# google/dynibar

Measured on AMD Instinct MI355X. Metric: rays/sec (64 samples x 8 src views), higher is better.
Workload: dtype f32 in / f32 accumulate; products from two half-float parts per operand (22-bit operands, 3 of the 4 partial products on the f16 matrix pipe, ~2^-20 relative per product); the exact 6-term bf16 build is tested beside it

## Files before the change

### dynibar_amd/csrc/dyn_mlp.h

```cpp
#pragma once
#include <utility>

#include "dyn_device.h"

#ifndef DYN_EXCLUSIVE_CU
#define DYN_EXCLUSIVE_CU 1
#endif
#if DYN_EXCLUSIVE_CU && defined(__AMDGCN__)
#define DYN_CLAIM_REGISTER_FILE() asm volatile("; the whole register file" ::: "v255", "a255")
#else
#define DYN_CLAIM_REGISTER_FILE()
#endif
#define DYN_NET_THREADS 256
#define DYN_VIEW_THREADS 512

__host__ __device__ constexpr int dyn_fi(int r, int h) { return (r & 3) + 8 * (r >> 2) + 4 * h; }

__device__ __forceinline__ f32x16 mfma32(float a, float b, f32x16 c) { return __builtin_amdgcn_mfma_f32_32x32x2f32(a, b, c, 0, 0, 0); }

template <int NT>
__device__ __forceinline__ void acc_zero(f32x16 (&acc)[NT]) {
#pragma unroll
  for (int t = 0; t < NT; ++t)
#pragma unroll
// ... 201 lines not shown
  int fill, issued;
  int nbuf;
#ifdef DYN_PHASE_TIMING
  int kid;
#endif
};


#ifndef B6_DMA_POLICY
#define B6_DMA_POLICY ""
#endif
#ifndef B6_DMA_WINDOW_NUM
#define B6_DMA_WINDOW_NUM 2
#define B6_DMA_WINDOW_DEN 3
#endif
template <int OFF>
__device__ __forceinline__ void b6_dma_piece(const float* g_uniform, unsigned lane_off, unsigned l, float* l_emu) {
#if defined(__AMDGCN__)
#pragma clang diagnostic push
#pragma clang diagnostic ignored "-Winline-asm"
  asm volatile("s_mov_b32 m0, %2\n\ts_nop 0\n\tglobal_load_lds_dwordx4 %0, %1 offset:%3" B6_DMA_POLICY ::"v"(lane_off), "s"(g_uniform), "s"(l), "n"(OFF) : "m0", "memory");
#pragma clang diagnostic pop
#else
  __builtin_amdgcn_global_load_lds((const __attribute__((address_space(1))) void*)((const char*)g_uniform + lane_off),
                                   (__attribute__((address_space(3))) void*)l_emu, 16, OFF, 0);
#endif
}
__device__ __forceinline__ int ring6_pieces(const WeightRing6& R) { return B6_CHUNK / R.round; }
__device__ __forceinline__ void ring6_piece(const WeightRing6& R, int k) {
  const int waves = R.round / 256, per_wave = B6_CHUNK / waves;
  const int grp = k / 6, i = k % 6;
  const int chunk = R.fill;
  const float* gu = R.gbase + (long)(chunk + (chunk >= R.skip_at ? R.skip_n : 0)) * B6_CHUNK + grp * 1536;
  const int slot = R.nbuf == 2 ? (chunk & 1) : 0;
  const unsigned l = R.lds_wave + (unsigned)((slot * B6_CHUNK + grp * 1536) * sizeof(float));
  float* le = R.buf + slot * B6_CHUNK + (threadIdx.x >> 6) * per_wave + 512 + grp * 1536;
  if (i == 0) b6_dma_piece<-2048>(gu, R.lane_off, l, le);
  if (i == 1) b6_dma_piece<-1024>(gu, R.lane_off, l, le);
  if (i == 2) b6_dma_piece<0>(gu, R.lane_off, l, le);
  if (i == 3) b6_dma_piece<1024>(gu, R.lane_off, l, le);
  if (i == 4) b6_dma_piece<2048>(gu, R.lane_off, l, le);
  if (i == 5) b6_dma_piece<3072>(gu, R.lane_off, l, le);
}
__device__ __forceinline__ void ring6_feed(WeightRing6& R, int pr, int npc) {
  if (R.fill < 0) return;
  const int n = ring6_pieces(R);
  const int den = (B6_DMA_WINDOW_NUM * npc + B6_DMA_WINDOW_DEN - 1) / B6_DMA_WINDOW_DEN > 0 ? (B6_DMA_WINDOW_NUM * npc + B6_DMA_WINDOW_DEN - 1) / B6_DMA_WINDOW_DEN : 1;
  int want = (n * (pr + 1) + den - 1) / den;
  if (want > n) want = n;
  for (; R.issued < want; ++R.issued) ring6_piece(R, R.issued);
}

__device__ __forceinline__ void ring6_issue(const WeightRing6& R, int chunk) {
  const int waves = R.round / 256, wave = threadIdx.x >> 6, lane = threadIdx.x & 63;
  const int per_wave = B6_CHUNK / waves;
  const float* g = R.gbase + (long)(chunk + (chunk >= R.skip_at ? R.skip_n : 0)) * B6_CHUNK + wave * per_wave + 512 + lane * 4;
  float* l = R.buf + (R.nbuf == 2 ? (chunk & 1) : 0) * B6_CHUNK + wave * per_wave + 512;
#pragma unroll
  for (int grp = 0; grp < 2; ++grp)
    if (grp * 1536 < per_wave) {
      const auto* gg = (const __attribute__((address_space(1))) void*)(g + grp * 1536);
      auto* ll = (__attribute__((address_space(3))) void*)(l + grp * 1536);
      __builtin_amdgcn_global_load_lds(gg, ll, 16, -2048, 0);
      __builtin_amdgcn_global_load_lds(gg, ll, 16, -1024, 0);
      __builtin_amdgcn_global_load_lds(gg, ll, 16, 0, 0);
      __builtin_amdgcn_global_load_lds(gg, ll, 16, 1024, 0);
      __builtin_amdgcn_global_load_lds(gg, ll, 16, 2048, 0);
      __builtin_amdgcn_global_load_lds(gg, ll, 16, 3072, 0);
    }
}
__device__ __forceinline__ void ring6_init(WeightRing6& R, const float* stream, int total, float* lds, int skip_at = 1 << 30, int skip_n = 0,
                                           int threads = 0, int nbuf = 2) {
  R.gbase = stream;
  R.buf = lds;
  R.next = 0;
  R.total = total - skip_n;
  R.skip_at = skip_at;
  R.skip_n = skip_n;
  R.round = (threads > 0 ? threads : (int)blockDim.x) * 4;
  R.nbuf = nbuf;
#if defined(__AMDGCN__)
  R.half = __builtin_amdgcn_readfirstlane((int)threadIdx.x >> 8);
#else
  R.half = (int)threadIdx.x >> 8;
#endif
  {
    const int waves = R.round / 256, per_wave = B6_CHUNK / waves;
#if defined(__AMDGCN__)
    const int wave = __builtin_amdgcn_readfirstlane((int)threadIdx.x >> 6);
    R.lds_wave = (unsigned)(size_t)(__attribute__((address_space(3))) void*)(lds + wave * per_wave + 512);
#else
    const int wave = (int)threadIdx.x >> 6;
    R.lds_wave = 0;
#endif
    R.lane_off = (unsigned)((wave * per_wave + 512 + (threadIdx.x & 63) * 4) * sizeof(float));
  }
  R.fill = -1;
  R.issued = 0;
  DYN_PHASE_RING_KID(R, 0);
  ring6_issue(R, 0);
}
__device__ __forceinline__ const float* ring6_acquire(WeightRing6& R) {
  DYN_PHASE_T0
  if (R.nbuf == 1) {
    const int c = R.next++;
    if (c > 0) {
      __syncthreads();
      ring6_issue(R, c);
    }
    __builtin_amdgcn_s_waitcnt(0x0F70);
    __syncthreads();
    DYN_PHASE_WAIT(R, c);
    return R.buf;
  }
  if (R.fill >= 0) {
    const int n = ring6_pieces(R);
    for (; R.issued < n; ++R.issued) ring6_piece(R, R.issued);
    R.fill = -1;
  }
  __builtin_amdgcn_s_waitcnt(0x0F70);
#ifdef DYN_PHASE_SKEW
  const unsigned long long skew_t1 = __builtin_readcyclecounter();
#endif
  __syncthreads();
  const int c = R.next++;
#ifdef DYN_PHASE_SKEW
  if ((threadIdx.x & 63) == 0 && blockIdx.x == gridDim.x / 2 && R.kid == 0) {
    g_skew[threadIdx.x >> 6][0] += skew_t1 - phase_t0;
    g_skew[threadIdx.x >> 6][1] += __builtin_readcyclecounter() - skew_t1;
    g_skew[threadIdx.x >> 6][2] += 1;
  }
#endif
  DYN_PHASE_WAIT(R, c);
  R.fill = c + 1 < R.total ? c + 1 : -1;
  R.issued = 0;
  return R.buf + (c & 1) * B6_CHUNK;
}

#ifndef B6_PRIO_FLIP
#define B6_PRIO_FLIP 2
#endif
#ifndef B6_PRIO_MODE
#define B6_PRIO_MODE 5
#endif
__device__ __forceinline__ void ring6_prio_flip(const WeightRing6& R, int phase) {
#if defined(__AMDGCN__)
  if (R.round != 8 * 256) return;
#if B6_PRIO_MODE == 1
  if (phase & 1) __builtin_amdgcn_s_setprio(1);
  else __builtin_amdgcn_s_setprio(0);
#elif B6_PRIO_MODE == 5
  if ((((int)threadIdx.x >> 8) ^ phase) & 1) __builtin_amdgcn_s_setprio(1);
  else __builtin_amdgcn_s_setprio(0);
#endif
#endif
}
__device__ __forceinline__ void split3_pair(float a, float b, unsigned& hi, unsigned& mid, unsigned& lo) {
#if DYN_SPLIT_F16
  const auto h = __builtin_amdgcn_cvt_pkrtz(a, b);
  hi = __builtin_bit_cast(unsigned, h);
#if defined(__AMDGCN__)
  unsigned m;
  asm("v_fma_mixlo_f16 %0, %1, -1.0, %2 op_sel_hi:[1,0,0]" : "=v"(m) : "v"(hi), "v"(a));
  asm("v_fma_mixhi_f16 %0, %1, -1.0, %2 op_sel:[1,0,0] op_sel_hi:[1,0,0]" : "+v"(m) : "v"(hi), "v"(b));
  mid = m;
#else
  const float ra = a - (float)h[0], rb = b - (float)h[1];
  mid = __builtin_bit_cast(unsigned, __builtin_amdgcn_cvt_pkrtz(ra, rb));
#endif
  lo = 0u;
#else
  f32x2v v = {a, b};
  hi = __builtin_bit_cast(unsigned, __builtin_convertvector(v, bf16x2v));
  f32x2v hf = {__uint_as_float(hi << 16), __uint_as_float(hi & 0xffff0000u)};
  f32x2v r1 = v - hf;
  mid = __builtin_bit_cast(unsigned, __builtin_convertvector(r1, bf16x2v));
#if DYN_SPLIT_PARTS == 3
  f32x2v mf = {__uint_as_float(mid << 16), __uint_as_float(mid & 0xffff0000u)};
  f32x2v r2 = r1 - mf;
  lo = __builtin_bit_cast(unsigned, __builtin_convertvector(r2, bf16x2v));
#else
  lo = 0u;
#endif
#endif
}

__device__ __forceinline__ f32x16 mfma_bf16(u32x4v a, u32x4v b, f32x16 c) {
#if DYN_SPLIT_F16
  return __builtin_amdgcn_mfma_f32_32x32x16_f16(__builtin_bit_cast(f16x8, a), __builtin_bit_cast(f16x8, b), c, 0, 0, 0);
#else
  return __builtin_amdgcn_mfma_f32_32x32x16_bf16(__builtin_bit_cast(bf16x8, a), __builtin_bit_cast(bf16x8, b), c, 0, 0, 0);
#endif
}

__host__ __device__ constexpr int b6_layer_chunks(int NT, int NSLOTS, int CP = B6_CHUNK_PAIRS) {
  return (((NSLOTS + 7) / 8) + (CP / NT) - 1) / (CP / NT);
}

struct B6A {
  u32x4v hi, mid, lo;
};
__device__ __forceinline__ B6A b6_load_a(const float* pair, int lane) {
  const u32x4v* w = reinterpret_cast<const u32x4v*>(pair) + lane;
  B6A a;
  a.hi = w[0]; a.mid = w[64];
#if DYN_SPLIT_PARTS == 3
  a.lo = w[128];
#endif
  return a;
}

template <int NSLOTS, int P0, int P1, class Feed>
__device__ __forceinline__ void b6_split_pairs(Feed& feed, int g, u32x4v& bh, u32x4v& bm, u32x4v& bl) {
#pragma unroll
  for (int p2 = P0; p2 < P1; ++p2) {
    const float v0 = (g * 8 + 2 * p2 < NSLOTS) ? feed(g * 8 + 2 * p2) : 0.f;
    const float v1 = (g * 8 + 2 * p2 + 1 < NSLOTS) ? feed(g * 8 + 2 * p2 + 1) : 0.f;
    unsigned h_, m_, l_;
    split3_pair(v0, v1, h_, m_, l_);
    bh[p2] = h_; bm[p2] = m_; bl[p2] = l_;
  }
}

#ifndef B6_AHEAD
#define B6_AHEAD 1
#endif
template <int NT, int NSLOTS, int AHEAD = B6_AHEAD, class Feed>
__device__ __forceinline__ void mlp_layer_b6(WeightRing6& R, f32x16 (&acc)[NT], Feed&& feed) {
  constexpr int NG = (NSLOTS + 7) / 8;
  constexpr int GPC = B6_CHUNK_PAIRS / NT;
  constexpr int NCH = (NG + GPC - 1) / GPC;
  static_assert(B6_CHUNK_PAIRS % NT == 0, "tiles per layer must divide the pairs of a chunk");
  static_assert(NT == 1 || NT == 2 || NT == 4 || NT == 8, "output tiles per layer");
  const int lane = threadIdx.x & 63;
  u32x4v bh, bm, bl, nh, nm, nl;
  b6_split_pairs<NSLOTS, 0, 4>(feed, 0, bh, bm, bl);
  nh = bh; nm = bm; nl = bl;
  __builtin_amdgcn_sched_barrier(0);
#pragma unroll
  for (int c = 0; c < NCH; ++c) {
    const float* buf = ring6_acquire(R);
    constexpr int NPC_MAX = B6_CHUNK_PAIRS;
    const int npc = (NG - c * GPC < GPC ? NG - c * GPC : GPC) * NT;
    B6A q[AHEAD + 1];
#pragma unroll
    for (int i = 0; i < AHEAD; ++i)
      if (i < npc) q[i] = b6_load_a(buf + i * B6_PAIR_FLOATS, lane);
    __builtin_amdgcn_sched_barrier(0);
#pragma unroll
    for (int pr = 0; pr < NPC_MAX; ++pr) {
      if (pr < npc) {
        const int gi = pr / NT, t = pr % NT;
        const int g = c * GPC + gi;
        ring6_feed(R, pr, npc);
#if B6_PRIO_FLIP && (B6_PRIO_MODE == 1 || B6_PRIO_MODE == 5)
        if (pr % B6_PRIO_FLIP == 0) ring6_prio_flip(R, (pr / B6_PRIO_FLIP) & 1);
#endif
        if (pr + AHEAD < npc) q[(pr + AHEAD) % (AHEAD + 1)] = b6_load_a(buf + (pr + AHEAD) * B6_PAIR_FLOATS, lane);
        if (g + 1 < NG) {
          if (NT == 1) b6_split_pairs<NSLOTS, 0, 4>(feed, g + 1, nh, nm, nl);
          if (NT == 2 && t == 0) b6_split_pairs<NSLOTS, 0, 2>(feed, g + 1, nh, nm, nl);
          if (NT == 2 && t == 1) b6_split_pairs<NSLOTS, 2, 4>(feed, g + 1, nh, nm, nl);
          if (NT == 4 && t == 0) b6_split_pairs<NSLOTS, 0, 1>(feed, g + 1, nh, nm, nl);
          if (NT == 4 && t == 1) b6_split_pairs<NSLOTS, 1, 2>(feed, g + 1, nh, nm, nl);
          if (NT == 4 && t == 2) b6_split_pairs<NSLOTS, 2, 3>(feed, g + 1, nh, nm, nl);
          if (NT == 4 && t == 3) b6_split_pairs<NSLOTS, 3, 4>(feed, g + 1, nh, nm, nl);
          if (NT == 8 && t == 0) b6_split_pairs<NSLOTS, 0, 1>(feed, g + 1, nh, nm, nl);
          if (NT == 8 && t == 2) b6_split_pairs<NSLOTS, 1, 2>(feed, g + 1, nh, nm, nl);
          if (NT == 8 && t == 4) b6_split_pairs<NSLOTS, 2, 3>(feed, g + 1, nh, nm, nl);
          if (NT == 8 && t == 6) b6_split_pairs<NSLOTS, 3, 4>(feed, g + 1, nh, nm, nl);
        }
        const B6A& cur = q[pr % (AHEAD + 1)];
#if DYN_SPLIT_TERMS == 6
        acc[t] = mfma_bf16(cur.lo, bh, acc[t]);
        acc[t] = mfma_bf16(cur.hi, bl, acc[t]);
        acc[t] = mfma_bf16(cur.mid, bm, acc[t]);
#endif
        acc[t] = mfma_bf16(cur.mid, bh, acc[t]);
        acc[t] = mfma_bf16(cur.hi, bm, acc[t]);
        acc[t] = mfma_bf16(cur.hi, bh, acc[t]);
        if (t == NT - 1) { bh = nh; bm = nm; bl = nl; }
        __builtin_amdgcn_sched_barrier(0);
      }
    }
  }
}

#ifndef B6D_AHEAD
#define B6D_AHEAD 4
#endif
#define B6D_SLOTS 3
struct WeightRing3 {
  const float* gbase;
  const float* glane;
  float* buf;
  unsigned lds_wave;
  unsigned lane_off;
  int next, total;
  int waves;
  int cf;
  int fill, issued;
  float* slot[B6D_SLOTS];
  unsigned lds_slot[B6D_SLOTS];
  int wrap;
  bool more;
#ifdef DYN_PHASE_TIMING
  int kid;
#endif
};
template <int OFF>
__device__ __forceinline__ void ring3_dma(const float* g, float* l_emu, unsigned l, const float* g_uniform, unsigned lane_off) {
#if defined(__AMDGCN__)
#pragma clang diagnostic push
#pragma clang diagnostic ignored "-Winline-asm"
  asm volatile("s_mov_b32 m0, %2\n\ts_nop 0\n\tglobal_load_lds_dwordx4 %0, %1 offset:%3" ::"v"(lane_off), "s"(g_uniform), "s"(l), "n"(OFF) : "m0", "memory");
#pragma clang diagnostic pop
#else
  __builtin_amdgcn_global_load_lds((const __attribute__((address_space(1))) void*)g, (__attribute__((address_space(3))) void*)l_emu, 16, OFF, 0);
#endif
}
__device__ __forceinline__ int ring3_pieces(const WeightRing3& R) { return R.cf / (R.waves * 256); }
__device__ __forceinline__ void ring3_piece(const WeightRing3& R, int chunk, int k) {
  const int per_wave = R.cf / R.waves;
  const int grp = k / 6, i = k % 6;
  const int sc = chunk >= R.total ? chunk - R.total : chunk;
  const float* g = R.glane + (long)sc * R.cf + grp * 1536;
  const float* gu = R.gbase + (long)sc * R.cf + grp * 1536;
  const unsigned l = R.lds_slot[chunk % B6D_SLOTS] + (unsigned)(grp * 1536 * sizeof(float));
  float* le = R.slot[chunk % B6D_SLOTS] + (threadIdx.x >> 6) * per_wave + 512 + grp * 1536;
  if (i == 0) ring3_dma<-2048>(g, le, l, gu, R.lane_off);
  if (i == 1) ring3_dma<-1024>(g, le, l, gu, R.lane_off);
  if (i == 2) ring3_dma<0>(g, le, l, gu, R.lane_off);
  if (i == 3) ring3_dma<1024>(g, le, l, gu, R.lane_off);
  if (i == 4) ring3_dma<2048>(g, le, l, gu, R.lane_off);
  if (i == 5) ring3_dma<3072>(g, le, l, gu, R.lane_off);
}
template <int ALLOW = 0>
__device__ __forceinline__ void ring3_barrier() {
#if defined(__AMDGCN__)
  static_assert(ALLOW >= 0 && ALLOW < 16, "vmcnt immediate");
  __builtin_amdgcn_s_waitcnt(0x0F70 | ALLOW);
  __builtin_amdgcn_s_barrier();
#else
  __syncthreads();
#endif
}
__device__ __forceinline__ void ring3_init(WeightRing3& R, const float* stream, int total, float* lds, int threads, int chunk_pairs = B6_CHUNK_PAIRS) {
  R.gbase = stream;
  R.buf = lds;
  R.next = 0;
  R.total = total;
  R.waves = threads / 64;
  R.cf = chunk_pairs * B6_PAIR_FLOATS;
  {
    const int per_wave = R.cf / R.waves;
#if defined(__AMDGCN__)
    const int wave = __builtin_amdgcn_readfirstlane((int)threadIdx.x >> 6);
    R.lds_wave = (unsigned)(size_t)(__attribute__((address_space(3))) void*)(lds + wave * per_wave + 512);
#else
    const int wave = threadIdx.x >> 6;
    R.lds_wave = 0;
#endif
    R.glane = stream + wave * per_wave + 512 + (threadIdx.x & 63) * 4;
    R.lane_off = (unsigned)((wave * per_wave + 512 + (threadIdx.x & 63) * 4) * sizeof(float));
  }
  R.fill = -1;
  R.issued = 0;
  R.wrap = 0;
  R.more = false;
  for (int j = 0; j < B6D_SLOTS; ++j) {
    R.slot[j] = lds + j * R.cf;
    R.lds_slot[j] = R.lds_wave + (unsigned)(j * R.cf * sizeof(float));
  }
  DYN_PHASE_RING_KID(R, 0);
  for (int c = 0; c < 2 && c < total; ++c)
    for (int k = 0; k < ring3_pieces(R); ++k) ring3_piece(R, c, k);
}
__device__ __forceinline__ void ring3_enter(WeightRing3& R) {
  if (R.next != 0) return;
  const int n = R.total > 1 ? ring3_pieces(R) : 0;
  if (n == 12) ring3_barrier<12>();
  else if (n == 8) ring3_barrier<8>();
  else if (n == 6) ring3_barrier<6>();
  else if (n == 4) ring3_barrier<4>();
  else ring3_barrier<0>();
}
__device__ __forceinline__ const float* ring3_slot(const WeightRing3& R, int chunk) { return R.slot[chunk % B6D_SLOTS]; }
#ifndef B6D_DMA_MARGIN
#define B6D_DMA_MARGIN 4
#endif
__device__ __forceinline__ void ring3_feed(WeightRing3& R, int half, int num, int den) {
  if (R.fill < 0) return;
  if (R.fill >= R.total && !R.more) return;
  const int n = ring3_pieces(R), h0 = n / 2;
  int want = half == 0 ? (h0 * num + den - 1) / den : h0 + ((n - h0) * num + den - 1) / den;
  if (want > n) want = n;
  for (; R.issued < want; ++R.issued) ring3_piece(R, R.fill, R.issued);
}
__device__ __forceinline__ void ring3_mid(WeightRing3& R) {
  DYN_PHASE_T0
  ring3_feed(R, 1, 1, 1);
  if (R.next + 1 < R.total || R.wrap) ring3_barrier();
  DYN_PHASE_WAIT(R, R.next);
  R.fill = (R.next + 2 < R.total || R.wrap) ? R.next + 2 : -1;
  R.issued = 0;
}
__device__ __forceinline__ void ring3_leave(WeightRing3& R) {
  if (R.wrap && R.next == R.total - 1) ring3_feed(R, 1, 1, 1);
  ++R.next;
}
__device__ __forceinline__ void ring3_next_pass(WeightRing3& R) {
  float* s0[B6D_SLOTS];
  unsigned l0[B6D_SLOTS];
  for (int j = 0; j < B6D_SLOTS; ++j) { s0[j] = R.slot[j]; l0[j] = R.lds_slot[j]; }
  for (int j = 0; j < B6D_SLOTS; ++j) { R.slot[j] = s0[(R.total + j) % B6D_SLOTS]; R.lds_slot[j] = l0[(R.total + j) % B6D_SLOTS]; }
  R.next = 0;
  R.fill = -1;
  R.issued = 0;
}

__device__ __forceinline__ float relu1(float v) {
#if defined(__AMDGCN__)
  float r;
  asm("v_max_f32_e32 %0, 0, %1" : "=v"(r) : "v"(v));
  return r;
#else
  return v > 0.f ? v : 0.f;
#endif
}

template <class F, int... Is>
__device__ __forceinline__ void dyn_static_for_impl(F&& f, std::integer_sequence<int, Is...>) {
  (f(std::integral_constant<int, Is>{}), ...);
}
template <int N, class F>
__device__ __forceinline__ void dyn_static_for(F&& f) {
  dyn_static_for_impl(static_cast<F&&>(f), std::make_integer_sequence<int, N>{});
}
#define DYN_INLINE_LAMBDA __attribute__((always_inline))

__device__ __forceinline__ f32x16 mfma_pinned(const u32x4v& a, u32x4v& b, f32x16 c) {
#if defined(__AMDGCN__)
  asm volatile("" : "+v"(b));
  f32x16 d = mfma_bf16(a, b, c);
  asm volatile("" : "+a"(d));
  return d;
#else
  return mfma_bf16(a, b, c);
#endif
}

template <int NT, int NSLOTS, int CP = B6_CHUNK_PAIRS, int AHEAD = B6D_AHEAD, class Feed>
__device__ __forceinline__ void mlp_layer_b6_duo(WeightRing3& R, f32x16 (&acc)[NT], Feed&& feed) {
  constexpr int NG = (NSLOTS + 7) / 8;
  constexpr int NP = NG * NT;
  constexpr int U = NT >= 2 ? 2 : 1;
  constexpr int QN = AHEAD + U;
  constexpr int NM = 3 * 4 * U / NT;
  static_assert(CP % NT == 0 && (NT == 1 || NT == 2 || NT == 4 || NT == 8), "output tiles per layer; pairs per chunk (CP) a multiple of them");
  static_assert(AHEAD % 2 == 0 && AHEAD >= 2 && AHEAD <= CP / 2, "the look-ahead must stay inside the published half chunk");
  const int lane = threadIdx.x & 63;
  const int c0 = R.next;
  u32x4v bh, bm, bl, nh, nm, nl;
  b6_split_pairs<NSLOTS, 0, 4>(feed, 0, bh, bm, bl);
  nh = bh; nm = bm; nl = bl;
  float v0 = 0.f, v1 = 0.f;
  B6A q[QN];
  auto load = [&](int P) DYN_INLINE_LAMBDA {
    return b6_load_a(ring3_slot(R, c0 + P / CP) + (P % CP) * B6_PAIR_FLOATS, lane);
  };
  ring3_enter(R);
#if !defined(__AMDGCN__)
  for (int i = 0; i < AHEAD && i < NP; ++i) q[i % QN] = load(i);
  for (int P = 0; P < NP; P += U) {
    const int pr = P % CP, npc = NP - (P - pr) < CP ? NP - (P - pr) : CP, mid = (npc / 2) / U * U;
    const int g = P / NT, t0 = P % NT, t1 = t0 + U - 1, um = (P % NT) / U;
    if (pr == mid) ring3_mid(R);
    auto gap = [&](int K) {
      for (int m = 0; m < NM; ++m) {
        const int at = NT == 1 ? 0 : (NM <= 4 ? 2 + m : m * 6 / NM);
        if (at != K || g + 1 >= NG) continue;
        const int step = um * NM + m, p2 = step / 3, st = step % 3, s0 = (g + 1) * 8 + 2 * p2;
        if (st == 0) v0 = s0 < NSLOTS ? feed(s0) : 0.f;
        if (st == 1) v1 = s0 + 1 < NSLOTS ? feed(s0 + 1) : 0.f;
        if (st == 2) {
          unsigned h_, m_, l_;
          split3_pair(v0, v1, h_, m_, l_);
          nh[p2] = h_; nm[p2] = m_; nl[p2] = l_;
        }
      }
    };
    auto dma = [&](int done) {
      const int wend = mid - B6D_DMA_MARGIN;
      if (pr >= mid) ring3_feed(R, 0, pr + done - mid, npc - mid);
      else if (wend <= 0) ring3_feed(R, 1, 1, 1);
      else ring3_feed(R, 1, pr + done < wend ? pr + done : wend, wend);
    };
    if (P + AHEAD < NP) q[(P + AHEAD) % QN] = load(P + AHEAD);
    gap(0);
    const B6A a0 = q[P % QN], a1 = q[(P + U - 1) % QN];
#if DYN_SPLIT_TERMS == 6
    acc[t0] = mfma_bf16(a0.lo, bh, acc[t0]);
    if (U == 2) acc[t1] = mfma_bf16(a1.lo, bh, acc[t1]);
    acc[t0] = mfma_bf16(a0.hi, bl, acc[t0]);
    if (U == 2) acc[t1] = mfma_bf16(a1.hi, bl, acc[t1]);
    acc[t0] = mfma_bf16(a0.mid, bm, acc[t0]);
    if (U == 2) acc[t1] = mfma_bf16(a1.mid, bm, acc[t1]);
#endif
    acc[t0] = mfma_bf16(a0.mid, bh, acc[t0]);
    if (U == 2) {
      if (P + AHEAD + 1 < NP) q[(P + AHEAD + 1) % QN] = load(P + AHEAD + 1);
      gap(1);
      acc[t1] = mfma_bf16(a1.mid, bh, acc[t1]);
      gap(2);
    }
    acc[t0] = mfma_bf16(a0.hi, bm, acc[t0]);
    if (U == 2) {
      gap(3);
      dma(1);
      acc[t1] = mfma_bf16(a1.hi, bm, acc[t1]);
      gap(4);
    }
    acc[t0] = mfma_bf16(a0.hi, bh, acc[t0]);
    if (U == 2) {
      gap(5);
      dma(U);
      acc[t1] = mfma_bf16(a1.hi, bh, acc[t1]);
    } else {
      dma(U);
    }
    if (t1 == NT - 1) { bh = nh; bm = nm; bl = nl; }
    if (pr + U == npc) ring3_leave(R);
  }
  return;
#endif
  dyn_static_for<(AHEAD < NP ? AHEAD : NP)>([&](auto I) DYN_INLINE_LAMBDA { q[decltype(I)::value % QN] = load(decltype(I)::value); });
  __builtin_amdgcn_sched_barrier(0);
  dyn_static_for<NP / U>([&](auto I) DYN_INLINE_LAMBDA {
    constexpr int P = decltype(I)::value * U;
    constexpr int pr = P % CP;
    constexpr int npc = NP - (P - pr) < CP ? NP - (P - pr) : CP;
    constexpr int mid = (npc / 2) / U * U;
    constexpr int g = P / NT, t0 = P % NT, t1 = t0 + U - 1;
    constexpr int um = (P % NT) / U;
    if constexpr (pr == mid) ring3_mid(R);
    auto gap = [&](auto K) DYN_INLINE_LAMBDA {
      dyn_static_for<NM>([&](auto M) DYN_INLINE_LAMBDA {
        constexpr int m = decltype(M)::value;
        constexpr int at = NT == 1 ? 0 : (NM <= 4 ? 2 + m : m * 6 / NM);
        if constexpr (at == decltype(K)::value && g + 1 < NG) {
          constexpr int step = um * NM + m, p2 = step / 3, st = step % 3, s0 = (g + 1) * 8 + 2 * p2;
          if constexpr (st == 0) v0 = s0 < NSLOTS ? feed(s0) : 0.f;
          if constexpr (st == 1) v1 = s0 + 1 < NSLOTS ? feed(s0 + 1) : 0.f;
          if constexpr (st == 2) {
            unsigned h_, m_, l_;
            split3_pair(v0, v1, h_, m_, l_);
            nh[p2] = h_; nm[p2] = m_; nl[p2] = l_;
          }
        }
      });
    };
    auto dma = [&](auto D) DYN_INLINE_LAMBDA {
      constexpr int done = decltype(D)::value;
      constexpr int wend = mid - B6D_DMA_MARGIN;
      if constexpr (pr >= mid) ring3_feed(R, 0, pr + done - mid, npc - mid);
      else if constexpr (wend <= 0) ring3_feed(R, 1, 1, 1);
      else ring3_feed(R, 1, pr + done < wend ? pr + done : wend, wend);
    };
    if constexpr (P + AHEAD < NP) q[(P + AHEAD) % QN] = load(P + AHEAD);
    gap(std::integral_constant<int, 0>{});
    const B6A& a0 = q[P % QN];
    const B6A& a1 = q[(P + U - 1) % QN];
#if DYN_SPLIT_TERMS == 6
    acc[t0] = mfma_pinned(a0.lo, bh, acc[t0]);
    if constexpr (U == 2) acc[t1] = mfma_pinned(a1.lo, bh, acc[t1]);
    acc[t0] = mfma_pinned(a0.hi, bl, acc[t0]);
    if constexpr (U == 2) acc[t1] = mfma_pinned(a1.hi, bl, acc[t1]);
    acc[t0] = mfma_pinned(a0.mid, bm, acc[t0]);
    if constexpr (U == 2) acc[t1] = mfma_pinned(a1.mid, bm, acc[t1]);
#endif
    acc[t0] = mfma_pinned(a0.mid, bh, acc[t0]);
    __builtin_amdgcn_sched_barrier(0);
    if constexpr (U == 2) {
      if constexpr (P + AHEAD + 1 < NP) q[(P + AHEAD + 1) % QN] = load(P + AHEAD + 1);
      gap(std::integral_constant<int, 1>{});
      acc[t1] = mfma_pinned(a1.mid, bh, acc[t1]);
      __builtin_amdgcn_sched_barrier(0);
      gap(std::integral_constant<int, 2>{});
    }
    acc[t0] = mfma_pinned(a0.hi, bm, acc[t0]);
    if constexpr (U == 2) {
      __builtin_amdgcn_sched_barrier(0);
      gap(std::integral_constant<int, 3>{});
      dma(std::integral_constant<int, 1>{});
      acc[t1] = mfma_pinned(a1.hi, bm, acc[t1]);
      __builtin_amdgcn_sched_barrier(0);
      gap(std::integral_constant<int, 4>{});
    }
    acc[t0] = mfma_pinned(a0.hi, bh, acc[t0]);
    if constexpr (U == 2) {
      __builtin_amdgcn_sched_barrier(0);
      gap(std::integral_constant<int, 5>{});
      dma(std::integral_constant<int, U>{});
      acc[t1] = mfma_pinned(a1.hi, bh, acc[t1]);
    } else {
      dma(std::integral_constant<int, U>{});
    }
    if constexpr (t1 == NT - 1) { bh = nh; bm = nm; bl = nl; }
    if constexpr (pr + U == npc) ring3_leave(R);
    __builtin_amdgcn_sched_barrier(0);
  });
}

template <int NT, int NSLOTS, int AHEAD = B6_AHEAD, class Feed>
__device__ __forceinline__ void mlp_layer_b6_lds(const float* w, f32x16 (&acc)[NT], Feed&& feed) {
  constexpr int NG = (NSLOTS + 7) / 8, NPR = NG * NT;
  static_assert(NT == 1 || NT == 2 || NT == 4 || NT == 8, "output tiles per layer");
  const int lane = threadIdx.x & 63;
  u32x4v bh, bm, bl, nh, nm, nl;
  b6_split_pairs<NSLOTS, 0, 4>(feed, 0, bh, bm, bl);
  nh = bh; nm = bm; nl = bl;
  B6A q[AHEAD + 1];
#pragma unroll
  for (int i = 0; i < AHEAD; ++i)
    if (i < NPR) q[i] = b6_load_a(w + i * B6_PAIR_FLOATS, lane);
  __builtin_amdgcn_sched_barrier(0);
#pragma unroll
  for (int pr = 0; pr < NPR; ++pr) {
    const int g = pr / NT, t = pr % NT;
    if (pr + AHEAD < NPR) q[(pr + AHEAD) % (AHEAD + 1)] = b6_load_a(w + (pr + AHEAD) * B6_PAIR_FLOATS, lane);
    if (g + 1 < NG) {
      if (NT == 1) b6_split_pairs<NSLOTS, 0, 4>(feed, g + 1, nh, nm, nl);
      if (NT == 2 && t == 0) b6_split_pairs<NSLOTS, 0, 2>(feed, g + 1, nh, nm, nl);
      if (NT == 2 && t == 1) b6_split_pairs<NSLOTS, 2, 4>(feed, g + 1, nh, nm, nl);
      if (NT == 4 && t == 0) b6_split_pairs<NSLOTS, 0, 1>(feed, g + 1, nh, nm, nl);
      if (NT == 4 && t == 1) b6_split_pairs<NSLOTS, 1, 2>(feed, g + 1, nh, nm, nl);
      if (NT == 4 && t == 2) b6_split_pairs<NSLOTS, 2, 3>(feed, g + 1, nh, nm, nl);
      if (NT == 4 && t == 3) b6_split_pairs<NSLOTS, 3, 4>(feed, g + 1, nh, nm, nl);
      if (NT == 8 && t == 0) b6_split_pairs<NSLOTS, 0, 1>(feed, g + 1, nh, nm, nl);
      if (NT == 8 && t == 2) b6_split_pairs<NSLOTS, 1, 2>(feed, g + 1, nh, nm, nl);
      if (NT == 8 && t == 4) b6_split_pairs<NSLOTS, 2, 3>(feed, g + 1, nh, nm, nl);
      if (NT == 8 && t == 6) b6_split_pairs<NSLOTS, 3, 4>(feed, g + 1, nh, nm, nl);
    }
    const B6A& cur = q[pr % (AHEAD + 1)];
#if DYN_SPLIT_TERMS == 6
    acc[t] = mfma_bf16(cur.lo, bh, acc[t]);
    acc[t] = mfma_bf16(cur.hi, bl, acc[t]);
    acc[t] = mfma_bf16(cur.mid, bm, acc[t]);
#endif
    acc[t] = mfma_bf16(cur.mid, bh, acc[t]);
    acc[t] = mfma_bf16(cur.hi, bm, acc[t]);
    acc[t] = mfma_bf16(cur.hi, bh, acc[t]);
    if (t == NT - 1) { bh = nh; bm = nm; bl = nl; }
    __builtin_amdgcn_sched_barrier(0);
  }
}

template <int NSLOTS>
struct B6TileW {
  B6A a[(NSLOTS + 7) / 8];
};
template <int NT, int NSLOTS>
__device__ __forceinline__ void b6_tile_prefetch(const float* layer_chunks, int my_tile, B6TileW<NSLOTS>& w) {
  constexpr int NG = (NSLOTS + 7) / 8;
  constexpr int GPC = B6_CHUNK_PAIRS / NT;
  const int lane = threadIdx.x & 63;
#pragma unroll
  for (int g = 0; g < NG; ++g) w.a[g] = b6_load_a(layer_chunks + (g / GPC) * B6_CHUNK + ((g % GPC) * NT + my_tile) * B6_PAIR_FLOATS, lane);
}
template <int NSLOTS, class Feed>
__device__ __forceinline__ void b6_tile_apply(const B6TileW<NSLOTS>& w, f32x16& acc, Feed&& feed) {
  constexpr int NG = (NSLOTS + 7) / 8;
#pragma unroll
  for (int g = 0; g < NG; ++g) {
    u32x4v bh, bm, bl;
    b6_split_pairs<NSLOTS, 0, 4>(feed, g, bh, bm, bl);
#if DYN_SPLIT_TERMS == 6
    acc = mfma_bf16(w.a[g].lo, bh, acc);
    acc = mfma_bf16(w.a[g].hi, bl, acc);
    acc = mfma_bf16(w.a[g].mid, bm, acc);
#endif
    acc = mfma_bf16(w.a[g].mid, bh, acc);
    acc = mfma_bf16(w.a[g].hi, bm, acc);
    acc = mfma_bf16(w.a[g].hi, bh, acc);
  }
}

typedef WeightRing6 NetRing;
#define NET_CHUNK B6_CHUNK
#define net_ring_init ring6_init
#define net_ring_init_t(R, stream, total, lds, threads) ring6_init(R, stream, total, lds, 1 << 30, 0, threads)
#define net_ring_init_1(R, stream, total, lds, threads) ring6_init(R, stream, total, lds, 1 << 30, 0, threads, 1)
#define net_layer mlp_layer_b6
__host__ __device__ constexpr int net_layer_chunks(int NT, int NSLOTS) { return b6_layer_chunks(NT, NSLOTS); }
```

### dynibar_amd/csrc/dyn_nets.hip

```cpp
#include <math.h>
#include <stdlib.h>
#include <string.h>

#include <functional>
#include <vector>

#include "dyn_host.h"
#include "dyn_mlp.h"
#include "dyn_pack.h"

namespace {

using SlotFn = std::function<float(int t, int i, int s, int h)>;

thread_local int g_pack_chunk_pairs = B6_CHUNK_PAIRS;
void pack_layer_b6(std::vector<float>& out, int NT, int NSLOTS, const SlotFn& fn) {
  const int CPAIRS = g_pack_chunk_pairs, CFLOATS = CPAIRS * B6_PAIR_FLOATS;
  const int NG = (NSLOTS + 7) / 8, GPC = CPAIRS / NT, NCH = (NG + GPC - 1) / GPC;
  const size_t base = out.size();
  out.resize(base + (size_t)NCH * CFLOATS, 0.f);
  unsigned short* img = reinterpret_cast<unsigned short*>(out.data() + base);
  for (int c = 0; c < NCH; ++c)
    for (int gi = 0; gi < GPC; ++gi) {
      const int g = c * GPC + gi;
      if (g >= NG) continue;
      for (int t = 0; t < NT; ++t)
        for (int lane = 0; lane < 64; ++lane)
          for (int e = 0; e < 8; ++e) {
            const int s = g * 8 + e;
            if (s >= NSLOTS) continue;
            const float w = fn(t, lane & 31, s, lane >> 5);
            unsigned short hi, mid, lo;
            split_weight(w, hi, mid, lo);
            const size_t pair = (size_t)c * CFLOATS * 2 + (size_t)(gi * NT + t) * B6_PAIR_FLOATS * 2;
            img[pair + 0 * 512 + lane * 8 + e] = hi;
            img[pair + 1 * 512 + lane * 8 + e] = mid;
            if (DYN_SPLIT_PARTS == 3) img[pair + 2 * 512 + lane * 8 + e] = lo;
          }
    }
}

void pack_net_layer(std::vector<float>& out, int NT, int NSLOTS, const SlotFn& fn) {
  pack_layer_b6(out, NT, NSLOTS, fn);
}

inline int chain_feature(int s, int h) { return 32 * (s / 16) + dyn_fi(s % 16, h); }

SlotFn chained(const float* W, const float* b, int nout, int nin, int ld, int col0 = 0) {
  return [=](int t, int i, int s, int h) -> float {
    const int n = 32 * t + i;
    if (n >= nout) return 0.f;
    const int nsteps_in = nin / 2;
    if (s < nsteps_in) return W[(size_t)n * ld + col0 + chain_feature(s, h)];
    if (s == nsteps_in && h == 0 && b != nullptr) return b[n];
    return 0.f;
  };
}

void pack_rowtab(std::vector<float>& out, const float* w, int n, double scale = 1.0) {
  for (int h = 0; h < 2; ++h)
    for (int k = 0; k < n / 2; ++k) out.push_back((float)((double)w[chain_feature(k, h)] * scale));
}

SlotFn scaled_wb(SlotFn fn, int nsteps_w, double kw, double kb) {
  return [=](int t, int i, int s, int h) -> float { return (float)((double)fn(t, i, s, h) * (s < nsteps_w ? kw : kb)); };
}

SlotFn scaled(SlotFn fn, double scale) {
  if (scale == 1.0) return fn;
  return [=](int t, int i, int s, int h) -> float { return (float)((double)fn(t, i, s, h) * scale); };
}

}

enum {
  ST_RAYDIR0_W, ST_RAYDIR0_B, ST_RAYDIR2_W, ST_RAYDIR2_B, ST_REFFEAT_W, ST_REFFEAT_B, ST_BASE0_W, ST_BASE0_B, ST_BASE2_W, ST_BASE2_B,
  ST_VIS0_W, ST_VIS0_B, ST_VIS2_W, ST_VIS2_B, ST_VISB0_W, ST_VISB0_B, ST_VISB2_W, ST_VISB2_B, ST_GEO0_W, ST_GEO0_B, ST_GEO2_W,
  ST_GEO2_B, ST_WQ, ST_WK, ST_WV, ST_FC, ST_LN_G, ST_LN_B, ST_OG0_W, ST_OG0_B, ST_OG2_W, ST_OG2_B, ST_RGB0_W, ST_RGB0_B,
  ST_RGB2_W, ST_RGB2_B, ST_RGB4_W, ST_RGB4_B, ST_S, ST_NUM_TENSORS
};

#define SA_L1P_STEPS 17
#define SA_L1V_STEPS 36
#define SA_L2_STEPS 128
#define SA_NX 37
#define SA_L3_STEPS (3 * SA_NX + 1)
#define SA_L3P_STEPS (2 * SA_NX)
#define SA_L3V_STEPS (SA_NX + 1)
#define SA_L4_STEPS 128
#define SA_L5_STEPS 64
constexpr int SA_CHUNKS = net_layer_chunks(8, SA_L1P_STEPS) + net_layer_chunks(8, SA_L1V_STEPS) + net_layer_chunks(2, SA_L2_STEPS) + net_layer_chunks(8, SA_L3P_STEPS) + net_layer_chunks(8, SA_L3V_STEPS) +
                          net_layer_chunks(4, SA_L4_STEPS) + 3 * net_layer_chunks(4, SA_L5_STEPS);
#ifndef DYN_POINTS_DUO
#define DYN_POINTS_DUO (DYN_SPLIT_TERMS == 3 ? 1 : 0)
#endif
#ifndef DYN_POINTS_PERSIST
#define DYN_POINTS_PERSIST 0
#endif
#if DYN_POINTS_DUO
#define PTS_CP 16
#define PTS_CHUNK (PTS_CP * B6_PAIR_FLOATS)
#define PTS_RING_SLOTS B6D_SLOTS
__host__ __device__ constexpr int pts_layer_chunks(int NT, int NSLOTS) { return b6_layer_chunks(NT, NSLOTS, PTS_CP); }
typedef WeightRing3 PtsRing;
#define pts_ring_init(R, stream, total, lds) ring3_init(R, stream, total, lds, DYN_NET_THREADS, PTS_CP)
#define PTS_LAYER(NT, NSLOTS) mlp_layer_b6_duo<NT, NSLOTS, PTS_CP>
#else
#define PTS_CHUNK NET_CHUNK
#define PTS_RING_SLOTS 2
__host__ __device__ constexpr int pts_layer_chunks(int NT, int NSLOTS) { return net_layer_chunks(NT, NSLOTS); }
typedef NetRing PtsRing;
#define pts_ring_init(R, stream, total, lds) net_ring_init_t(R, stream, total, lds, DYN_NET_THREADS)
#define PTS_LAYER(NT, NSLOTS) net_layer<NT, NSLOTS>
#endif
constexpr int SB_CHUNKS = pts_layer_chunks(8, 129) + pts_layer_chunks(4, 129) + 4 * pts_layer_chunks(4, 64) + 2 * pts_layer_chunks(4, 65);
#define SC_L11_STEPS 67
constexpr int SC_CHUNKS = net_layer_chunks(4, SC_L11_STEPS) + net_layer_chunks(2, 64);
#define SA_CT 848
#define SB_CT 400
#define SC_CT 144
constexpr size_t ST_OFF_A = 0;
constexpr size_t ST_OFF_B = ST_OFF_A + (size_t)SA_CHUNKS * NET_CHUNK;
constexpr size_t ST_OFF_C = ST_OFF_B + (size_t)SB_CHUNKS * PTS_CHUNK;
constexpr size_t ST_OFF_CTA = ST_OFF_C + (size_t)SC_CHUNKS * NET_CHUNK;
constexpr size_t ST_OFF_CTB = ST_OFF_CTA + SA_CT;
constexpr size_t ST_OFF_CTC = ST_OFF_CTB + SB_CT;
constexpr size_t ST_OFF_REF = ST_OFF_CTC + SC_CT;
constexpr size_t ST_BLOB_FLOATS = ST_OFF_REF + 35 * 66 + 36;

enum {
  DT_RAYDIR0_W, DT_RAYDIR0_B, DT_RAYDIR2_W, DT_RAYDIR2_B, DT_BASE0_W, DT_BASE0_B, DT_BASE2_W, DT_BASE2_B, DT_VIS0_W, DT_VIS0_B, DT_VIS2_W,
  DT_VIS2_B, DT_VISB0_W, DT_VISB0_B, DT_VISB2_W, DT_VISB2_B, DT_GEO0_W, DT_GEO0_B, DT_GEO2_W, DT_GEO2_B, DT_WQ, DT_WK, DT_WV, DT_FC, DT_LN_G,
  DT_LN_B, DT_REFPTS0_W, DT_REFPTS0_B, DT_REFPTS2_W, DT_REFPTS2_B, DT_OG0_W, DT_OG0_B, DT_OG2_W, DT_OG2_B, DT_RGB0_W, DT_RGB0_B, DT_RGB2_W,
  DT_RGB2_B, DT_RGB4_W, DT_RGB4_B, DT_NUM_TENSORS
};
#define DA_NX 18
#define DA_L3_STEPS (3 * DA_NX + 1)
#define DA_L3P_STEPS (2 * DA_NX)
#define DA_L3V_STEPS (DA_NX + 1)
constexpr int DA_CHUNKS = net_layer_chunks(8, DA_L3P_STEPS) + net_layer_chunks(8, DA_L3V_STEPS) + net_layer_chunks(4, SA_L4_STEPS) + 3 * net_layer_chunks(4, SA_L5_STEPS);
constexpr int DB_CHUNKS = pts_layer_chunks(8, 129) + pts_layer_chunks(4, 129) + 4 * pts_layer_chunks(4, 64) + pts_layer_chunks(8, 81) +
                          pts_layer_chunks(4, 129) + pts_layer_chunks(4, 65) + pts_layer_chunks(4, 78) + pts_layer_chunks(2, 65);
#define DB_CT 592
constexpr size_t DY_OFF_A = 0;
constexpr size_t DY_OFF_B = DY_OFF_A + (size_t)DA_CHUNKS * NET_CHUNK;
constexpr size_t DY_OFF_CTA = DY_OFF_B + (size_t)DB_CHUNKS * PTS_CHUNK;
constexpr size_t DY_OFF_CTB = DY_OFF_CTA + SA_CT;
constexpr size_t DY_OFF_POSENC = DY_OFF_CTB + DB_CT;
constexpr size_t DY_OFF_TIME = DY_OFF_POSENC + 256 * 128;
constexpr size_t DY_BLOB_FLOATS = DY_OFF_TIME + 256 * 21 + 256 + 35 * 256 + 36;
__host__ __device__ constexpr int da_c35(int q, int h) { return h == 0 ? q : (q < 17 ? 18 + q : -1); }

__host__ __device__ constexpr int sa_c70(int q, int h) {
  if (q < 18) return h == 0 ? q : (q < 17 ? 18 + q : -1);
  if (q < 34) return 35 + dyn_fi(q - 18, h);
  return h == 0 ? 35 + 32 + (q - 34) : -1;
}

static int sa_l1p_col(int s, int h) {
  if (s < 15) {
    const int c = s / 5, fi = s % 5;
    return 3 + (h * 5 + fi) * 3 + c;
  }
  const int k = (s - 15) * 2 + h;
  return k < 3 ? k : -1;
}
static int sa_l1v_col(int s, int h) {
  if (s < 30) {
    const int c = s / 5, fi = s % 5;
    return 33 + 6 + (h * 5 + fi) * 6 + c;
  }
  const int k = (s - 30) * 2 + h;
  if (k < 6) return 33 + k;
  if (k < 10) return 99 + (k - 6);
  return k == 10 ? -2 : -1;
}

extern "C" size_t dyn_static_net_blob_floats(void) { return ST_BLOB_FLOATS; }

extern "C" int dyn_static_net_pack(const float* const* T, int F, float* blob, size_t blob_floats) {
  DYN_REQUIRE(T && blob, "dyn_static_net_pack: null pointer");
  DYN_REQUIRE(F == 32, "dyn_static_net_pack: the kernels are specialised for 32 feature channels (coarse_feat_dim = fine_feat_dim = 32)");
  DYN_REQUIRE(blob_floats >= ST_BLOB_FLOATS, "dyn_static_net_pack: blob too small");
  for (int i = 0; i < ST_NUM_TENSORS; ++i) DYN_REQUIRE(T[i] != nullptr, "dyn_static_net_pack: tensor %d is NULL", i);
  std::vector<float> o;
  g_pack_range_error = false;
  o.reserve(ST_BLOB_FLOATS);
  {
    const float *W = T[ST_RAYDIR0_W], *b = T[ST_RAYDIR0_B];
    pack_net_layer(o, 8, SA_L1P_STEPS, scaled([=](int t, int i, int s, int h) -> float {
      const int n = 32 * t + i, c = sa_l1p_col(s, h);
      return c >= 0 ? W[n * 103 + c] : 0.f;
    }, DYN_ELU_PRE));
    pack_net_layer(o, 8, SA_L1V_STEPS, scaled([=](int t, int i, int s, int h) -> float {
      const int n = 32 * t + i, c = sa_l1v_col(s, h);
      return c >= 0 ? W[n * 103 + c] : (c == -2 ? b[n] : 0.f);
    }, DYN_ELU_PRE));
  }
  pack_net_layer(o, 2, SA_L2_STEPS, scaled(chained(T[ST_RAYDIR2_W], nullptr, 35, 256, 256), DYN_ELU_POST));
  {
    const float *W = T[ST_BASE0_W], *b = T[ST_BASE0_B];
    pack_net_layer(o, 8, SA_L3P_STEPS, scaled([=](int t, int i, int s, int h) -> float {
      const int c = sa_c70(s % SA_NX, h);
      return c < 0 ? 0.f : W[(32 * t + i) * 210 + (s / SA_NX) * 70 + c];
    }, DYN_ELU_PRE));
    pack_net_layer(o, 8, SA_L3V_STEPS, scaled([=](int t, int i, int s, int h) -> float {
      const int n = 32 * t + i;
      if (s == SA_NX) return h == 0 ? b[n] : 0.f;
      const int c = sa_c70(s, h);
      return c < 0 ? 0.f : W[n * 210 + 140 + c];
    }, DYN_ELU_PRE));
  }
  pack_net_layer(o, 4, SA_L4_STEPS, scaled(chained(T[ST_BASE2_W], nullptr, 128, 256, 256), DYN_ELU_POST));
  pack_net_layer(o, 4, SA_L5_STEPS, scaled(chained(T[ST_VIS0_W], nullptr, 128, 128, 128), DYN_ELU_PRE));
  pack_net_layer(o, 4, SA_L5_STEPS, scaled(chained(T[ST_VIS2_W], nullptr, 128, 128, 128), DYN_ELU_POST));
  pack_net_layer(o, 4, SA_L5_STEPS, scaled(chained(T[ST_VISB0_W], nullptr, 128, 128, 128), DYN_ELU_PRE));
  DYN_REQUIRE(o.size() == ST_OFF_B, "static pack: A stream size mismatch");
#if DYN_POINTS_DUO
  g_pack_chunk_pairs = PTS_CP;
#endif
  {
    const float *W = T[ST_GEO0_W], *b = T[ST_GEO0_B];
    pack_net_layer(o, 8, 129, scaled([=](int t, int i, int s, int h) -> float {
      const int n = 32 * t + i;
      if (s < 128) return W[n * 257 + (s < 64 ? 0 : 128) + chain_feature(s % 64, h)];
      return h == 0 ? W[n * 257 + 256] : b[n];
    }, DYN_ELU_PRE));
  }
  pack_net_layer(o, 4, 129, scaled_wb(chained(T[ST_GEO2_W], T[ST_GEO2_B], 128, 256, 256), 128, DYN_ELU_POST, 1.0));
  pack_net_layer(o, 4, 64, chained(T[ST_WQ], nullptr, 128, 128, 128));
  pack_net_layer(o, 4, 64, chained(T[ST_WK], nullptr, 128, 128, 128));
  pack_net_layer(o, 4, 64, chained(T[ST_WV], nullptr, 128, 128, 128));
  pack_net_layer(o, 4, 64, chained(T[ST_FC], nullptr, 128, 128, 128));
  pack_net_layer(o, 4, 65, scaled(chained(T[ST_OG0_W], T[ST_OG0_B], 128, 128, 128), DYN_ELU_PRE));
  pack_net_layer(o, 4, 65, scaled(chained(T[ST_RGB0_W], T[ST_RGB0_B], 128, 128, 261), DYN_ELU_PRE));
  g_pack_chunk_pairs = B6_CHUNK_PAIRS;
  DYN_REQUIRE(o.size() == ST_OFF_C, "static pack: B stream size mismatch");
  {
    const float* W = T[ST_RGB0_W];
    pack_net_layer(o, 4, SC_L11_STEPS, scaled([=](int t, int i, int s, int h) -> float {
      const int n = 32 * t + i;
      if (s < 64) return W[n * 261 + 128 + chain_feature(s, h)];
      const int k = (s - 64) * 2 + h;
      return k < 5 ? W[n * 261 + 256 + k] : 0.f;
    }, DYN_ELU_PRE));
  }
  pack_net_layer(o, 2, 64, scaled(chained(T[ST_RGB2_W], nullptr, 64, 128, 128), DYN_ELU_POST * DYN_ELU_PRE));
  DYN_REQUIRE(o.size() == ST_OFF_CTA, "static pack: C stream size mismatch");
  pack_rowtab(o, T[ST_VIS2_W] + 128 * 128, 128, DYN_ELU_POST);
  pack_rowtab(o, T[ST_VISB2_W], 128, DYN_ELU_POST);
  o.push_back(T[ST_VIS2_B][128]);
  o.push_back(T[ST_VISB2_B][0]);
  o.push_back(fabsf(T[ST_S][0]));
  o.resize(ST_OFF_CTA + 272, 0.f);
  pack_rowtab(o, T[ST_BASE2_B], 128);
  pack_rowtab(o, T[ST_VIS0_B], 128, DYN_ELU_PRE);
  pack_rowtab(o, T[ST_VIS2_B], 128);
  pack_rowtab(o, T[ST_VISB0_B], 128, DYN_ELU_PRE);
  {
    float b64[64] = {0.f};
    for (int i = 0; i < 35; ++i) b64[i] = T[ST_RAYDIR2_B][i];
    pack_rowtab(o, b64, 64);
  }
  o.resize(ST_OFF_CTB, 0.f);
  pack_rowtab(o, T[ST_LN_G], 128);
  pack_rowtab(o, T[ST_LN_B], 128);
  pack_rowtab(o, T[ST_OG2_W], 128, DYN_ELU_POST);
  o.push_back(T[ST_OG2_B][0]);
  o.resize(ST_OFF_CTC, 0.f);
  pack_rowtab(o, T[ST_RGB4_W], 64, DYN_ELU_POST);
  o.push_back(T[ST_RGB4_B][0]);
  o.resize(ST_OFF_CTC + 80, 0.f);
  pack_rowtab(o, T[ST_RGB2_B], 64, DYN_ELU_PRE);
  o.resize(ST_OFF_REF, 0.f);
  for (int i = 0; i < 35 * 66; ++i) o.push_back(T[ST_REFFEAT_W][i]);
  for (int i = 0; i < 35; ++i) o.push_back(T[ST_REFFEAT_B][i]);
  o.resize(ST_BLOB_FLOATS, 0.f);
  DYN_REQUIRE(!g_pack_range_error, "dyn_static_net_pack: a weight is outside the half-float range of the split engine (|w| >= 65504 or not finite)");
  for (size_t i = 0; i < ST_BLOB_FLOATS; ++i) blob[i] = o[i];
  return 0;
}

static bool dense_views(int V) {
  static const int mode = getenv("DYN_DENSE_VIEWS") ? atoi(getenv("DYN_DENSE_VIEWS")) : -1;
  if (mode == 0) return false;
  if (mode == 1) return V >= 9;
  return (V >= 9 && V <= 12) || (V >= 17 && V <= 26);
}
struct StaticWs {
  bool dense, ragged;
  long n_pts, n_tiles_a, n_tiles_b;
  int PT, TPR;
  size_t off_x, off_vis, off_gin, off_nvalid, off_hg, off_ref, total;
  size_t off_qkvg;
  long n_seg, n_wg_max;
  size_t off_bits, off_emin, off_segcnt, off_segstart, off_wgstart;
  size_t off_rowtab, off_ptab;
};
#define RAG_SEG 1024
#define RAG_SEG_WGS 160
#define RAG_MAX_PTS 32
#define RAG_PTAB 36

#define DYN_MAX_SAMPLES 256
#define SB_GIN_RECS 33
#define SB_HG_RECS 16

#ifndef DYN_BLEND_WS
#define DYN_BLEND_WS (DYN_SPLIT_TERMS == 3 ? 1 : 0)
#endif
static bool ragged_rows_enabled() {
  static const int off = getenv("DYN_RAGGED") ? (atoi(getenv("DYN_RAGGED")) == 0) : 0;
  static const int blend_stream = getenv("DYN_BLEND_STREAM") != nullptr;
  return DYN_BLEND_WS && !off && !blend_stream;
}
static StaticWs static_ws(int R, int S, int V, bool dynamic = false) {
  StaticWs w;
  w.n_pts = (long)R * S;
  w.dense = dense_views(V);
  w.ragged = w.dense && ragged_rows_enabled();
  w.PT = w.dense ? 256 / V : 32 / (V <= 4 ? 4 : (V <= 8 ? 8 : (V <= 16 ? 16 : 32)));
  w.n_tiles_a = w.dense ? ((w.n_pts + w.PT - 1) / w.PT) * 8 : (w.n_pts + w.PT - 1) / w.PT;
  w.n_seg = (w.n_pts + RAG_SEG - 1) / RAG_SEG;
  w.n_wg_max = w.ragged ? (w.n_pts + w.PT - 1) / w.PT + w.n_seg : 0;
  if (w.ragged) w.n_tiles_a = w.n_wg_max * 8;
  int tpr = (S + 31) / 32;
  w.TPR = tpr <= 1 ? 1 : (tpr <= 2 ? 2 : ((tpr + 3) / 4) * 4);
  w.n_tiles_b = (long)R * w.TPR;
  size_t o = 0;
  w.off_x = o; o += dynamic ? 0 : (size_t)w.n_tiles_a * 64 * 64;
  w.off_vis = o; o += dynamic ? 0 : (size_t)w.n_tiles_a * 128;
  w.off_gin = o; o += (size_t)w.n_tiles_b * SB_GIN_RECS * 256;
  w.off_nvalid = o; o += (size_t)((w.n_pts + 3) & ~3L);
  w.off_hg = o; o += dynamic ? 0 : (size_t)w.n_tiles_b * SB_HG_RECS * 256;
  w.off_ref = o; o += dynamic ? 64 : (size_t)R * 36;
  o = (o + 3) & ~(size_t)3;
  w.off_qkvg = o; o += w.TPR > 4 ? (size_t)w.n_tiles_b * 4 * 4096 : 0;
  w.off_bits = o; o += w.ragged ? (size_t)((w.n_pts + 3) & ~3L) : 0;
  w.off_emin = o; o += w.ragged ? (size_t)((w.n_pts + 3) & ~3L) : 0;
  w.off_segcnt = o; o += w.ragged ? (size_t)((w.n_seg + 3) & ~3L) : 0;
  w.off_segstart = o; o += w.ragged ? (size_t)w.n_seg * RAG_SEG_WGS : 0;
  w.off_wgstart = o; o += w.ragged ? (size_t)((w.n_wg_max + 2 + 3) & ~3L) : 0;
  w.off_rowtab = o; o += w.ragged ? (size_t)w.n_wg_max * 128 : 0;
  w.off_ptab = o; o += w.ragged ? (size_t)w.n_wg_max * RAG_PTAB : 0;
  w.total = o;
  return w;
}

extern "C" size_t dyn_static_net_workspace_bytes(int R, int S, int V) {
  if (R <= 0 || S <= 0 || V <= 0 || V > 32) return 0;
  return static_ws(R, S, V).total * sizeof(float);
}

__device__ __forceinline__ void unit3(float x, float y, float z, float& ox, float& oy, float& oz) {
  const float d = fmaxf(sqrtf(x * x + y * y + z * z), 1e-12f);
  ox = x / d; oy = y / d; oz = z / d;
}

__device__ __forceinline__ void sincos_small(float x, float& s, float& c) {
  const float y = rintf(x * 0.63661977236758134f);
  const int q = (int)y;
  float r = fmaf(y, -1.57079637050628662109375f, x);
  r = fmaf(y, 4.37113900018624283e-8f, r);
  const float z = r * r;
  const float ps = fmaf(fmaf(fmaf(-1.9515295891e-4f, z, 8.3321608736e-3f), z, -1.6666654611e-1f) * z, r, r);
  const float pc = fmaf(fmaf(fmaf(2.443315711809948e-5f, z, -1.388731625493765e-3f), z, 4.166664568298827e-2f), z * z, fmaf(z, -0.5f, 1.0f));
  const bool swap = q & 1;
  const float sv = swap ? pc : ps, cv = swap ? ps : pc;
  s = __uint_as_float(__float_as_uint(sv) ^ ((unsigned)(q & 2) << 30));
  c = __uint_as_float(__float_as_uint(cv) ^ ((unsigned)((q + 1) & 2) << 30));
}

template <int NF>
__device__ __forceinline__ void octave_embed(float x, int h, float* out) {
  float sn, cs;
  sincos_small(x, sn, cs);
#pragma unroll
  for (int f = 0; f < NF; ++f) {
    out[f] = h == 0 ? cs : sn;
    const float s2 = 2.0f * sn * cs;
    cs = cs * cs - sn * sn;
    sn = s2;
  }
}

#define REF_RAYS 8
__global__ void __launch_bounds__(256, 1) k_static_ref_feat(const float* __restrict__ ray_o, const float* __restrict__ ray_d, const float* __restrict__ Wref, int R,
                                  float* __restrict__ ref_feat) {
  DYN_CLAIM_REGISTER_FILE();
  float* pe = reinterpret_cast<float*>(dyn_smem);
  const int r0 = blockIdx.x * REF_RAYS;
  for (int t = threadIdx.x; t < REF_RAYS * 66; t += 256) {
    const int rl = t / 66, jj = t - rl * 66;
    const int r = r0 + rl < R ? r0 + rl : R - 1;
    float d[3], c[6];
    unit3(ray_d[r * 3], ray_d[r * 3 + 1], ray_d[r * 3 + 2], d[0], d[1], d[2]);
    const float ox = ray_o[r * 3], oy = ray_o[r * 3 + 1], oz = ray_o[r * 3 + 2];
    c[0] = d[0]; c[1] = d[1]; c[2] = d[2];
    c[3] = oy * d[2] - oz * d[1];
    c[4] = oz * d[0] - ox * d[2];
    c[5] = ox * d[1] - oy * d[0];
    if (dyn_ref_cross_axis(R) != DYN_CROSS_XYZ) {
      float m[3];
      dyn_ref_moment_over_rays(ray_o, ray_d, r, m);
      c[3] = m[0]; c[4] = m[1]; c[5] = m[2];
    }
    const int e = jj < 6 ? jj : (jj - 6) % 6;
    float ck = c[0];
    ck = e == 1 ? c[1] : ck; ck = e == 2 ? c[2] : ck; ck = e == 3 ? c[3] : ck; ck = e == 4 ? c[4] : ck; ck = e == 5 ? c[5] : ck;
    float v = ck;
    if (jj >= 6) {
      const int f = ((jj - 6) / 6) % 5, fn = (jj - 6) / 30;
      const float a = (float)(1 << f) * ck;
      v = fn == 0 ? cosf(a) : sinf(a);
    }
    pe[t] = v;
  }
  __syncthreads();
  for (int t = threadIdx.x; t < REF_RAYS * 36; t += 256) {
    const int rl = t / 36, ch = t - rl * 36;
    if (r0 + rl >= R) continue;
    float acc = 0.f;
    if (ch < 35) {
      const float* w = Wref + ch * 66;
      const float* x = pe + rl * 66;
      acc = Wref[35 * 66 + ch];
      for (int j = 0; j < 66; ++j) acc = fmaf(w[j], x[j], acc);
    }
    ref_feat[(long)(r0 + rl) * 36 + ch] = acc;
  }
}

struct StaticArgs {
  int R, S, V, PT, TPR;
  int anti_alias, mask_rgb;
  long n_pts, n_tiles_a, n_tiles_b;
  float shift;
  const float* blob;
  const float* ray_d;
  const float* pts;
  const float* rgb_feat;
  const float* ray_diff;
  const float* mask;
  const float* centers;
  float* raw;
  float* ws;
  StaticWs o;
  const unsigned* rg_bits;
  const float* rg_emin;
  const int* rg_wg;
  const unsigned short* rg_rowtab;
  const int* rg_ptab;
};
__device__ __forceinline__ long point_rec(const StaticArgs& p, long point, int h, int n_rec) {
  const long ray = point / p.S;
  const int smp = (int)(point - ray * p.S);
  return ((ray * p.TPR + (smp >> 5)) * n_rec) * 64 + (smp & 31) + 32 * h;
}

#define POOL_FLOATS(NX) (2 * (NX) * 2 * 32)
#define RES_STRIDE 260
#define RES_FLOATS (RES_STRIDE * 32)
__device__ __forceinline__ void res_put(float* res, int wave, int j, int h, const f32x16& acc) {
  float4* d = reinterpret_cast<float4*>(res + j * RES_STRIDE + wave * 32 + 4 * h);
#pragma unroll
  for (int q = 0; q < 4; ++q) d[2 * q] = make_float4(acc[4 * q], acc[4 * q + 1], acc[4 * q + 2], acc[4 * q + 3]);
}
__device__ __forceinline__ void res_get(const float* res, int col, int h, f32x16 (&a1)[8]) {
  const float4* s4 = reinterpret_cast<const float4*>(res + col * RES_STRIDE + 4 * h);
#pragma unroll
  for (int t = 0; t < 8; ++t)
#pragma unroll
    for (int q = 0; q < 4; ++q) {
      const float4 v = s4[t * 8 + 2 * q];
      a1[t][4 * q] = v.x; a1[t][4 * q + 1] = v.y; a1[t][4 * q + 2] = v.z; a1[t][4 * q + 3] = v.w;
    }
}

#define DENSE_STRIDE 258
#define DENSE_SCALARS 512
#define DENSE_EXTRA 2304
struct DenseRows {
  int V, PTW, rw, p_local, view, base;
  int cnt;
  float* scal;
  const int* pbase;
  long point0;
  int n_rows;
};
__device__ __forceinline__ DenseRows dense_rows(int V, int PTW, float* scal, long wgi = -1) {
  DenseRows d;
  d.V = V; d.PTW = PTW; d.scal = scal;
  d.rw = (threadIdx.x >> 6) * 32 + (threadIdx.x & 31);
  d.p_local = d.rw / V;
  d.view = d.rw - d.p_local * V;
  d.base = (d.p_local < PTW ? d.p_local : PTW - 1) * V;
  d.cnt = V;
  d.pbase = nullptr;
  d.point0 = (wgi >= 0 ? wgi : (long)blockIdx.x) * PTW;
  d.n_rows = PTW * V;
  return d;
}
__device__ __forceinline__ int dense_pt_base(const DenseRows& d, int pnt) { return d.pbase != nullptr ? d.pbase[pnt] : pnt * d.V; }
__device__ __forceinline__ int dense_pt_cnt(const DenseRows& d, int pnt) { return d.pbase != nullptr ? d.pbase[pnt + 1] - d.pbase[pnt] : d.V; }

struct RaggedHead {
  unsigned short ri;
  int n_rows, point0, np;
};
__device__ __forceinline__ RaggedHead ragged_head(const unsigned short* rowtab, const int* ptab, long wgi, int rw) {
  RaggedHead h;
  h.ri = rowtab[wgi * 256 + rw];
  h.n_rows = ptab[wgi * RAG_PTAB + 32];
  h.point0 = ptab[wgi * RAG_PTAB + 33];
  h.np = ptab[wgi * RAG_PTAB + 34];
  return h;
}
__device__ __forceinline__ DenseRows ragged_rows(int V, const unsigned short* rowtab, const int* ptab, long wgi, float* scal, int* pbase,
                                                 const RaggedHead* pre = nullptr) {
  const int tid = threadIdx.x;
  const int* pt = ptab + wgi * RAG_PTAB;
  DenseRows d;
  d.rw = (tid >> 6) * 32 + (tid & 31);
  const RaggedHead hd = pre != nullptr ? *pre : ragged_head(rowtab, ptab, wgi, d.rw);
  const unsigned short ri = hd.ri;
  if (pbase != nullptr && tid < RAG_PTAB) pbase[tid] = pt[tid];
  d.V = V; d.scal = scal; d.pbase = pbase != nullptr ? pbase : pt;
  d.n_rows = hd.n_rows;
  d.point0 = hd.point0;
  d.PTW = hd.np;
  const bool live = d.rw < d.n_rows;
  d.p_local = live ? (ri & 0xff) : RAG_MAX_PTS + 1;
  d.view = live ? (ri >> 8) : 0;
  const int pc = live ? d.p_local : d.PTW - 1;
  d.base = pt[pc];
  d.cnt = pt[pc + 1] - d.base;
  return d;
}

__device__ __forceinline__ float aa_exp(float s_abs, float dot) { return expm1f(s_abs * (dot - 1.0f)); }

__global__ void __launch_bounds__(256) k_ragged_points(long n_pts, int V, const float* __restrict__ mask, const float4* __restrict__ ray_diff, const float* __restrict__ s_abs,
                                                       unsigned* __restrict__ bits, float* __restrict__ emin) {
  float* dw = reinterpret_cast<float*>(dyn_smem);
  unsigned char* mk = reinterpret_cast<unsigned char*>(dw + 256 * V);
  const long p0 = (long)blockIdx.x * 256;
  const int np = (int)(n_pts - p0 < 256 ? n_pts - p0 : 256), n = np * V;
  const bool aa = s_abs != nullptr;
  for (int i = threadIdx.x; i < n; i += 256) {
    mk[i] = mask[p0 * V + i] != 0.f ? 1 : 0;
    if (aa) dw[i] = ray_diff[p0 * V + i].w;
  }
  __syncthreads();
  const int t = threadIdx.x;
  if (t >= np) return;
  unsigned b = 0u;
  float m = 3.0e38f;
  const float sa = aa ? s_abs[0] : 0.f;
  for (int v = 0; v < V; ++v) {
    if (mk[t * V + v]) b |= 1u << v;
    if (aa) m = fminf(m, aa_exp(sa, dw[t * V + v]));
  }
  bits[p0 + t] = b;
  if (aa) emin[p0 + t] = m;
}

__global__ void __launch_bounds__(256) k_ragged_segments(long n_pts, long n_seg, const unsigned* __restrict__ bits, int* __restrict__ seg_cnt, int* __restrict__ seg_start) {
  int* pre = reinterpret_cast<int*>(dyn_smem);
  int* part = pre + RAG_SEG + 4;
  unsigned short* nxt = reinterpret_cast<unsigned short*>(part + 256);
  const int tid = threadIdx.x;
  const long seg = blockIdx.x;
  const long p0 = seg * RAG_SEG;
  const int n = (int)((p0 + RAG_SEG < n_pts ? p0 + RAG_SEG : n_pts) - p0);
  int r4[4], sum = 0;
#pragma unroll
  for (int j = 0; j < 4; ++j) {
    const int i = 4 * tid + j;
    const unsigned b = i < n ? bits[p0 + i] : 0u;
    r4[j] = i < n ? (b != 0u ? __popc(b) : 1) : 0;
// ... 336 lines not shown
      for (int r = 0; r < 16; ++r) x[t][r] += elu1(a6[t][r]);
  }
  float vis2;
  {
    f32x16 a7[4];
    acc_init_bias<4>(a7, ctab + 656);
    DYN_PHASE(15);
    net_layer<4, SA_L5_STEPS>(ring, a7, [&](int s) { return x[s / 16][s % 16] * vis; });
    DYN_PHASE(16);
    acc_elu_s(a7);
    vis2 = sigmoid1(row_dot<4>(a7, ctab + 128) + ctab[257]) * msk;
  }
  DYN_PHASE(17);
  const bool tile_ok = tile < p.n_tiles_a;
  if (STORE_X && tile_ok) {
    float4* xw = reinterpret_cast<float4*>(p.ws + p.o.off_x) + tile * 16 * 64 + lane;
#pragma unroll
    for (int t = 0; t < 4; ++t)
#pragma unroll
      for (int q = 0; q < 4; ++q) nt_store4<4>(xw + (t * 4 + q) * 64, make_float4(x[t][q * 4], x[t][q * 4 + 1], x[t][q * 4 + 2], x[t][q * 4 + 3]));
    if (h == 0) nt_store1<4>(p.ws + p.o.off_vis + (tile * 32 + (lane & 31)) * 4, vis2);
  }
  DYN_PHASE(18);
  if constexpr (VSEG == 0) {
    const DenseRows& d = *dr;
    const int tid = threadIdx.x;
    float vsum, nvalid;
    dense_all2(d, vis2, msk, vsum, nvalid);
    const float w2 = vis2 / (vsum + 1e-8f);
    const float wmean = (vsum / (vsum + 1e-8f)) / (float)V;
    constexpr int XS = 132;
    float* tab = lds_base;
    float* wrow = lds_base + 256 * XS;
    const long point0 = d.point0;
    {
      float4* mine = reinterpret_cast<float4*>(tab + d.rw * XS) + h;
#pragma unroll
      for (int t = 0; t < 4; ++t)
#pragma unroll
        for (int q = 0; q < 4; ++q) mine[8 * t + 2 * q] = make_float4(x[t][q * 4], x[t][q * 4 + 1], x[t][q * 4 + 2], x[t][q * 4 + 3]);
      if (h == 0) wrow[d.rw] = w2;
    }
    __syncthreads();
    for (int task = tid; task < d.PTW * 32; task += DYN_VIEW_THREADS) {
      const int pnt = task >> 5, qd = task & 31;
      const int pb = dense_pt_base(d, pnt), pn = dense_pt_cnt(d, pnt);
      const float* src = tab + pb * XS + qd * 4;
      const float* w = wrow + pb;
      float4 m0 = make_float4(0.f, 0.f, 0.f, 0.f), m1 = m0;
      int k = 0;
      for (; k + 2 <= pn; k += 2) {
        const float4 x0 = dense_quad(src, k, XS, pn), x1 = dense_quad(src, k + 1, XS, pn);
        const float w0 = dense_w(w, k, pn), w1 = dense_w(w, k + 1, pn);
        m0.x = fmaf(w0, x0.x, m0.x); m0.y = fmaf(w0, x0.y, m0.y); m0.z = fmaf(w0, x0.z, m0.z); m0.w = fmaf(w0, x0.w, m0.w);
        m1.x = fmaf(w1, x1.x, m1.x); m1.y = fmaf(w1, x1.y, m1.y); m1.z = fmaf(w1, x1.z, m1.z); m1.w = fmaf(w1, x1.w, m1.w);
      }
      if (k < pn) {
        const float4 x0 = dense_quad(src, k, XS, pn);
        const float w0 = dense_w(w, k, pn);
        m0.x = fmaf(w0, x0.x, m0.x); m0.y = fmaf(w0, x0.y, m0.y); m0.z = fmaf(w0, x0.z, m0.z); m0.w = fmaf(w0, x0.w, m0.w);
      }
      const float mean[4] = {m0.x + m1.x, m0.y + m1.y, m0.z + m1.z, m0.w + m1.w};
      float v0[4] = {0.f, 0.f, 0.f, 0.f}, v1[4] = {0.f, 0.f, 0.f, 0.f};
      for (k = 0; k + 2 <= pn; k += 2) {
        const float4 x0 = dense_quad(src, k, XS, pn), x1 = dense_quad(src, k + 1, XS, pn);
        const float w0 = dense_w(w, k, pn), w1 = dense_w(w, k + 1, pn);
        const float a0[4] = {x0.x, x0.y, x0.z, x0.w}, b0[4] = {x1.x, x1.y, x1.z, x1.w};
#pragma unroll
        for (int e = 0; e < 4; ++e) {
          const float d0 = a0[e] - mean[e], d1 = b0[e] - mean[e];
          v0[e] = fmaf(w0, d0 * d0, v0[e]);
          v1[e] = fmaf(w1, d1 * d1, v1[e]);
        }
      }
      if (k < pn) {
        const float4 x0 = dense_quad(src, k, XS, pn);
        const float w0 = dense_w(w, k, pn);
        const float a0[4] = {x0.x, x0.y, x0.z, x0.w};
#pragma unroll
        for (int e = 0; e < 4; ++e) {
          const float d0 = a0[e] - mean[e];
          v0[e] = fmaf(w0, d0 * d0, v0[e]);
        }
      }
      const long pt = point0 + pnt;
      if (pt < p.n_pts) {
        const int g = 4 * (qd >> 3) + ((qd >> 1) & 3);
        float4* gin = reinterpret_cast<float4*>(p.ws + p.o.off_gin) + point_rec(p, pt, qd & 1, SB_GIN_RECS);
        nt_store4<4>(gin + g * 64, make_float4(mean[0], mean[1], mean[2], mean[3]));
        nt_store4<4>(gin + (16 + g) * 64, make_float4(v0[0] + v1[0], v0[1] + v1[1], v0[2] + v1[2], v0[3] + v1[3]));
      }
    }
    if (valid && d.rw == d.base) {
      float4* gin = reinterpret_cast<float4*>(p.ws + p.o.off_gin) + point_rec(p, point, h, SB_GIN_RECS);
      gin[32 * 64] = make_float4(h == 0 ? wmean : 1.0f, 0.f, 0.f, 0.f);
      if (h == 0) p.ws[p.o.off_nvalid + point] = nvalid;
    }
  } else {
  const float w2 = vis2 / (seg_sum<VSEG>(vis2, V, seg_base) + 1e-8f);
  const float wmean = seg_sum<VSEG>(w2, V, seg_base) / (float)V;
  const float nvalid = seg_sum<VSEG>(msk, V, seg_base);
  float4* gin = reinterpret_cast<float4*>(p.ws + p.o.off_gin) + (valid ? point_rec(p, point, h, SB_GIN_RECS) : 0);
#pragma unroll
  for (int t = 0; t < 4; ++t)
#pragma unroll
    for (int q = 0; q < 4; ++q) {
      float m[4], vv[4];
#pragma unroll
      for (int e = 0; e < 4; ++e) m[e] = x[t][q * 4 + e] * w2;
      seg_sum4<VSEG>(m[0], m[1], m[2], m[3]);
#pragma unroll
      for (int e = 0; e < 4; ++e) {
        const float d = x[t][q * 4 + e] - m[e];
        vv[e] = w2 * (d * d);
      }
      seg_sum4<VSEG>(vv[0], vv[1], vv[2], vv[3]);
      const int g = t * 4 + q;
      const int sel = g & (VSEG - 1);
      const bool mine = valid && (view == (sel < V ? sel : 0));
      if (mine) {
        nt_store4<4>(gin + g * 64, make_float4(m[0], m[1], m[2], m[3]));
        nt_store4<4>(gin + (16 + g) * 64, make_float4(vv[0], vv[1], vv[2], vv[3]));
      }
    }
  if (valid && view == 0) {
    gin[32 * 64] = make_float4(h == 0 ? wmean : 1.0f, 0.f, 0.f, 0.f);
    if (h == 0) p.ws[p.o.off_nvalid + point] = nvalid;
  }
  }
}

template <int VSEG, int VC = 0, bool RAG = false>
__global__ void __launch_bounds__(DYN_VIEW_THREADS, 2) k_static_views(StaticArgs p) {
  static_assert(VC == 0 || VSEG == 0, "a compile-time view count is a dense-rows specialisation");
  static_assert(!RAG || VSEG == 0, "ragged rows are a dense-rows flavour");
  if (RAG && (int)blockIdx.x >= p.rg_wg[0]) return;
  constexpr int PHASE_KID = 0;
  (void)PHASE_KID;
  float* lds = reinterpret_cast<float*>(dyn_smem);
  float* ctab = lds + 2 * NET_CHUNK;
  const int tid = threadIdx.x, lane = tid & 63, j = lane & 31, h = lane >> 5, wave = tid >> 6;
  for (int i = tid; i < SA_CT; i += DYN_VIEW_THREADS) ctab[i] = p.blob[ST_OFF_CTA + i];
  NetRing ring;
  DYN_PHASE(0);
  constexpr bool POOLED = VSEG >= 8 || VSEG == 0;
  constexpr int SA_L1P_CHUNKS = net_layer_chunks(8, SA_L1P_STEPS);
  constexpr int SA_POOLED_AT = SA_L1P_CHUNKS + net_layer_chunks(8, SA_L1V_STEPS) + net_layer_chunks(2, SA_L2_STEPS);
  constexpr int LDS_FLOATS = 2 * NET_CHUNK + SA_CT + POOL_FLOATS(SA_NX) + RES_FLOATS + (VSEG == 0 ? DENSE_EXTRA : 0);

  const int V = VC > 0 ? VC : p.V;
  const long tile = (long)blockIdx.x * (DYN_VIEW_THREADS / 64) + wave;
  const DenseRows dr = RAG ? ragged_rows(V, p.rg_rowtab, p.rg_ptab, blockIdx.x, lds + LDS_FLOATS - DENSE_SCALARS, reinterpret_cast<int*>(lds + LDS_FLOATS))
                           : dense_rows(V, VC > 0 ? 256 / VC : p.PT, lds + LDS_FLOATS - DENSE_SCALARS);
  const int PT = RAG ? dr.PTW : (VC > 0 ? 256 / VC : p.PT);
  const int p_local = VSEG == 0 ? dr.p_local : j / (VSEG == 0 ? 1 : VSEG);
  const int view = VSEG == 0 ? dr.view : (j & (VSEG - 1));
  const long point = VSEG == 0 ? dr.point0 + p_local : tile * PT + p_local;
  const bool valid = (VSEG == 0 ? p_local < PT : view < V) && (point < p.n_pts);
  const int seg_base = 0;
  const long pv = valid ? point * V + view : 0;
  net_ring_init(ring, p.blob + ST_OFF_A + (POOLED ? (size_t)SA_L1P_CHUNKS * NET_CHUNK : 0), SA_CHUNKS - (POOLED ? SA_L1P_CHUNKS : 0), lds,
                SA_POOLED_AT - (POOLED ? SA_L1P_CHUNKS : 0), POOLED ? net_layer_chunks(8, SA_L3P_STEPS) : 0, DYN_VIEW_THREADS);

  float msk = valid ? p.mask[pv] : 0.f;
  float4 rd = valid ? reinterpret_cast<const float4*>(p.ray_diff)[pv] : make_float4(0.f, 0.f, 0.f, 0.f);
  float px = 0.f, py = 0.f, pz = 0.f, cx = 0.f, cy = 0.f, cz = 0.f;
  if (valid) {
    px = p.pts[point * 3]; py = p.pts[point * 3 + 1]; pz = p.pts[point * 3 + 2];
    cx = p.centers[view * 16 + 12]; cy = p.centers[view * 16 + 13]; cz = p.centers[view * 16 + 14];
  }
  const int cross_axis = dyn_src_cross_axis(V, p.R, p.S);
  float mq[3] = {0.f, 0.f, 0.f};
  if (cross_axis != DYN_CROSS_XYZ && valid) {
    const int ray = (int)(point / p.S), smp = (int)(point - (long)ray * p.S);
    dyn_src_moment_over_axis(cross_axis, view, ray, smp,
        [&](int, int rr, int ss, float (&q)[3]) { const float* s3 = p.pts + ((long)rr * p.S + ss) * 3; q[0] = s3[0]; q[1] = s3[1]; q[2] = s3[2]; },
        [&](int vv, float (&c3)[3]) { c3[0] = p.centers[vv * 16 + 12]; c3[1] = p.centers[vv * 16 + 13]; c3[2] = p.centers[vv * 16 + 14]; }, mq);
  }
  float xin[SA_NX];
  f32x16 a1[8];
  const bool h0 = h == 0;
  if constexpr (POOLED) {
    B6TileW<SA_L1P_STEPS> pw1;
    b6_tile_prefetch<8, SA_L1P_STEPS>(p.blob + ST_OFF_A, wave, pw1);
    const int npw = VSEG == 0 ? PT : (DYN_VIEW_THREADS / 64) * PT;
    const long qp = VSEG == 0 ? dr.point0 + j : (long)blockIdx.x * npw + j;
    const bool qok = j < npw && qp < p.n_pts;
    const float qx = qok ? p.pts[qp * 3] : 0.f, qy = qok ? p.pts[qp * 3 + 1] : 0.f, qz = qok ? p.pts[qp * 3 + 2] : 0.f;
    float in1p[SA_L1P_STEPS];
    octave_embed<5>(qx, h, in1p);
    octave_embed<5>(qy, h, in1p + 5);
    octave_embed<5>(qz, h, in1p + 10);
    in1p[15] = h0 ? qx : qy;
    in1p[16] = h0 ? qz : 0.f;
    f32x16 accp[1];
    acc_zero(accp);
    b6_tile_apply<SA_L1P_STEPS>(pw1, accp[0], [&](int s) { return in1p[s]; });
    float* res = ctab + SA_CT + POOL_FLOATS(SA_NX);
    res_put(res, wave, j, h, accp[0]);
    __syncthreads();
    res_get(res, VSEG == 0 ? (dr.p_local < dr.PTW ? dr.p_local : dr.PTW - 1) : wave * PT + p_local, h, a1);
  } else {
    float in1p[SA_L1P_STEPS];
    octave_embed<5>(px, h, in1p);
    octave_embed<5>(py, h, in1p + 5);
    octave_embed<5>(pz, h, in1p + 10);
    in1p[15] = h0 ? px : py;
    in1p[16] = h0 ? pz : 0.f;
    acc_zero(a1);
    net_layer<8, SA_L1P_STEPS>(ring, a1, [&](int s) { return in1p[s]; });
  }
  {
    float c6[6];
    unit3(px - cx, py - cy, pz - cz, c6[0], c6[1], c6[2]);
    c6[3] = cy * c6[2] - cz * c6[1];
    c6[4] = cz * c6[0] - cx * c6[2];
    c6[5] = cx * c6[1] - cy * c6[0];
    if (cross_axis != DYN_CROSS_XYZ) { c6[3] = mq[0]; c6[4] = mq[1]; c6[5] = mq[2]; }
    float in1[SA_L1V_STEPS];
#pragma unroll
    for (int c = 0; c < 6; ++c) octave_embed<5>(c6[c], h, in1 + c * 5);
    in1[30] = h0 ? c6[0] : c6[1];
    in1[31] = h0 ? c6[2] : c6[3];
    in1[32] = h0 ? c6[4] : c6[5];
    in1[33] = h0 ? rd.x : rd.y;
    in1[34] = h0 ? rd.z : rd.w;
    in1[35] = h0 ? 1.0f : 0.0f;
    DYN_PHASE(1);
    net_layer<8, SA_L1V_STEPS>(ring, a1, [&](int s) { return in1[s]; });
    DYN_PHASE(2);
  }
  {
    f32x16 a2[2];
    acc_init_bias<2>(a2, ctab + 784);
    net_layer<2, SA_L2_STEPS>(ring, a2, [&](int s) {
      if (s == 64) {
#pragma unroll
        for (int q = 0; q < 18; ++q) {
          const int ch = h == 0 ? q : 18 + q;
          xin[q] = (valid && ch < 35) ? nt_load1<2>(p.rgb_feat + pv * 35 + ch) : 0.f;
        }
      }
      return elu_s(a1[s / 16][s % 16]);
    });
    const float* rf = p.ws + p.o.off_ref + (valid ? (point / p.S) * 36 : 0);
#pragma unroll
    for (int r = 0; r < 16; ++r) xin[18 + r] = a2[0][r] * rf[dyn_fi(r, h)];
#pragma unroll
    for (int r = 0; r < 3; ++r) xin[34 + r] = h == 0 ? a2[1][r] * rf[32 + r] : 0.f;
    if (h == 0 && tile < p.n_tiles_a) {
      float* rec = p.ws + p.o.off_vis + (tile * 32 + j) * 4;
      nt_store1<4>(rec + 1, xin[0]); nt_store1<4>(rec + 2, xin[1]); nt_store1<4>(rec + 3, xin[2]);
    }
  }
  DYN_PHASE(4);
  if (p.mask_rgb) {
    const float s3 = (xin[0] + xin[1]) + xin[2];
    msk *= (__shfl(s3, j) > 1e-3f) ? 1.0f : 0.0f;
  }
  float wgt;
  if (p.anti_alias) {
    const float e = ((VSEG == 0 ? p_local < PT : view < V)) ? aa_exp(ctab[258], rd.w) : 3.0e38f;
    const float emin = RAG ? (valid ? p.rg_emin[point] : e) : views_min<VSEG>(dr, e);
    wgt = (e - emin) * msk;
  } else {
    wgt = msk;
  }
  const float wraw = views_sum<VSEG>(dr, wgt);
  wgt = wgt / (wraw + 1e-8f);

  DYN_PHASE(5);
  base_fc0<VSEG, SA_NX>(ring, p.blob + ST_OFF_A + (size_t)SA_POOLED_AT * NET_CHUNK, xin, wgt, V, view, p_local, ctab + SA_CT, a1, &dr, wraw / (wraw + 1e-8f));
  DYN_PHASE(10);
  views_tail<VSEG, true>(ring, a1, p, ctab, wgt, msk, tile, point, valid, view, seg_base, &dr, lds, VC);
  DYN_PHASE(20);
}

#define SB_KL_FLOATS 4096
#define SB_VL_LD 132
#define SB_VL_FLOATS (32 * SB_VL_LD)

__device__ __forceinline__ void lds_barrier() {
#if defined(__AMDGCN__) && DYN_POINTS_DUO
  __builtin_amdgcn_s_waitcnt(0xC07F);
  __builtin_amdgcn_s_barrier();
#else
  __syncthreads();
#endif
}

constexpr int SB_CHUNKS_QKV = pts_layer_chunks(8, 129) + pts_layer_chunks(4, 129) + 3 * pts_layer_chunks(4, 64);
static int dyn_cu_count() {
  static int n_cu[DYN_MAX_DEVICES] = {0};
  int dev = 0;
  (void)hipGetDevice(&dev);
  const int slot = (dev >= 0 && dev < DYN_MAX_DEVICES) ? dev : 0;
  if (n_cu[slot] == 0) {
    hipDeviceProp_t prop;
    n_cu[slot] = (hipGetDeviceProperties(&prop, dev) == hipSuccess && prop.multiProcessorCount > 0) ? prop.multiProcessorCount : 256;
  }
  return n_cu[slot];
}

static dim3 points_grid(dim3 full) {
#if DYN_POINTS_DUO && DYN_POINTS_PERSIST
  static int n_cu[DYN_MAX_DEVICES] = {0};
  int dev = 0;
  (void)hipGetDevice(&dev);
  const int slot = (dev >= 0 && dev < DYN_MAX_DEVICES) ? dev : 0;
  if (n_cu[slot] == 0) {
    hipDeviceProp_t prop;
    n_cu[slot] = (hipGetDeviceProperties(&prop, dev) == hipSuccess && prop.multiProcessorCount > 0) ? prop.multiProcessorCount : 256;
  }
  static const int no_persist = getenv("DYN_POINTS_NO_PERSIST") != nullptr;
  return (no_persist || full.x <= (unsigned)n_cu[slot]) ? full : dim3((unsigned)n_cu[slot]);
#else
  return full;
#endif
}

template <bool DYN, int PHASE>
__global__ void __launch_bounds__(DYN_NET_THREADS, 1) k_net_points(StaticArgs p) {
  constexpr int PHASE_KID = 1;
  (void)PHASE_KID;
  DYN_PHASE(0);
  DYN_CLAIM_REGISTER_FILE();
  float* lds = reinterpret_cast<float*>(dyn_smem);
  float* ctab = lds + PTS_RING_SLOTS * PTS_CHUNK;
  float* Kl = ctab + (DYN ? DB_CT : SB_CT);
  float* Vl = Kl + SB_KL_FLOATS;
  const int tid = threadIdx.x, lane = tid & 63, j = lane & 31, h = lane >> 5, wave = tid >> 6;
  constexpr int CT = DYN ? DB_CT : SB_CT;
  for (int i = tid; i < CT; i += DYN_NET_THREADS) ctab[i] = p.blob[(DYN ? DY_OFF_CTB : ST_OFF_CTB) + i];
  PtsRing ring;
  if (PHASE == 2)
    pts_ring_init(ring, p.blob + (DYN ? DY_OFF_B : ST_OFF_B) + (size_t)SB_CHUNKS_QKV * PTS_CHUNK, (DYN ? DB_CHUNKS : SB_CHUNKS) - SB_CHUNKS_QKV, lds);
  else
    pts_ring_init(ring, p.blob + (DYN ? DY_OFF_B : ST_OFF_B), PHASE == 1 ? SB_CHUNKS_QKV : (DYN ? DB_CHUNKS : SB_CHUNKS), lds);
  DYN_PHASE_RING_KID(ring, 1);
  lds_barrier();

  const int TPR = p.TPR;
  const float one_h0 = h == 0 ? 1.0f : 0.0f;
  constexpr bool PERSIST = DYN_POINTS_PERSIST && DYN_POINTS_DUO && PHASE == 0;
  const long n_wg = (p.n_tiles_b + 3) / 4;
  auto gin_src = [&](long wgi, bool& valid_) DYN_INLINE_LAMBDA {
    const long tile_ = wgi * 4 + wave;
    const long ray_ = tile_ / TPR;
    valid_ = (ray_ < p.R) && ((int)(tile_ - ray_ * TPR) * 32 + j < p.S);
    return reinterpret_cast<const float4*>(p.ws + p.o.off_gin) + (tile_ < p.n_tiles_b ? tile_ : 0) * SB_GIN_RECS * 64 + lane;
  };
#if DYN_POINTS_DUO
  ring.wrap = PERSIST ? 1 : 0;
#endif
  long wgi = blockIdx.x;
  do {
  const bool more = PERSIST && wgi + gridDim.x < n_wg;
#if DYN_POINTS_DUO
  ring.more = more;
#endif
  const long tile = wgi * 4 + wave;
  const long ray = tile / TPR;
  const int kt_self = (int)(tile - ray * TPR);
  const int smp = kt_self * 32 + j;
  const bool valid = (ray < p.R) && (smp < p.S);
  const long point = valid ? ray * p.S + smp : 0;
  const float nvalid = valid ? p.ws[p.o.off_nvalid + point] : 0.f;

  float4* hand = reinterpret_cast<float4*>(p.ws + p.o.off_qkvg) + (PHASE == 0 ? 0 : tile * 4096) + lane;
  f32x16 g[4];
  if (PHASE == 2) {
    if (ray < p.R) {
#pragma unroll
      for (int t = 0; t < 4; ++t)
#pragma unroll
        for (int q = 0; q < 4; ++q) {
          const float4 v = hand[(t * 4 + q) * 64];
          g[t][q * 4] = v.x; g[t][q * 4 + 1] = v.y; g[t][q * 4 + 2] = v.z; g[t][q * 4 + 3] = v.w;
        }
    } else {
      acc_zero(g);
    }
  } else {
    f32x16 a9[8];
    {
      float gin[129];
      bool gv;
      const float4* src = gin_src(wgi, gv);
#pragma unroll
      for (int i = 0; i < 32; ++i) {
        const float4 v = gv ? nt_load4<4>(src + i * 64) : make_float4(0.f, 0.f, 0.f, 0.f);
        gin[i * 4] = v.x; gin[i * 4 + 1] = v.y; gin[i * 4 + 2] = v.z; gin[i * 4 + 3] = v.w;
      }
      gin[128] = gv ? src[32 * 64].x : (h == 1 ? 1.0f : 0.f);
      acc_zero(a9);
      PTS_LAYER(8, 129)(ring, a9, [&](int s) { return gin[s]; });
    }
    acc_zero(g);
    PTS_LAYER(4, 129)(ring, g, [&](int s) { return s < 128 ? elu_s(a9[s / 16][s % 16]) : one_h0; });
    acc_elu(g);
  }
  if (DYN && PHASE != 2) {
    const float4* pe = reinterpret_cast<const float4*>(p.blob + DY_OFF_POSENC + ((valid ? smp : 0) * 2 + h) * 64);
#pragma unroll
    for (int t = 0; t < 4; ++t)
#pragma unroll
      for (int q = 0; q < 4; ++q) {
        const float4 v = pe[t * 4 + q];
        g[t][q * 4] += v.x; g[t][q * 4 + 1] += v.y; g[t][q * 4 + 2] += v.z; g[t][q * 4 + 3] += v.w;
      }
  }
  DYN_PHASE(1);
  f32x16 att[4];
  const float inv_temp = 1.0f / 5.656854249492381f;
  const bool q_ok = nvalid > 1.0f;
  if (PHASE == 2) {
    f32x16 qh[4];
#pragma unroll
    for (int t = 0; t < 4; ++t)
#pragma unroll
      for (int q = 0; q < 4; ++q) {
        const float4 v = hand[(16 + t * 4 + q) * 64];
        qh[t][q * 4] = v.x * inv_temp; qh[t][q * 4 + 1] = v.y * inv_temp; qh[t][q * 4 + 2] = v.z * inv_temp; qh[t][q * 4 + 3] = v.w * inv_temp;
      }
    const float4* ray_hand = reinterpret_cast<const float4*>(p.ws + p.o.off_qkvg) + ray * TPR * 4096;
    const int n_blocks = TPR / 4;
#pragma unroll
    for (int hd = 0; hd < 4; ++hd) {
      float run_max = -3.0e38f, run_sum = 0.f;
      f32x16 oh;
#pragma unroll
      for (int r = 0; r < 16; ++r) oh[r] = 0.f;
      for (int kb = 0; kb < n_blocks; ++kb) {
        __syncthreads();
        {
          const float4* kv = ray_hand + (long)(kb * 4 + wave) * 4096 + lane;
#pragma unroll
          for (int q = 0; q < 4; ++q) {
            reinterpret_cast<float4*>(Kl)[(wave * 4 + q) * 64 + lane] = kv[(32 + hd * 4 + q) * 64];
            const float4 v = kv[(48 + hd * 4 + q) * 64];
            Vl[dyn_fi(q * 4 + 0, h) * SB_VL_LD + wave * 32 + j] = v.x;
            Vl[dyn_fi(q * 4 + 1, h) * SB_VL_LD + wave * 32 + j] = v.y;
            Vl[dyn_fi(q * 4 + 2, h) * SB_VL_LD + wave * 32 + j] = v.z;
            Vl[dyn_fi(q * 4 + 3, h) * SB_VL_LD + wave * 32 + j] = v.w;
          }
        }
        __syncthreads();
        f32x16 sc[4];
        acc_zero(sc);
#pragma unroll
        for (int kt = 0; kt < 4; ++kt)
#pragma unroll
          for (int q = 0; q < 4; ++q) {
            const float4 a = reinterpret_cast<const float4*>(Kl)[(kt * 4 + q) * 64 + lane];
            sc[kt] = mfma32(a.x, qh[hd][q * 4 + 0], sc[kt]);
            sc[kt] = mfma32(a.y, qh[hd][q * 4 + 1], sc[kt]);
            sc[kt] = mfma32(a.z, qh[hd][q * 4 + 2], sc[kt]);
            sc[kt] = mfma32(a.w, qh[hd][q * 4 + 3], sc[kt]);
          }
        float mx = run_max;
#pragma unroll
        for (int kt = 0; kt < 4; ++kt)
#pragma unroll
          for (int r = 0; r < 16; ++r) {
            const bool key_ok = (kb * 4 + kt) * 32 + dyn_fi(r, h) < p.S;
            float v = q_ok ? sc[kt][r] : -1e9f;
            v = key_ok ? v : -3.0e38f;
            sc[kt][r] = v;
            mx = fmaxf(mx, v);
          }
        mx = fmaxf(mx, __shfl_xor(mx, 32));
        const float rescale = __expf(run_max - mx);
        float sum = 0.f;
#pragma unroll
        for (int kt = 0; kt < 4; ++kt)
#pragma unroll
          for (int r = 0; r < 16; ++r) {
            const float e = sc[kt][r] > -1.0e38f ? __expf(sc[kt][r] - mx) : 0.f;
            sc[kt][r] = e;
            sum += e;
          }
        sum += __shfl_xor(sum, 32);
        run_sum = run_sum * rescale + sum;
        run_max = mx;
#pragma unroll
        for (int r = 0; r < 16; ++r) oh[r] *= rescale;
#pragma unroll
        for (int kt = 0; kt < 4; ++kt)
#pragma unroll
          for (int q = 0; q < 4; ++q) {
            const float4 a = *reinterpret_cast<const float4*>(Vl + j * SB_VL_LD + kt * 32 + 8 * q + 4 * h);
            oh = mfma32(a.x, sc[kt][q * 4 + 0], oh);
            oh = mfma32(a.y, sc[kt][q * 4 + 1], oh);
            oh = mfma32(a.z, sc[kt][q * 4 + 2], oh);
            oh = mfma32(a.w, sc[kt][q * 4 + 3], oh);
          }
      }
      const float inv = 1.0f / run_sum;
#pragma unroll
      for (int r = 0; r < 16; ++r) att[hd][r] = oh[r] * inv;
    }
  } else {
    f32x16 qh[4], kh[4], vh[4];
    acc_zero(qh); acc_zero(kh); acc_zero(vh);
    PTS_LAYER(4, 64)(ring, qh, [&](int s) { return g[s / 16][s % 16]; });
    PTS_LAYER(4, 64)(ring, kh, [&](int s) { return g[s / 16][s % 16]; });
    PTS_LAYER(4, 64)(ring, vh, [&](int s) { return g[s / 16][s % 16]; });
    if (PHASE == 1) {
#pragma unroll
      for (int t = 0; t < 4; ++t)
#pragma unroll
        for (int q = 0; q < 4; ++q) {
          hand[(t * 4 + q) * 64] = make_float4(g[t][q * 4], g[t][q * 4 + 1], g[t][q * 4 + 2], g[t][q * 4 + 3]);
          hand[(16 + t * 4 + q) * 64] = make_float4(qh[t][q * 4], qh[t][q * 4 + 1], qh[t][q * 4 + 2], qh[t][q * 4 + 3]);
          hand[(32 + t * 4 + q) * 64] = make_float4(kh[t][q * 4], kh[t][q * 4 + 1], kh[t][q * 4 + 2], kh[t][q * 4 + 3]);
          hand[(48 + t * 4 + q) * 64] = make_float4(vh[t][q * 4], vh[t][q * 4 + 1], vh[t][q * 4 + 2], vh[t][q * 4 + 3]);
        }
      return;
    }
    const int wave0 = wave - kt_self;
    DYN_PHASE(2);
    auto split8 = [&](const float (&v)[8], u32x4v& hi, u32x4v& mid) {
#pragma unroll
      for (int p2 = 0; p2 < 4; ++p2) {
        unsigned h_, m_, l_;
        split3_pair(v[2 * p2], v[2 * p2 + 1], h_, m_, l_);
        hi[p2] = h_; mid[p2] = m_;
      }
    };
    u32x4v* Kimg = reinterpret_cast<u32x4v*>(Kl);
#pragma unroll
    for (int hd = 0; hd < 4; ++hd) {
      lds_barrier();
#pragma unroll
      for (int m = 0; m < 2; ++m) {
        float kv[8];
#pragma unroll
        for (int e = 0; e < 8; ++e) kv[e] = kh[hd][8 * m + e];
        u32x4v khi, kmid;
        split8(kv, khi, kmid);
        Kimg[((wave * 2 + m) * 2 + 0) * 64 + lane] = khi;
        Kimg[((wave * 2 + m) * 2 + 1) * 64 + lane] = kmid;
      }
#pragma unroll
      for (int r = 0; r < 16; ++r) Vl[dyn_fi(r, h) * SB_VL_LD + wave * 32 + j] = vh[hd][r];
      u32x4v qhi[2], qmid[2];
#pragma unroll
      for (int m = 0; m < 2; ++m) {
        float qv[8];
#pragma unroll
        for (int e = 0; e < 8; ++e) qv[e] = qh[hd][8 * m + e] * inv_temp;
        split8(qv, qhi[m], qmid[m]);
      }
      lds_barrier();
      f32x16 sc[4];
      acc_zero(sc);
#pragma unroll
      for (int kt = 0; kt < 4; ++kt)
        if (kt < TPR) {
#pragma unroll
          for (int m = 0; m < 2; ++m) {
            const u32x4v ahi = Kimg[(((wave0 + kt) * 2 + m) * 2 + 0) * 64 + lane], amid = Kimg[(((wave0 + kt) * 2 + m) * 2 + 1) * 64 + lane];
            sc[kt] = mfma_bf16(amid, qhi[m], sc[kt]);
            sc[kt] = mfma_bf16(ahi, qmid[m], sc[kt]);
            sc[kt] = mfma_bf16(ahi, qhi[m], sc[kt]);
          }
        }
      float mx = -3.0e38f;
#pragma unroll
      for (int kt = 0; kt < 4; ++kt)
        if (kt < TPR) {
#pragma unroll
          for (int r = 0; r < 16; ++r) {
            const bool key_ok = kt * 32 + dyn_fi(r, h) < p.S;
            float v = q_ok ? sc[kt][r] : -1e9f;
            v = key_ok ? v : -3.0e38f;
            sc[kt][r] = v;
            mx = fmaxf(mx, v);
          }
        }
      mx = fmaxf(mx, __shfl_xor(mx, 32));
      float sum = 0.f;
#pragma unroll
      for (int kt = 0; kt < 4; ++kt)
        if (kt < TPR) {
#pragma unroll
          for (int r = 0; r < 16; ++r) {
            const float e = sc[kt][r] > -1.0e38f ? __expf(sc[kt][r] - mx) : 0.f;
            sc[kt][r] = e;
            sum += e;
          }
        }
      sum += __shfl_xor(sum, 32);
      const float inv = 1.0f / sum;
      f32x16 oh;
#pragma unroll
      for (int r = 0; r < 16; ++r) oh[r] = 0.f;
#pragma unroll
      for (int kt = 0; kt < 4; ++kt)
        if (kt < TPR) {
#pragma unroll
          for (int m = 0; m < 2; ++m) {
            const float* vrow = Vl + j * SB_VL_LD + (wave0 + kt) * 32 + 16 * m + 4 * h;
            const float4 v0 = *reinterpret_cast<const float4*>(vrow), v1 = *reinterpret_cast<const float4*>(vrow + 8);
            const float vv[8] = {v0.x, v0.y, v0.z, v0.w, v1.x, v1.y, v1.z, v1.w};
            float pv[8];
#pragma unroll
            for (int e = 0; e < 8; ++e) pv[e] = sc[kt][8 * m + e] * inv;
            u32x4v ahi, amid, phi, pmid;
            split8(vv, ahi, amid);
            split8(pv, phi, pmid);
            oh = mfma_bf16(amid, phi, oh);
            oh = mfma_bf16(ahi, pmid, oh);
            oh = mfma_bf16(ahi, phi, oh);
          }
        }
      att[hd] = oh;
    }
  }
  {
    f32x16 o[4];
    acc_zero(o);
    DYN_PHASE(3);
    PTS_LAYER(4, 64)(ring, o, [&](int s) { return att[s / 16][s % 16]; });
    float s1 = 0.f;
#pragma unroll
    for (int t = 0; t < 4; ++t)
#pragma unroll
      for (int r = 0; r < 16; ++r) {
        o[t][r] += g[t][r];
        s1 += o[t][r];
      }
    s1 += __shfl_xor(s1, 32);
    const float mu = s1 * (1.0f / 128.0f);
    float s2 = 0.f;
#pragma unroll
    for (int t = 0; t < 4; ++t)
#pragma unroll
      for (int r = 0; r < 16; ++r) {
        const float d = o[t][r] - mu;
        s2 += d * d;
      }
    s2 += __shfl_xor(s2, 32);
    const float rstd = 1.0f / sqrtf(s2 * (1.0f / 128.0f) + 1e-6f);
    const float* gam = ctab + h * 64;
    const float* bet = ctab + 128 + h * 64;
#pragma unroll
    for (int t = 0; t < 4; ++t)
#pragma unroll
      for (int r = 0; r < 16; ++r) g[t][r] = (o[t][r] - mu) * rstd * gam[t * 16 + r] + bet[t * 16 + r];
  }
  DYN_PHASE(4);
  float pf[SB_GIN_RECS];
  if (PERSIST) {
    bool gv;
    const float* nsrc = reinterpret_cast<const float*>(gin_src(more ? wgi + gridDim.x : wgi, gv));
#pragma unroll
    for (int i = 0; i < SB_GIN_RECS; ++i) pf[i] = (more && gv) ? nsrc[i * 256] : 0.f;
  }
  if (!DYN) {
    f32x16 a[4];
    acc_zero(a);
    PTS_LAYER(4, 65)(ring, a, [&](int s) { return s < 64 ? g[s / 16][s % 16] : one_h0; });
    acc_elu_s(a);
    float sigma = row_dot<4>(a, ctab + 256) + ctab[384];
    if (nvalid < 1.0f) sigma = -1e9f;
    if (valid && h == 0) p.raw[point * 4 + 3] = sigma;
    acc_zero(a);
    PTS_LAYER(4, 65)(ring, a, [&](int s) { return s < 64 ? g[s / 16][s % 16] : one_h0; });
    if (valid) {
      float4* dst = reinterpret_cast<float4*>(p.ws + p.o.off_hg) + tile * SB_HG_RECS * 64 + lane;
#pragma unroll
      for (int t = 0; t < 4; ++t)
#pragma unroll
        for (int q = 0; q < 4; ++q) dst[(t * 4 + q) * 64] = make_float4(a[t][q * 4], a[t][q * 4 + 1], a[t][q * 4 + 2], a[t][q * 4 + 3]);
    }
  } else {
    f32x16 g2[4];
    {
      float pe[17];
      float c3[3] = {0.f, 0.f, 0.f};
      if (valid) { c3[0] = p.pts[point * 3]; c3[1] = p.pts[point * 3 + 1]; c3[2] = p.pts[point * 3 + 2]; }
#pragma unroll
      for (int c = 0; c < 3; ++c) octave_embed<5>(c3[c], h, pe + c * 5);
      pe[15] = h == 0 ? c3[0] : c3[1];
      pe[16] = h == 0 ? c3[2] : 1.0f;
      f32x16 a8[8];
      acc_zero(a8);
      PTS_LAYER(8, 81)(ring, a8, [&](int s) { return s < 64 ? g[s / 16][s % 16] : pe[s - 64]; });
      acc_zero(g2);
      PTS_LAYER(4, 129)(ring, g2, [&](int s) { return s < 128 ? elu_s(a8[s / 16][s % 16]) : one_h0; });
    }
    f32x16 a[4];
    acc_zero(a);
    PTS_LAYER(4, 65)(ring, a, [&](int s) {
      if (s >= 64) return one_h0;
      const float r = elu1(g2[s / 16][s % 16]);
      g2[s / 16][s % 16] = r;
      return r;
    });
    acc_elu_s(a);
    float sigma = row_dot<4>(a, ctab + 256) + ctab[384] - p.shift;
    if (nvalid < 1.0f) sigma = -1e9f;
    float pd[14];
    {
      float d3[3] = {0.f, 0.f, 1.f};
      if (valid) unit3(p.ray_d[ray * 3], p.ray_d[ray * 3 + 1], p.ray_d[ray * 3 + 2], d3[0], d3[1], d3[2]);
#pragma unroll
      for (int c = 0; c < 3; ++c) octave_embed<4>(d3[c], h, pd + c * 4);
      pd[12] = h == 0 ? d3[0] : d3[1];
      pd[13] = h == 0 ? d3[2] : 1.0f;
    }
    acc_zero(a);
    PTS_LAYER(4, 78)(ring, a, [&](int s) { return s < 64 ? g2[s / 16][s % 16] : pd[s - 64]; });
    f32x16 b2[2];
    acc_zero(b2);
    PTS_LAYER(2, 65)(ring, b2, [&](int s) { return s < 64 ? elu_s(a[s / 16][s % 16]) : one_h0; });
    acc_elu_s(b2);
    float rgb[3];
#pragma unroll
    for (int c = 0; c < 3; ++c) {
      rgb[c] = sigmoid1(row_dot<2>(b2, ctab + 400 + c * 64) + ctab[385 + c]);
      if (nvalid == 0.f) rgb[c] = 0.f;
    }
    if (valid && h == 0) reinterpret_cast<float4*>(p.raw)[point] = make_float4(rgb[0], rgb[1], rgb[2], sigma);
  }
  DYN_PHASE(20);
#if DYN_POINTS_DUO
  if (PERSIST) {
    float sink = nvalid;
#if defined(__AMDGCN__)
    asm volatile("" : "+v"(sink));
#endif
#pragma unroll
    for (int i = 0; i < SB_GIN_RECS; ++i) sink += pf[i];
#if defined(__AMDGCN__)
    asm volatile("" ::"v"(sink));
#endif
    ring3_next_pass(ring);
  }
#endif
  wgi += gridDim.x;
  } while (PERSIST && wgi < n_wg);
}

#define DYN_BLEND_THREADS 256
template <int VSEG, int THREADS>
__device__ __forceinline__ void static_blend_body(StaticArgs p) {
  constexpr int PHASE_KID = 2;
  (void)PHASE_KID;
  DYN_PHASE(0);
  float* lds = reinterpret_cast<float*>(dyn_smem);
  float* ctab = lds + NET_CHUNK;
  const int tid = threadIdx.x, lane = tid & 63, j = lane & 31, h = lane >> 5, wave = tid >> 6;
  for (int i = tid; i < SC_CT; i += THREADS) ctab[i] = p.blob[ST_OFF_CTC + i];
  NetRing ring;
  net_ring_init_1(ring, p.blob + ST_OFF_C, SC_CHUNKS, lds, THREADS);
  DYN_PHASE_RING_KID(ring, 2);

  const int V = p.V;
  const long tile = (long)blockIdx.x * (THREADS / 64) + wave;
  const bool tile_ok = tile < p.n_tiles_a;
  const DenseRows dr = dense_rows(V, p.PT, ctab + SC_CT);
  const int p_local = VSEG == 0 ? dr.p_local : j / (VSEG == 0 ? 1 : VSEG);
  const int view = VSEG == 0 ? dr.view : (j & (VSEG - 1));
  const long point = VSEG == 0 ? (long)blockIdx.x * p.PT + p_local : tile * p.PT + p_local;
  const bool valid = (VSEG == 0 ? p_local < p.PT : view < V) && (point < p.n_pts);
  const long pv = valid ? point * V + view : 0;

  float msk = valid ? p.mask[pv] : 0.f;
  const float4 rd = valid ? reinterpret_cast<const float4*>(p.ray_diff)[pv] : make_float4(0.f, 0.f, 0.f, 0.f);
  const float4 vrec = tile_ok ? reinterpret_cast<const float4*>(p.ws + p.o.off_vis)[tile * 32 + j] : make_float4(0.f, 0.f, 0.f, 0.f);
  const float vis2 = vrec.x;
  const float rgb_in[3] = {valid ? vrec.y : 0.f, valid ? vrec.z : 0.f, valid ? vrec.w : 0.f};
  if (p.mask_rgb && !((rgb_in[0] + rgb_in[1]) + rgb_in[2] > 1e-3f)) msk = 0.f;
  f32x16 a[4];
  {
    f32x16 x[4];
    const float4* xw = reinterpret_cast<const float4*>(p.ws + p.o.off_x) + (tile_ok ? tile : 0) * 16 * 64 + lane;
    const float4* hg = reinterpret_cast<const float4*>(p.ws + p.o.off_hg) + (valid ? point_rec(p, point, h, SB_HG_RECS) : 0);
#pragma unroll
    for (int t = 0; t < 4; ++t)
#pragma unroll
      for (int q = 0; q < 4; ++q) {
        const float4 v = tile_ok ? nt_load4<8>(xw + (t * 4 + q) * 64) : make_float4(0.f, 0.f, 0.f, 0.f);
        x[t][q * 4] = v.x; x[t][q * 4 + 1] = v.y; x[t][q * 4 + 2] = v.z; x[t][q * 4 + 3] = v.w;
        const float4 b = valid ? hg[(t * 4 + q) * 64] : make_float4(0.f, 0.f, 0.f, 0.f);
        a[t][q * 4] = b.x; a[t][q * 4 + 1] = b.y; a[t][q * 4 + 2] = b.z; a[t][q * 4 + 3] = b.w;
      }
    const float extra[3] = {h == 0 ? vis2 : rd.x, h == 0 ? rd.y : rd.z, h == 0 ? rd.w : 0.f};
    net_layer<4, SC_L11_STEPS>(ring, a, [&](int s) { return s < 64 ? x[s / 16][s % 16] : extra[s - 64]; });
  }
  f32x16 b2[2];
  acc_init_bias<2>(b2, ctab + 80);
  net_layer<2, 64>(ring, b2, [&](int s) { return elu_s(a[s / 16][s % 16]); });
  acc_elu_s(b2);
  float logit = row_dot<2>(b2, ctab) + ctab[64];
  if (msk == 0.f) logit = -1e9f;
  if (VSEG == 0 ? p_local >= p.PT : view >= V) logit = -3.0e38f;
  const float mx = views_max<VSEG>(dr, logit);
  const float e = (VSEG == 0 && p_local >= p.PT) ? 0.f : __expf(logit - mx);
  const float bw = e / views_sum<VSEG>(dr, e);
#pragma unroll
  for (int c = 0; c < 3; ++c) {
    const float v = views_sum<VSEG>(dr, rgb_in[c] * bw);
    if (valid && (VSEG == 0 ? dr.rw == dr.base : view == 0) && h == 0) p.raw[point * 4 + c] = v;
  }
  DYN_PHASE(20);
}
#define SC_L11_PAIRS (((SC_L11_STEPS + 7) / 8) * 4)
#define SC_L12_PAIRS ((64 / 8) * 2)
#define SC_WS_FLOATS ((SC_L11_PAIRS + SC_L12_PAIRS) * B6_PAIR_FLOATS)
#ifndef DYN_BLEND_WS_THREADS
#define DYN_BLEND_WS_THREADS 512
#endif
#if DYN_BLEND_WS
__device__ __forceinline__ long n_units_of(const StaticArgs& p, bool rag, int vseg, int nw) {
  return rag ? p.rg_wg[0] : (vseg == 0 ? (p.n_tiles_a + nw - 1) / nw : p.n_tiles_a);
}
template <int VSEG, int THREADS, bool RAG = false>
__device__ __forceinline__ void static_blend_ws_body(StaticArgs p) {
  float* lds = reinterpret_cast<float*>(dyn_smem);
  float* ctab = lds + SC_WS_FLOATS;
  const int tid = threadIdx.x, lane = tid & 63, j = lane & 31, h = lane >> 5, wave = tid >> 6;
  for (int i = tid; i < SC_CT; i += THREADS) ctab[i] = p.blob[ST_OFF_CTC + i];
  {
    constexpr int CP = B6_CHUNK_PAIRS, L11_CH = net_layer_chunks(4, SC_L11_STEPS);
    const float4* src = reinterpret_cast<const float4*>(p.blob + ST_OFF_C);
    float4* dst = reinterpret_cast<float4*>(lds);
    for (int i = tid; i < SC_WS_FLOATS / 4; i += THREADS) {
      const int pair = i / (B6_PAIR_FLOATS / 4), within = i - pair * (B6_PAIR_FLOATS / 4);
      const int sp = pair < SC_L11_PAIRS ? pair : L11_CH * CP + (pair - SC_L11_PAIRS);
      dst[i] = src[(long)sp * (B6_PAIR_FLOATS / 4) + within];
    }
  }
  __syncthreads();
  const float* w11 = lds;
  const float* w12 = lds + SC_L11_PAIRS * B6_PAIR_FLOATS;
  const int V = p.V;
  constexpr int NW = THREADS / 64;
  DenseRows dr = dense_rows(V, p.PT, ctab + SC_CT, 0);
#ifndef DYN_BLEND_PREFETCH
#define DYN_BLEND_PREFETCH 1
#endif
  f32x16 x[4];
  auto tile_of = [&](long u_) { return VSEG == 0 ? u_ * NW + wave : u_; };
  auto load_x = [&](long u_, int t) DYN_INLINE_LAMBDA {
    const long tl = tile_of(u_);
    const bool ok = u_ < n_units_of(p, RAG, VSEG, NW) && tl < p.n_tiles_a;
    const float4* xw = reinterpret_cast<const float4*>(p.ws + p.o.off_x) + (ok ? tl : 0) * 16 * 64 + lane;
#pragma unroll
    for (int q = 0; q < 4; ++q) {
      const float4 v = ok ? nt_load4<8>(xw + (t * 4 + q) * 64) : make_float4(0.f, 0.f, 0.f, 0.f);
      x[t][q * 4] = v.x; x[t][q * 4 + 1] = v.y; x[t][q * 4 + 2] = v.z; x[t][q * 4 + 3] = v.w;
    }
  };
  const long n_units = n_units_of(p, RAG, VSEG, NW);
  const long first = VSEG == 0 ? blockIdx.x : (long)blockIdx.x * NW + wave, step = VSEG == 0 ? gridDim.x : (long)gridDim.x * NW;
  if (DYN_BLEND_PREFETCH) {
#pragma unroll
    for (int t = 0; t < 4; ++t) load_x(first, t);
  }
  RaggedHead head_next = {0, 0, 0, 0};
  if (RAG && first < n_units) head_next = ragged_head(p.rg_rowtab, p.rg_ptab, first, dr.rw);
  for (long u = first; u < n_units; u += step) {
    if (RAG) {
      const RaggedHead head = head_next;
      if (u + step < n_units) head_next = ragged_head(p.rg_rowtab, p.rg_ptab, u + step, dr.rw);
      dr = ragged_rows(V, p.rg_rowtab, p.rg_ptab, u, ctab + SC_CT, nullptr, &head);
    } else if (VSEG == 0) {
      dr.point0 = u * p.PT;
    }
    const int PT = RAG ? dr.PTW : p.PT;
    const int p_local = VSEG == 0 ? dr.p_local : j / (VSEG == 0 ? 1 : VSEG);
    const int view = VSEG == 0 ? dr.view : (j & (VSEG - 1));
    const long tile = VSEG == 0 ? u * NW + wave : u;
    const bool tile_ok = tile < p.n_tiles_a;
    const long point = VSEG == 0 ? dr.point0 + p_local : tile * PT + p_local;
    const bool valid = (VSEG == 0 ? p_local < PT : view < V) && (point < p.n_pts);
    const long pv = valid ? point * V + view : 0;
    float msk = valid ? p.mask[pv] : 0.f;
    const float4 rd = valid ? reinterpret_cast<const float4*>(p.ray_diff)[pv] : make_float4(0.f, 0.f, 0.f, 0.f);
    const float4 vrec = tile_ok ? reinterpret_cast<const float4*>(p.ws + p.o.off_vis)[tile * 32 + j] : make_float4(0.f, 0.f, 0.f, 0.f);
    const float vis2 = vrec.x;
    const float rgb_in[3] = {valid ? vrec.y : 0.f, valid ? vrec.z : 0.f, valid ? vrec.w : 0.f};
    if (p.mask_rgb && !((rgb_in[0] + rgb_in[1]) + rgb_in[2] > 1e-3f)) msk = 0.f;
    f32x16 a[4];
    {
      const float4* hg = reinterpret_cast<const float4*>(p.ws + p.o.off_hg) + (valid ? point_rec(p, point, h, SB_HG_RECS) : 0);
#pragma unroll
      for (int t = 0; t < 4; ++t) {
        if (!DYN_BLEND_PREFETCH) load_x(u, t);
#pragma unroll
        for (int q = 0; q < 4; ++q) {
          const float4 b = valid ? hg[(t * 4 + q) * 64] : make_float4(0.f, 0.f, 0.f, 0.f);
          a[t][q * 4] = b.x; a[t][q * 4 + 1] = b.y; a[t][q * 4 + 2] = b.z; a[t][q * 4 + 3] = b.w;
        }
      }
      const float extra[3] = {h == 0 ? vis2 : rd.x, h == 0 ? rd.y : rd.z, h == 0 ? rd.w : 0.f};
      mlp_layer_b6_lds<4, SC_L11_STEPS>(w11, a, [&](int s) { return s < 64 ? x[s / 16][s % 16] : extra[s - 64]; });
    }
    f32x16 b2[2];
    acc_init_bias<2>(b2, ctab + 80);
    mlp_layer_b6_lds<2, 64>(w12, b2, [&](int s) {
      const float r = elu_s(a[s / 16][s % 16]);
      if (DYN_BLEND_PREFETCH && (s & 15) == 15) load_x(u + step, s / 16);
      return r;
    });
    acc_elu_s(b2);
    float logit = row_dot<2>(b2, ctab) + ctab[64];
    if (msk == 0.f) logit = -1e9f;
    if (VSEG == 0 ? p_local >= PT : view >= V) logit = -3.0e38f;
    const float mx = views_max<VSEG>(dr, logit);
    const float e = (VSEG == 0 && p_local >= PT) ? 0.f : __expf(logit - mx);
    const float bw = e / views_sum<VSEG>(dr, e);
    const bool writer = valid && (VSEG == 0 ? dr.rw == dr.base : view == 0) && h == 0;
    const bool all_masked = RAG && writer && p.ws[p.o.off_nvalid + point] == 0.f;
#pragma unroll
    for (int c = 0; c < 3; ++c) {
      float v = views_sum<VSEG>(dr, rgb_in[c] * bw);
      if (all_masked) {
        const float wv = 1.0f / (float)V;
        v = 0.f;
        for (int k = 0; k < V; ++k) v += p.rgb_feat[(point * V + k) * 35 + c] * wv;
      }
      if (writer) p.raw[point * 4 + c] = v;
    }
  }
}
template <int VSEG>
__global__ void __launch_bounds__(DYN_BLEND_WS_THREADS, 1) k_static_blend_ws(StaticArgs p) { static_blend_ws_body<VSEG, DYN_BLEND_WS_THREADS>(p); }
template <bool RAG>
__global__ void __launch_bounds__(DYN_VIEW_THREADS, 1) k_static_blend_dense_ws(StaticArgs p) { static_blend_ws_body<0, DYN_VIEW_THREADS, RAG>(p); }
#endif

template <int VSEG>
__global__ void __launch_bounds__(DYN_BLEND_THREADS, 3) k_static_blend(StaticArgs p) { static_blend_body<VSEG, DYN_BLEND_THREADS>(p); }
__global__ void __launch_bounds__(DYN_VIEW_THREADS, 1) k_static_blend_dense(StaticArgs p) { static_blend_body<0, DYN_VIEW_THREADS>(p); }


static int ragged_plan(StaticArgs& a, const float* s_abs, hipStream_t stream) {
  unsigned* bits = reinterpret_cast<unsigned*>(a.ws + a.o.off_bits);
  float* emin = a.ws + a.o.off_emin;
  int* seg_cnt = reinterpret_cast<int*>(a.ws + a.o.off_segcnt);
  int* seg_start = reinterpret_cast<int*>(a.ws + a.o.off_segstart);
  int* wg = reinterpret_cast<int*>(a.ws + a.o.off_wgstart);
  unsigned short* rowtab = reinterpret_cast<unsigned short*>(a.ws + a.o.off_rowtab);
  int* ptab = reinterpret_cast<int*>(a.ws + a.o.off_ptab);
  a.rg_bits = bits; a.rg_emin = emin; a.rg_wg = wg; a.rg_rowtab = rowtab; a.rg_ptab = ptab;
  DYN_REQUIRE(a.n_pts < (1L << 31), "ragged plan: R * S must stay below 2^31 points");
  DYN_LAUNCH(DYN_K_STATIC_PLAN, "k_ragged_points", k_ragged_points, dim3(dyn_cdiv(a.n_pts, 256)), dim3(256), (size_t)256 * a.V * 5, stream, a.n_pts, a.V, a.mask,
             reinterpret_cast<const float4*>(a.ray_diff), s_abs, bits, emin);
  DYN_LAUNCH(DYN_K_STATIC_PLAN, "k_ragged_segments", k_ragged_segments, dim3((unsigned)a.o.n_seg), dim3(256), (RAG_SEG + 4 + 256) * sizeof(int) + RAG_SEG * sizeof(unsigned short), stream, a.n_pts, a.o.n_seg, bits, seg_cnt, seg_start);
  DYN_LAUNCH(DYN_K_STATIC_PLAN, "k_ragged_scatter", k_ragged_scatter, dim3(1), dim3(1024), 1028 * sizeof(int), stream, a.n_pts, a.o.n_seg, seg_cnt, seg_start, wg);
  DYN_LAUNCH(DYN_K_STATIC_PLAN, "k_ragged_tables", k_ragged_tables, dim3((unsigned)a.o.n_wg_max), dim3(64), 0, stream, bits, wg, rowtab, ptab);
  return 0;
}

extern "C" int dyn_static_net(const DynStaticNetParams* q, void* stream_) {
  DYN_REQUIRE(q, "dyn_static_net: null params");
  DYN_REQUIRE(q->R > 0 && q->S > 0 && q->V > 0, "dyn_static_net: empty problem");
  DYN_REQUIRE(q->V <= 32, "dyn_static_net: at most 32 source views");
  DYN_REQUIRE(q->S <= DYN_MAX_SAMPLES, "dyn_static_net: at most %d samples per ray", DYN_MAX_SAMPLES);
  DYN_REQUIRE(q->blob && q->ray_o && q->ray_d && q->pts && q->rgb_feat && q->ray_diff && q->mask && q->centers && q->raw && q->workspace,
              "dyn_static_net: null pointer");
  hipStream_t stream = (hipStream_t)stream_;
  StaticArgs a;
  a.R = q->R; a.S = q->S; a.V = q->V;
  a.o = static_ws(q->R, q->S, q->V);
  DYN_REQUIRE(q->workspace_bytes >= a.o.total * sizeof(float), "dyn_static_net: workspace too small (%zu < %zu bytes)", q->workspace_bytes,
              a.o.total * sizeof(float));
  a.PT = a.o.PT; a.TPR = a.o.TPR;
  a.anti_alias = q->anti_alias_pooling; a.mask_rgb = q->mask_rgb;
  a.n_pts = a.o.n_pts; a.n_tiles_a = a.o.n_tiles_a; a.n_tiles_b = a.o.n_tiles_b;
  a.blob = q->blob; a.pts = q->pts; a.rgb_feat = q->rgb_feat; a.ray_diff = q->ray_diff; a.mask = q->mask; a.centers = q->centers;
  a.raw = q->raw; a.ws = (float*)q->workspace;
  a.rg_bits = nullptr; a.rg_emin = nullptr; a.rg_wg = nullptr; a.rg_rowtab = nullptr; a.rg_ptab = nullptr;

  DYN_LAUNCH(DYN_K_STATIC_REF, "k_static_ref_feat", k_static_ref_feat, dim3(dyn_cdiv(q->R, REF_RAYS)), dim3(256), REF_RAYS * 66 * sizeof(float), stream, q->ray_o,
             q->ray_d, q->blob + ST_OFF_REF, q->R, a.ws + a.o.off_ref);
  const dim3 grid_a(dyn_cdiv(a.n_tiles_a, DYN_VIEW_THREADS / 64)), grid_b(dyn_cdiv(a.n_tiles_b, 4)), blk(DYN_NET_THREADS), blk_v(DYN_VIEW_THREADS);
  const size_t lds_a = (2 * NET_CHUNK + SA_CT + POOL_FLOATS(SA_NX) + RES_FLOATS) * sizeof(float);
  const size_t lds_b = (PTS_RING_SLOTS * PTS_CHUNK + SB_CT + SB_KL_FLOATS + SB_VL_FLOATS) * sizeof(float);
  const size_t lds_c = (NET_CHUNK + SC_CT) * sizeof(float);
  const dim3 grid_c(dyn_cdiv(a.n_tiles_a, DYN_BLEND_THREADS / 64)), blk_c(DYN_BLEND_THREADS);
  const size_t lds_rag = (DENSE_EXTRA + RAG_PTAB) * sizeof(float);
  if (a.o.ragged) {
    const int rc = ragged_plan(a, a.anti_alias ? a.blob + ST_OFF_CTA + 258 : nullptr, stream);
    if (rc != 0) return rc;
  }
  if (a.o.ragged && a.V == 11) DYN_LAUNCH(DYN_K_STATIC_VIEWS, "k_static_views", (k_static_views<0, 11, true>), grid_a, blk_v, lds_a + lds_rag, stream, a);
  else if (a.o.ragged) DYN_LAUNCH(DYN_K_STATIC_VIEWS, "k_static_views", (k_static_views<0, 0, true>), grid_a, blk_v, lds_a + lds_rag, stream, a);
  else if (a.o.dense && a.V == 11) DYN_LAUNCH(DYN_K_STATIC_VIEWS, "k_static_views", (k_static_views<0, 11>), grid_a, blk_v, lds_a + DENSE_EXTRA * sizeof(float), stream, a);
  else if (a.o.dense) DYN_LAUNCH(DYN_K_STATIC_VIEWS, "k_static_views", k_static_views<0>, grid_a, blk_v, lds_a + DENSE_EXTRA * sizeof(float), stream, a);
  else if (q->V <= 4) DYN_LAUNCH(DYN_K_STATIC_VIEWS, "k_static_views", k_static_views<4>, grid_a, blk_v, lds_a, stream, a);
  else if (q->V <= 8) DYN_LAUNCH(DYN_K_STATIC_VIEWS, "k_static_views", k_static_views<8>, grid_a, blk_v, lds_a, stream, a);
  else if (q->V <= 16) DYN_LAUNCH(DYN_K_STATIC_VIEWS, "k_static_views", k_static_views<16>, grid_a, blk_v, lds_a, stream, a);
  else DYN_LAUNCH(DYN_K_STATIC_VIEWS, "k_static_views", k_static_views<32>, grid_a, blk_v, lds_a, stream, a);
  if (a.TPR <= 4) {
    DYN_LAUNCH(DYN_K_STATIC_POINTS, "k_static_points", (k_net_points<false, 0>), points_grid(grid_b), blk, lds_b, stream, a);
  } else {
    DYN_LAUNCH(DYN_K_STATIC_POINTS_QKV, "k_static_points_qkv", (k_net_points<false, 1>), grid_b, blk, lds_b, stream, a);
    DYN_LAUNCH(DYN_K_STATIC_POINTS, "k_static_points", (k_net_points<false, 2>), grid_b, blk, lds_b, stream, a);
  }
#if DYN_BLEND_WS
  static const int blend_stream = getenv("DYN_BLEND_STREAM") != nullptr;
  if (!blend_stream) {
    const size_t lds_w = (SC_WS_FLOATS + SC_CT + DENSE_SCALARS + RAG_PTAB) * sizeof(float);
    const unsigned n_cu = (unsigned)dyn_cu_count();
    if (a.o.dense) {
      const unsigned nb = (unsigned)dyn_cdiv(a.n_tiles_a, DYN_VIEW_THREADS / 64);
      if (a.o.ragged) DYN_LAUNCH(DYN_K_STATIC_BLEND, "k_static_blend", k_static_blend_dense_ws<true>, dim3(nb < n_cu ? nb : n_cu), blk_v, lds_w, stream, a);
      else DYN_LAUNCH(DYN_K_STATIC_BLEND, "k_static_blend", k_static_blend_dense_ws<false>, dim3(nb < n_cu ? nb : n_cu), blk_v, lds_w, stream, a);
    } else {
      const unsigned nb = (unsigned)dyn_cdiv(a.n_tiles_a, DYN_BLEND_WS_THREADS / 64);
      const dim3 gw(nb < n_cu ? nb : n_cu), bw_(DYN_BLEND_WS_THREADS);
      if (q->V <= 4) DYN_LAUNCH(DYN_K_STATIC_BLEND, "k_static_blend", k_static_blend_ws<4>, gw, bw_, lds_w, stream, a);
      else if (q->V <= 8) DYN_LAUNCH(DYN_K_STATIC_BLEND, "k_static_blend", k_static_blend_ws<8>, gw, bw_, lds_w, stream, a);
      else if (q->V <= 16) DYN_LAUNCH(DYN_K_STATIC_BLEND, "k_static_blend", k_static_blend_ws<16>, gw, bw_, lds_w, stream, a);
      else DYN_LAUNCH(DYN_K_STATIC_BLEND, "k_static_blend", k_static_blend_ws<32>, gw, bw_, lds_w, stream, a);
    }
    return 0;
  }
#endif
  if (a.o.dense) DYN_LAUNCH(DYN_K_STATIC_BLEND, "k_static_blend", k_static_blend_dense, grid_a, blk_v, lds_c + DENSE_SCALARS * sizeof(float), stream, a);
  else if (q->V <= 4) DYN_LAUNCH(DYN_K_STATIC_BLEND, "k_static_blend", k_static_blend<4>, grid_c, blk_c, lds_c, stream, a);
  else if (q->V <= 8) DYN_LAUNCH(DYN_K_STATIC_BLEND, "k_static_blend", k_static_blend<8>, grid_c, blk_c, lds_c, stream, a);
  else if (q->V <= 16) DYN_LAUNCH(DYN_K_STATIC_BLEND, "k_static_blend", k_static_blend<16>, grid_c, blk_c, lds_c, stream, a);
  else DYN_LAUNCH(DYN_K_STATIC_BLEND, "k_static_blend", k_static_blend<32>, grid_c, blk_c, lds_c, stream, a);
  return 0;
}

extern "C" size_t dyn_dynamic_net_blob_floats(void) { return DY_BLOB_FLOATS; }

extern "C" int dyn_dynamic_net_pack(const float* const* T, int F, float* blob, size_t blob_floats) {
  DYN_REQUIRE(T && blob, "dyn_dynamic_net_pack: null pointer");
  DYN_REQUIRE(F == 32, "dyn_dynamic_net_pack: the kernels are specialised for 32 feature channels");
  DYN_REQUIRE(blob_floats >= DY_BLOB_FLOATS, "dyn_dynamic_net_pack: blob too small");
  for (int i = 0; i < DT_NUM_TENSORS; ++i) DYN_REQUIRE(T[i] != nullptr, "dyn_dynamic_net_pack: tensor %d is NULL", i);
  std::vector<float> o;
  g_pack_range_error = false;
  o.reserve(DY_BLOB_FLOATS);
  {
    const float *W = T[DT_BASE0_W], *b = T[DT_BASE0_B];
    pack_net_layer(o, 8, DA_L3P_STEPS, scaled([=](int t, int i, int s, int h) -> float {
      const int c = da_c35(s % DA_NX, h);
      return c < 0 ? 0.f : W[(32 * t + i) * 105 + (s / DA_NX) * 35 + c];
    }, DYN_ELU_PRE));
    pack_net_layer(o, 8, DA_L3V_STEPS, scaled([=](int t, int i, int s, int h) -> float {
      const int n = 32 * t + i;
      if (s == DA_NX) return h == 0 ? b[n] : 0.f;
      const int c = da_c35(s, h);
      return c < 0 ? 0.f : W[n * 105 + 70 + c];
    }, DYN_ELU_PRE));
  }
  pack_net_layer(o, 4, SA_L4_STEPS, scaled(chained(T[DT_BASE2_W], nullptr, 128, 256, 256), DYN_ELU_POST));
  pack_net_layer(o, 4, SA_L5_STEPS, scaled(chained(T[DT_VIS0_W], nullptr, 128, 128, 128), DYN_ELU_PRE));
  pack_net_layer(o, 4, SA_L5_STEPS, scaled(chained(T[DT_VIS2_W], nullptr, 128, 128, 128), DYN_ELU_POST));
  pack_net_layer(o, 4, SA_L5_STEPS, scaled(chained(T[DT_VISB0_W], nullptr, 128, 128, 128), DYN_ELU_PRE));
  DYN_REQUIRE(o.size() == DY_OFF_B, "dynamic pack: A stream size mismatch");
#if DYN_POINTS_DUO
  g_pack_chunk_pairs = PTS_CP;
#endif
  {
    const float *W = T[DT_GEO0_W], *b = T[DT_GEO0_B];
    pack_net_layer(o, 8, 129, scaled([=](int t, int i, int s, int h) -> float {
      const int n = 32 * t + i;
      if (s < 128) return W[n * 257 + (s < 64 ? 0 : 128) + chain_feature(s % 64, h)];
      return h == 0 ? W[n * 257 + 256] : b[n];
    }, DYN_ELU_PRE));
  }
  pack_net_layer(o, 4, 129, scaled_wb(chained(T[DT_GEO2_W], T[DT_GEO2_B], 128, 256, 256), 128, DYN_ELU_POST, 1.0));
  pack_net_layer(o, 4, 64, chained(T[DT_WQ], nullptr, 128, 128, 128));
  pack_net_layer(o, 4, 64, chained(T[DT_WK], nullptr, 128, 128, 128));
  pack_net_layer(o, 4, 64, chained(T[DT_WV], nullptr, 128, 128, 128));
  pack_net_layer(o, 4, 64, chained(T[DT_FC], nullptr, 128, 128, 128));
  {
    const float *W = T[DT_REFPTS0_W], *b = T[DT_REFPTS0_B];
    pack_net_layer(o, 8, 81, scaled([=](int t, int i, int s, int h) -> float {
      const int n = 32 * t + i;
      if (s < 64) return W[n * 161 + chain_feature(s, h)];
      if (s < 79) { const int c = (s - 64) / 5, f = (s - 64) % 5; return W[n * 161 + 128 + 3 + (h * 5 + f) * 3 + c]; }
      if (s == 79) return W[n * 161 + 128 + h];
      return h == 0 ? W[n * 161 + 128 + 2] : b[n];
    }, DYN_ELU_PRE));
  }
  pack_net_layer(o, 4, 129, scaled_wb(chained(T[DT_REFPTS2_W], T[DT_REFPTS2_B], 128, 256, 256), 128, DYN_ELU_POST, 1.0));
  pack_net_layer(o, 4, 65, scaled(chained(T[DT_OG0_W], T[DT_OG0_B], 128, 128, 128), DYN_ELU_PRE));
  {
    const float *W = T[DT_RGB0_W], *b = T[DT_RGB0_B];
    pack_net_layer(o, 4, 78, scaled([=](int t, int i, int s, int h) -> float {
      const int n = 32 * t + i;
      if (s < 64) return W[n * 155 + chain_feature(s, h)];
      if (s < 76) { const int c = (s - 64) / 4, f = (s - 64) % 4; return W[n * 155 + 128 + 3 + (h * 4 + f) * 3 + c]; }
      if (s == 76) return W[n * 155 + 128 + h];
      return h == 0 ? W[n * 155 + 128 + 2] : b[n];
    }, DYN_ELU_PRE));
  }
  pack_net_layer(o, 2, 65, scaled_wb(chained(T[DT_RGB2_W], T[DT_RGB2_B], 64, 128, 128), 64, DYN_ELU_POST * DYN_ELU_PRE, DYN_ELU_PRE));
  g_pack_chunk_pairs = B6_CHUNK_PAIRS;
  DYN_REQUIRE(o.size() == DY_OFF_CTA, "dynamic pack: B stream size mismatch");
  pack_rowtab(o, T[DT_VIS2_W] + 128 * 128, 128, DYN_ELU_POST);
  pack_rowtab(o, T[DT_VISB2_W], 128, DYN_ELU_POST);
  o.push_back(T[DT_VIS2_B][128]);
  o.push_back(T[DT_VISB2_B][0]);
  o.resize(DY_OFF_CTA + 272, 0.f);
  pack_rowtab(o, T[DT_BASE2_B], 128);
  pack_rowtab(o, T[DT_VIS0_B], 128, DYN_ELU_PRE);
  pack_rowtab(o, T[DT_VIS2_B], 128);
  pack_rowtab(o, T[DT_VISB0_B], 128, DYN_ELU_PRE);
  o.resize(DY_OFF_CTB, 0.f);
  pack_rowtab(o, T[DT_LN_G], 128);
  pack_rowtab(o, T[DT_LN_B], 128);
  pack_rowtab(o, T[DT_OG2_W], 128, DYN_ELU_POST);
  o.push_back(T[DT_OG2_B][0]);
  for (int c = 0; c < 3; ++c) o.push_back(T[DT_RGB4_B][c]);
  o.resize(DY_OFF_CTB + 400, 0.f);
  for (int c = 0; c < 3; ++c) pack_rowtab(o, T[DT_RGB4_W] + c * 64, 64, DYN_ELU_POST);
  o.resize(DY_OFF_POSENC, 0.f);
  for (int pos = 0; pos < DYN_MAX_SAMPLES; ++pos)
    for (int h = 0; h < 2; ++h)
      for (int k = 0; k < 64; ++k) {
        const int f = chain_feature(k, h);
        const double ang = (double)pos / pow(10000.0, 2.0 * (f / 2) / 128.0);
        o.push_back((float)((f % 2 == 0) ? sin(ang) : cos(ang)));
      }
  for (int i = 0; i < 256 * 21; ++i) o.push_back(T[DT_RAYDIR0_W][i]);
  for (int i = 0; i < 256; ++i) o.push_back(T[DT_RAYDIR0_B][i]);
  for (int i = 0; i < 35 * 256; ++i) o.push_back(T[DT_RAYDIR2_W][i]);
  for (int i = 0; i < 35; ++i) o.push_back(T[DT_RAYDIR2_B][i]);
  o.resize(DY_BLOB_FLOATS, 0.f);
  DYN_REQUIRE(!g_pack_range_error, "dyn_dynamic_net_pack: a weight is outside the half-float range of the split engine (|w| >= 65504 or not finite)");
  for (size_t i = 0; i < DY_BLOB_FLOATS; ++i) blob[i] = o[i];
  return 0;
}

extern "C" size_t dyn_dynamic_net_workspace_bytes(int R, int S, int V) {
  if (R <= 0 || S <= 0 || V <= 0 || V > 32) return 0;
  return static_ws(R, S, V, true).total * sizeof(float);
}

__global__ void __launch_bounds__(256) k_dynamic_time_feat(const float* __restrict__ Wt, const float* __restrict__ time, float* __restrict__ out) {
  float* hid = reinterpret_cast<float*>(dyn_smem);
  const int tid = threadIdx.x;
  const float t = time[0];
  float pe[21];
  pe[0] = t;
  for (int f = 0; f < 10; ++f) {
    const float a = (float)(1 << f) * t;
    pe[1 + f] = cosf(a);
    pe[11 + f] = sinf(a);
  }
  {
    const float* w = Wt + tid * 21;
    float acc = Wt[256 * 21 + tid];
    for (int k = 0; k < 21; ++k) acc = fmaf(w[k], pe[k], acc);
    hid[tid] = acc > 0.f ? acc : expm1f(acc);
  }
  __syncthreads();
  if (tid < 35) {
    const float* w = Wt + 256 * 21 + 256 + tid * 256;
    float acc = Wt[256 * 21 + 256 + 35 * 256 + tid];
    for (int k = 0; k < 256; ++k) acc = fmaf(w[k], hid[k], acc);
    out[tid] = acc > 0.f ? acc : expm1f(acc);
  } else if (tid < 36) {
    out[tid] = 0.f;
  }
}

template <int VSEG, bool RAG = false>
__global__ void __launch_bounds__(DYN_VIEW_THREADS, 2) k_dynamic_views(StaticArgs p) {
  static_assert(!RAG || VSEG == 0, "ragged rows are a dense-rows flavour");
  if (RAG && (int)blockIdx.x >= p.rg_wg[0]) return;
  float* lds = reinterpret_cast<float*>(dyn_smem);
  float* ctab = lds + 2 * NET_CHUNK;
  const int tid = threadIdx.x, lane = tid & 63, j = lane & 31, h = lane >> 5, wave = tid >> 6;
  for (int i = tid; i < SA_CT; i += DYN_VIEW_THREADS) ctab[i] = p.blob[DY_OFF_CTA + i];
  NetRing ring;
  constexpr int LDS_FLOATS = 2 * NET_CHUNK + SA_CT + POOL_FLOATS(SA_NX) + RES_FLOATS + (VSEG == 0 ? DENSE_EXTRA : 0);
  net_ring_init(ring, p.blob + DY_OFF_A, DA_CHUNKS, lds, 0, (VSEG >= 8 || VSEG == 0) ? net_layer_chunks(8, DA_L3P_STEPS) : 0, DYN_VIEW_THREADS);

  const int V = p.V;
  const long tile = (long)blockIdx.x * (DYN_VIEW_THREADS / 64) + wave;
  const DenseRows dr = RAG ? ragged_rows(V, p.rg_rowtab, p.rg_ptab, blockIdx.x, lds + LDS_FLOATS - DENSE_SCALARS, reinterpret_cast<int*>(lds + LDS_FLOATS))
                           : dense_rows(V, p.PT, lds + LDS_FLOATS - DENSE_SCALARS);
  const int PT = RAG ? dr.PTW : p.PT;
  const int p_local = VSEG == 0 ? dr.p_local : j / (VSEG == 0 ? 1 : VSEG);
  const int view = VSEG == 0 ? dr.view : (j & (VSEG - 1));
  const long point = VSEG == 0 ? dr.point0 + p_local : tile * PT + p_local;
  const bool valid = (VSEG == 0 ? p_local < PT : view < V) && (point < p.n_pts);
  const int seg_base = 0;
  const long pv = valid ? point * V + view : 0;
  const float msk = valid ? p.mask[pv] : 0.f;
  const float* tf = p.ws + p.o.off_ref;
  float xin[DA_NX];
#pragma unroll
  for (int q = 0; q < DA_NX; ++q) {
    const int ch = h == 0 ? q : 18 + q;
    xin[q] = (valid && ch < 35) ? nt_load1<2>(p.rgb_feat + pv * 35 + ch) + tf[ch] : 0.f;
  }
  const float wraw = views_sum<VSEG>(dr, msk);
  const float wgt = msk / (wraw + 1e-8f);
  f32x16 a1[8];
  base_fc0<VSEG, DA_NX>(ring, p.blob + DY_OFF_A, xin, wgt, V, view, p_local, ctab + SA_CT, a1, &dr, wraw / (wraw + 1e-8f));
  views_tail<VSEG, false>(ring, a1, p, ctab, wgt, msk, tile, point, valid, view, seg_base, &dr, lds);
}

extern "C" int dyn_dynamic_net(const DynDynamicNetParams* q, void* stream_) {
  DYN_REQUIRE(q, "dyn_dynamic_net: null params");
  DYN_REQUIRE(q->R > 0 && q->S > 0 && q->V > 0, "dyn_dynamic_net: empty problem");
  DYN_REQUIRE(q->V <= 32, "dyn_dynamic_net: at most 32 source views");
  DYN_REQUIRE(q->S <= DYN_MAX_SAMPLES, "dyn_dynamic_net: at most %d samples per ray", DYN_MAX_SAMPLES);
  DYN_REQUIRE(q->blob && q->ray_d && q->pts && q->rgb_feat && q->mask && q->time && q->raw && q->workspace, "dyn_dynamic_net: null pointer");
  hipStream_t stream = (hipStream_t)stream_;
  StaticArgs a;
  a.R = q->R; a.S = q->S; a.V = q->V;
  a.o = static_ws(q->R, q->S, q->V, true);
  DYN_REQUIRE(q->workspace_bytes >= a.o.total * sizeof(float), "dyn_dynamic_net: workspace too small (%zu < %zu bytes)", q->workspace_bytes,
              a.o.total * sizeof(float));
  a.PT = a.o.PT; a.TPR = a.o.TPR;
  a.anti_alias = 0; a.mask_rgb = 0;
  a.n_pts = a.o.n_pts; a.n_tiles_a = a.o.n_tiles_a; a.n_tiles_b = a.o.n_tiles_b;
  a.shift = q->shift;
  a.blob = q->blob; a.ray_d = q->ray_d; a.pts = q->pts; a.rgb_feat = q->rgb_feat; a.ray_diff = nullptr; a.mask = q->mask; a.centers = nullptr;
  a.raw = q->raw; a.ws = (float*)q->workspace;
  a.rg_bits = nullptr; a.rg_emin = nullptr; a.rg_wg = nullptr; a.rg_rowtab = nullptr; a.rg_ptab = nullptr;
  DYN_LAUNCH(DYN_K_DYNAMIC_TIME, "k_dynamic_time_feat", k_dynamic_time_feat, dim3(1), dim3(256), 256 * sizeof(float), stream,
             q->blob + DY_OFF_TIME, q->time, a.ws + a.o.off_ref);
  const dim3 grid_a(dyn_cdiv(a.n_tiles_a, DYN_VIEW_THREADS / 64)), grid_b(dyn_cdiv(a.n_tiles_b, 4)), blk(DYN_NET_THREADS), blk_v(DYN_VIEW_THREADS);
  const size_t lds_a = (2 * NET_CHUNK + SA_CT + POOL_FLOATS(SA_NX) + RES_FLOATS) * sizeof(float);
  const size_t lds_b = (PTS_RING_SLOTS * PTS_CHUNK + DB_CT + SB_KL_FLOATS + SB_VL_FLOATS) * sizeof(float);
  if (a.o.ragged) {
    const int rc = ragged_plan(a, nullptr, stream);
    if (rc != 0) return rc;
    DYN_LAUNCH(DYN_K_DYNAMIC_VIEWS, "k_dynamic_views", (k_dynamic_views<0, true>), grid_a, blk_v, lds_a + (DENSE_EXTRA + RAG_PTAB) * sizeof(float), stream, a);
  } else if (a.o.dense) DYN_LAUNCH(DYN_K_DYNAMIC_VIEWS, "k_dynamic_views", k_dynamic_views<0>, grid_a, blk_v, lds_a + DENSE_EXTRA * sizeof(float), stream, a);
  else if (q->V <= 4) DYN_LAUNCH(DYN_K_DYNAMIC_VIEWS, "k_dynamic_views", k_dynamic_views<4>, grid_a, blk_v, lds_a, stream, a);
  else if (q->V <= 8) DYN_LAUNCH(DYN_K_DYNAMIC_VIEWS, "k_dynamic_views", k_dynamic_views<8>, grid_a, blk_v, lds_a, stream, a);
  else if (q->V <= 16) DYN_LAUNCH(DYN_K_DYNAMIC_VIEWS, "k_dynamic_views", k_dynamic_views<16>, grid_a, blk_v, lds_a, stream, a);
  else DYN_LAUNCH(DYN_K_DYNAMIC_VIEWS, "k_dynamic_views", k_dynamic_views<32>, grid_a, blk_v, lds_a, stream, a);
  if (a.TPR <= 4) {
    DYN_LAUNCH(DYN_K_DYNAMIC_POINTS, "k_dynamic_points", (k_net_points<true, 0>), points_grid(grid_b), blk, lds_b, stream, a);
  } else {
    DYN_LAUNCH(DYN_K_DYNAMIC_POINTS_QKV, "k_dynamic_points_qkv", (k_net_points<true, 1>), grid_b, blk, lds_b, stream, a);
    DYN_LAUNCH(DYN_K_DYNAMIC_POINTS, "k_dynamic_points", (k_net_points<true, 2>), grid_b, blk, lds_b, stream, a);
  }
  return 0;
}

enum { MT_L0_W, MT_L0_B, MT_L1_W, MT_L1_B, MT_L2_W, MT_L2_B, MT_L3_W, MT_L3_B, MT_L4_W, MT_L4_B, MT_L5_W, MT_L5_B, MT_L6_W, MT_L6_B, MT_L7_W,
       MT_L7_B, MT_COEFF_W, MT_COEFF_B, MT_NUM_TENSORS };
#define MO_PE_STEPS 66
constexpr int MO_CHUNKS = net_layer_chunks(8, MO_PE_STEPS + 1) + 4 * net_layer_chunks(8, 129) + net_layer_chunks(8, MO_PE_STEPS + 129) +
                          2 * net_layer_chunks(8, 129) + net_layer_chunks(1, 129);
constexpr size_t MO_OFF_FREQ = (size_t)MO_CHUNKS * NET_CHUNK;
constexpr size_t MO_BLOB_FLOATS = MO_OFF_FREQ + 16;

extern "C" size_t dyn_motion_mlp_blob_floats(void) { return MO_BLOB_FLOATS; }

static int mo_pe_col(int s, int h) {
  if (s < 64) { const int c = s / 16, f = s % 16; return 4 + (h * 16 + f) * 4 + c; }
  return (s - 64) * 2 + h;
}

extern "C" int dyn_motion_mlp_pack(const float* const* T, int num_basis, float* blob, size_t blob_floats) {
  DYN_REQUIRE(T && blob, "dyn_motion_mlp_pack: null pointer");
  DYN_REQUIRE(num_basis >= 1 && 3 * num_basis <= 32, "dyn_motion_mlp_pack: 3 * num_basis must be at most 32");
  DYN_REQUIRE(blob_floats >= MO_BLOB_FLOATS, "dyn_motion_mlp_pack: blob too small");
  for (int i = 0; i < MT_NUM_TENSORS; ++i) DYN_REQUIRE(T[i] != nullptr, "dyn_motion_mlp_pack: tensor %d is NULL", i);
  std::vector<float> o;
  g_pack_range_error = false;
  o.reserve(MO_BLOB_FLOATS);
  {
    const float *W = T[MT_L0_W], *b = T[MT_L0_B];
    pack_net_layer(o, 8, MO_PE_STEPS + 1, [=](int t, int i, int s, int h) -> float {
      const int n = 32 * t + i;
      if (s < MO_PE_STEPS) return W[n * 132 + mo_pe_col(s, h)];
      return h == 0 ? b[n] : 0.f;
    });
  }
  for (int l = 1; l <= 4; ++l) pack_net_layer(o, 8, 129, chained(T[MT_L0_W + 2 * l], T[MT_L0_B + 2 * l], 256, 256, 256));
  {
    const float *W = T[MT_L5_W], *b = T[MT_L5_B];
    pack_net_layer(o, 8, MO_PE_STEPS + 129, [=](int t, int i, int s, int h) -> float {
      const int n = 32 * t + i;
      if (s < MO_PE_STEPS) return W[n * 388 + mo_pe_col(s, h)];
      const int s2 = s - MO_PE_STEPS;
      if (s2 < 128) return W[n * 388 + 132 + chain_feature(s2, h)];
      return h == 0 ? b[n] : 0.f;
    });
  }
  pack_net_layer(o, 8, 129, chained(T[MT_L6_W], T[MT_L6_B], 256, 256, 256));
  pack_net_layer(o, 8, 129, chained(T[MT_L7_W], T[MT_L7_B], 256, 256, 256));
  pack_net_layer(o, 1, 129, chained(T[MT_COEFF_W], T[MT_COEFF_B], 3 * num_basis, 256, 256));
  DYN_REQUIRE(o.size() == MO_OFF_FREQ, "motion pack: stream size mismatch");
  {
    const float step = (17.0f - 1.0f) / 15.0f;
    for (int i = 0; i < 16; ++i) o.push_back(i < 8 ? 1.0f + (float)i * step : 17.0f - (float)(15 - i) * step);
  }
  DYN_REQUIRE(!g_pack_range_error, "dyn_motion_mlp_pack: a weight is outside the half-float range of the split engine (|w| >= 65504 or not finite)");
  for (size_t i = 0; i < MO_BLOB_FLOATS; ++i) blob[i] = o[i];
  return 0;
}

__device__ __attribute__((noinline)) float sin_or_cos_huge(float x, int want_sin) { return want_sin ? sinf(x) : cosf(x); }

__device__ __forceinline__ void motion_embed(const float (&c4)[4], const float* __restrict__ freq, int h, float (&pe)[MO_PE_STEPS]) {
#pragma unroll
  for (int c = 0; c < 4; ++c)
#pragma unroll
    for (int f = 0; f < 16; ++f) {
      float sn, cs;
      const float arg = freq[f] * c4[c];
      sincos_small(arg, sn, cs);
      float v = h == 0 ? cs : sn;
      if (__builtin_expect(fabsf(arg) > 1.0e6f, 0)) v = sin_or_cos_huge(arg, h);
      pe[c * 16 + f] = v;
    }
  pe[64] = h == 0 ? c4[0] : c4[1];
  pe[65] = h == 0 ? c4[2] : c4[3];
}

#ifndef DYN_MOTION_DUO
#define DYN_MOTION_DUO 1
#endif
#if DYN_MOTION_DUO
typedef WeightRing3 MotionRing;
#define MOTION_RING_SLOTS B6D_SLOTS
#define motion_ring_init(R, stream, total, lds) ring3_init(R, stream, total, lds, DYN_NET_THREADS)
#define motion_layer mlp_layer_b6_duo
#else
typedef NetRing MotionRing;
#define MOTION_RING_SLOTS 2
#define motion_ring_init(R, stream, total, lds) net_ring_init_t(R, stream, total, lds, DYN_NET_THREADS)
#define motion_layer net_layer
#endif

__global__ void __launch_bounds__(256) k_motion_zero_tail(long R, int S, int n_zero_last, int n_out, float* __restrict__ coeff) {
  const long i = (long)blockIdx.x * blockDim.x + threadIdx.x;
  const long per_ray = (long)n_zero_last * n_out;
  if (i >= R * per_ray) return;
  const long ray = i / per_ray;
  coeff[(ray * S + (S - n_zero_last)) * n_out + (i - ray * per_ray)] = 0.f;
}

__global__ void __launch_bounds__(DYN_NET_THREADS, 1)
k_motion_mlp(const float* __restrict__ blob, const float* __restrict__ pts, const float* __restrict__ time, long n_kept, int S, int n_zero_last,
             int n_out, float inv_div, float* __restrict__ coeff) {
  DYN_CLAIM_REGISTER_FILE();
  float* lds = reinterpret_cast<float*>(dyn_smem);
  const int tid = threadIdx.x, lane = tid & 63, j = lane & 31, h = lane >> 5, wave = tid >> 6;
  MotionRing ring;
  motion_ring_init(ring, blob, MO_CHUNKS, lds);
  const long row = ((long)blockIdx.x * 4 + wave) * 32 + j;
  const bool valid = row < n_kept;
  const int Sk = S - n_zero_last;
  const long ray = (valid ? row : 0) / Sk;
  const long point = ray * S + ((valid ? row : 0) - ray * Sk);
  float c4[4] = {0.f, 0.f, 0.f, time[0]};
  if (valid) { c4[0] = pts[point * 3]; c4[1] = pts[point * 3 + 1]; c4[2] = pts[point * 3 + 2]; }
  const float* freq = blob + MO_OFF_FREQ;
  const float one_h0 = h == 0 ? 1.0f : 0.0f;
  f32x16 a[8], b[8];
  float pe[MO_PE_STEPS];
  motion_embed(c4, freq, h, pe);
  acc_zero(a);
  motion_layer<8, MO_PE_STEPS + 1>(ring, a, [&](int s) { return s < MO_PE_STEPS ? pe[s] : one_h0; });
  acc_zero(b);
  motion_layer<8, 129>(ring, b, [&](int s) { return s < 128 ? relu1(a[s / 16][s % 16]) : one_h0; });
  acc_zero(a);
  motion_layer<8, 129>(ring, a, [&](int s) { return s < 128 ? relu1(b[s / 16][s % 16]) : one_h0; });
  acc_zero(b);
  motion_layer<8, 129>(ring, b, [&](int s) { return s < 128 ? relu1(a[s / 16][s % 16]) : one_h0; });
  acc_zero(a);
  motion_layer<8, 129>(ring, a, [&](int s) { return s < 128 ? relu1(b[s / 16][s % 16]) : one_h0; });
  acc_zero(b);
  motion_layer<8, MO_PE_STEPS + 129>(ring, b, [&](int s) {
    if (s < MO_PE_STEPS) return pe[s];
    return s - MO_PE_STEPS < 128 ? relu1(a[(s - MO_PE_STEPS) / 16][(s - MO_PE_STEPS) % 16]) : one_h0;
  });
  acc_zero(a);
  motion_layer<8, 129>(ring, a, [&](int s) { return s < 128 ? relu1(b[s / 16][s % 16]) : one_h0; });
  acc_zero(b);
  motion_layer<8, 129>(ring, b, [&](int s) { return s < 128 ? relu1(a[s / 16][s % 16]) : one_h0; });
  f32x16 c1[1];
  acc_zero(c1);
  motion_layer<1, 129>(ring, c1, [&](int s) { return s < 128 ? relu1(b[s / 16][s % 16]) : one_h0; });
  if (valid) {
#pragma unroll
    for (int r = 0; r < 16; ++r) {
      const int f = dyn_fi(r, h);
      if (f < n_out) coeff[point * n_out + f] = c1[0][r] * inv_div;
    }
  }
}

extern "C" int dyn_motion_mlp(const float* blob, const float* pts, const float* time, int R, int S, int num_basis, int n_zero_last,
                              float sf_mag_div, float* coeff, void* stream) {
  DYN_REQUIRE(blob && pts && time && coeff, "dyn_motion_mlp: null pointer");
  DYN_REQUIRE(R > 0 && S > 0 && num_basis >= 1 && 3 * num_basis <= 32 && n_zero_last >= 0 && sf_mag_div != 0.f, "dyn_motion_mlp: bad argument");
  const int nz = n_zero_last < S ? n_zero_last : S;
  const long n_kept = (long)R * (S - nz);
  if (n_kept > 0)
    DYN_LAUNCH(DYN_K_MOTION_MLP, "k_motion_mlp", k_motion_mlp, dim3(dyn_cdiv(n_kept, 128)), dim3(DYN_NET_THREADS), MOTION_RING_SLOTS * NET_CHUNK * sizeof(float),
               (hipStream_t)stream, blob, pts, time, n_kept, S, nz, 3 * num_basis, 1.0f / sf_mag_div, coeff);
  if (nz > 0)
    DYN_LAUNCH(DYN_K_MOTION_TAIL, "k_motion_zero_tail", k_motion_zero_tail, dim3(dyn_cdiv((long)R * nz * 3 * num_basis, 256)), dim3(256), 0, (hipStream_t)stream, (long)R, S, nz,
               3 * num_basis, coeff);
  return 0;
}

extern "C" int dyn_mlp_split_terms(void) {
  return DYN_SPLIT_TERMS;
}
extern "C" int dyn_mlp_split_kind(void) {
#if DYN_SPLIT_F16
  return 2;
#else
  return 1;
#endif
}

__global__ void __launch_bounds__(DYN_NET_THREADS, 2) k_selftest(const float* __restrict__ stream, const float* __restrict__ x, float* __restrict__ y,
                                                                  int rows) {
  float* lds = reinterpret_cast<float*>(dyn_smem);
  const int lane = threadIdx.x & 63, j = lane & 31, h = lane >> 5, wave = threadIdx.x >> 6;
  NetRing ring;
  net_ring_init_t(ring, stream, 2 * net_layer_chunks(2, 33), lds, DYN_NET_THREADS);
  const int row = (blockIdx.x * 4 + wave) * 32 + j;
  f32x16 in[2];
#pragma unroll
  for (int s = 0; s < 32; ++s) in[s / 16][s % 16] = row < rows ? x[row * 64 + 32 * (s / 16) + dyn_fi(s % 16, h)] : 0.f;
  const float one_h0 = h == 0 ? 1.0f : 0.0f;
#pragma unroll
  for (int rep = 0; rep < 2; ++rep) {
    f32x16 acc[2];
    acc_zero(acc);
    net_layer<2, 33>(ring, acc, [&](int s) { return s < 32 ? in[s / 16][s % 16] : one_h0; });
    acc_elu(acc);
    in[0] = acc[0];
    in[1] = acc[1];
  }
  if (row < rows)
#pragma unroll
    for (int s = 0; s < 32; ++s) y[row * 64 + 32 * (s / 16) + dyn_fi(s % 16, h)] = in[s / 16][s % 16];
}

extern "C" int dyn_mlp_selftest(const float* W, const float* b, const float* x, float* y, int rows, float* stream_buf, void* stream) {
  DYN_REQUIRE(W && b && x && y && stream_buf && rows > 0, "dyn_mlp_selftest: bad argument");
  std::vector<float> o;
  pack_net_layer(o, 2, 33, chained(W, b, 64, 64, 64));
  pack_net_layer(o, 2, 33, chained(W, b, 64, 64, 64));
  if (hipMemcpy(stream_buf, o.data(), o.size() * sizeof(float), hipMemcpyHostToDevice) != hipSuccess) {
    dyn_set_error("dyn_mlp_selftest: hipMemcpy failed");
    return DYN_E_LAUNCH;
  }
  DYN_LAUNCH(DYN_K_SELFTEST, "k_selftest", k_selftest, dim3(dyn_cdiv(rows, 128)), dim3(DYN_NET_THREADS), 2 * NET_CHUNK * sizeof(float),
             (hipStream_t)stream, stream_buf, x, y, rows);
  return 0;
}
```

Measured before the change: 1.532 million.

## Add 8-wave points kernel with head-interleaved QKV weight stream

Replaces the 4-wave points kernel with a new 512-thread, 8-wave variant (two blocks per CU) when the duo split engine is active and TPR<=4. It packs a second copy of the B weight stream with Q/K/V interleaved per head so attention can run per head, splits the first layer into parts to cut register pressure, and keeps accumulators in VGPRs instead of AGPRs. The unused persistent-grid and ring-wrap machinery is removed. This is meant to share each weight chunk across more waves and raise occupancy, at the cost of a larger weight blob and more LDS per block.

Measured after the change: 1.596 million, median of 6. 1.04x the previous value.

```diff
diff --git a/dynibar_amd/csrc/dyn_mlp.h b/dynibar_amd/csrc/dyn_mlp.h
--- a/dynibar_amd/csrc/dyn_mlp.h
+++ b/dynibar_amd/csrc/dyn_mlp.h
@@ -527,8 +527,6 @@
   int fill, issued;
   float* slot[B6D_SLOTS];
   unsigned lds_slot[B6D_SLOTS];
-  int wrap;
-  bool more;
 #ifdef DYN_PHASE_TIMING
   int kid;
 #endif
@@ -548,9 +546,8 @@
 __device__ __forceinline__ void ring3_piece(const WeightRing3& R, int chunk, int k) {
   const int per_wave = R.cf / R.waves;
   const int grp = k / 6, i = k % 6;
-  const int sc = chunk >= R.total ? chunk - R.total : chunk;
-  const float* g = R.glane + (long)sc * R.cf + grp * 1536;
-  const float* gu = R.gbase + (long)sc * R.cf + grp * 1536;
+  const float* g = R.glane + (long)chunk * R.cf + grp * 1536;
+  const float* gu = R.gbase + (long)chunk * R.cf + grp * 1536;
   const unsigned l = R.lds_slot[chunk % B6D_SLOTS] + (unsigned)(grp * 1536 * sizeof(float));
   float* le = R.slot[chunk % B6D_SLOTS] + (threadIdx.x >> 6) * per_wave + 512 + grp * 1536;
   if (i == 0) ring3_dma<-2048>(g, le, l, gu, R.lane_off);
@@ -591,8 +588,6 @@
   }
   R.fill = -1;
   R.issued = 0;
-  R.wrap = 0;
-  R.more = false;
   for (int j = 0; j < B6D_SLOTS; ++j) {
     R.slot[j] = lds + j * R.cf;
     R.lds_slot[j] = R.lds_wave + (unsigned)(j * R.cf * sizeof(float));
@@ -616,7 +611,6 @@
 #endif
 __device__ __forceinline__ void ring3_feed(WeightRing3& R, int half, int num, int den) {
   if (R.fill < 0) return;
-  if (R.fill >= R.total && !R.more) return;
   const int n = ring3_pieces(R), h0 = n / 2;
   int want = half == 0 ? (h0 * num + den - 1) / den : h0 + ((n - h0) * num + den - 1) / den;
   if (want > n) want = n;
@@ -625,24 +619,12 @@
 __device__ __forceinline__ void ring3_mid(WeightRing3& R) {
   DYN_PHASE_T0
   ring3_feed(R, 1, 1, 1);
-  if (R.next + 1 < R.total || R.wrap) ring3_barrier();
+  if (R.next + 1 < R.total) ring3_barrier();
   DYN_PHASE_WAIT(R, R.next);
-  R.fill = (R.next + 2 < R.total || R.wrap) ? R.next + 2 : -1;
+  R.fill = R.next + 2 < R.total ? R.next + 2 : -1;
   R.issued = 0;
 }
-__device__ __forceinline__ void ring3_leave(WeightRing3& R) {
-  if (R.wrap && R.next == R.total - 1) ring3_feed(R, 1, 1, 1);
-  ++R.next;
-}
-__device__ __forceinline__ void ring3_next_pass(WeightRing3& R) {
-  float* s0[B6D_SLOTS];
-  unsigned l0[B6D_SLOTS];
-  for (int j = 0; j < B6D_SLOTS; ++j) { s0[j] = R.slot[j]; l0[j] = R.lds_slot[j]; }
-  for (int j = 0; j < B6D_SLOTS; ++j) { R.slot[j] = s0[(R.total + j) % B6D_SLOTS]; R.lds_slot[j] = l0[(R.total + j) % B6D_SLOTS]; }
-  R.next = 0;
-  R.fill = -1;
-  R.issued = 0;
-}
+__device__ __forceinline__ void ring3_leave(WeightRing3& R) { ++R.next; }
 
 __device__ __forceinline__ float relu1(float v) {
 #if defined(__AMDGCN__)
@@ -664,18 +646,20 @@
 }
 #define DYN_INLINE_LAMBDA __attribute__((always_inline))
 
+template <bool ACC_AGPR = true>
 __device__ __forceinline__ f32x16 mfma_pinned(const u32x4v& a, u32x4v& b, f32x16 c) {
 #if defined(__AMDGCN__)
   asm volatile("" : "+v"(b));
   f32x16 d = mfma_bf16(a, b, c);
-  asm volatile("" : "+a"(d));
+  if constexpr (ACC_AGPR) asm volatile("" : "+a"(d));
+  else asm volatile("" : "+v"(d));
   return d;
 #else
   return mfma_bf16(a, b, c);
 #endif
 }
 
-template <int NT, int NSLOTS, int CP = B6_CHUNK_PAIRS, int AHEAD = B6D_AHEAD, class Feed>
+template <int NT, int NSLOTS, int CP = B6_CHUNK_PAIRS, int AHEAD = B6D_AHEAD, bool ACC_AGPR = true, class Feed>
 __device__ __forceinline__ void mlp_layer_b6_duo(WeightRing3& R, f32x16 (&acc)[NT], Feed&& feed) {
   constexpr int NG = (NSLOTS + 7) / 8;
   constexpr int NP = NG * NT;
@@ -797,37 +781,37 @@
     const B6A& a0 = q[P % QN];
     const B6A& a1 = q[(P + U - 1) % QN];
 #if DYN_SPLIT_TERMS == 6
-    acc[t0] = mfma_pinned(a0.lo, bh, acc[t0]);
-    if constexpr (U == 2) acc[t1] = mfma_pinned(a1.lo, bh, acc[t1]);
-    acc[t0] = mfma_pinned(a0.hi, bl, acc[t0]);
-    if constexpr (U == 2) acc[t1] = mfma_pinned(a1.hi, bl, acc[t1]);
-    acc[t0] = mfma_pinned(a0.mid, bm, acc[t0]);
-    if constexpr (U == 2) acc[t1] = mfma_pinned(a1.mid, bm, acc[t1]);
-#endif
-    acc[t0] = mfma_pinned(a0.mid, bh, acc[t0]);
+    acc[t0] = mfma_pinned<ACC_AGPR>(a0.lo, bh, acc[t0]);
+    if constexpr (U == 2) acc[t1] = mfma_pinned<ACC_AGPR>(a1.lo, bh, acc[t1]);
+    acc[t0] = mfma_pinned<ACC_AGPR>(a0.hi, bl, acc[t0]);
+    if constexpr (U == 2) acc[t1] = mfma_pinned<ACC_AGPR>(a1.hi, bl, acc[t1]);
+    acc[t0] = mfma_pinned<ACC_AGPR>(a0.mid, bm, acc[t0]);
+    if constexpr (U == 2) acc[t1] = mfma_pinned<ACC_AGPR>(a1.mid, bm, acc[t1]);
+#endif
+    acc[t0] = mfma_pinned<ACC_AGPR>(a0.mid, bh, acc[t0]);
     __builtin_amdgcn_sched_barrier(0);
     if constexpr (U == 2) {
       if constexpr (P + AHEAD + 1 < NP) q[(P + AHEAD + 1) % QN] = load(P + AHEAD + 1);
       gap(std::integral_constant<int, 1>{});
-      acc[t1] = mfma_pinned(a1.mid, bh, acc[t1]);
+      acc[t1] = mfma_pinned<ACC_AGPR>(a1.mid, bh, acc[t1]);
       __builtin_amdgcn_sched_barrier(0);
       gap(std::integral_constant<int, 2>{});
     }
-    acc[t0] = mfma_pinned(a0.hi, bm, acc[t0]);
+    acc[t0] = mfma_pinned<ACC_AGPR>(a0.hi, bm, acc[t0]);
     if constexpr (U == 2) {
       __builtin_amdgcn_sched_barrier(0);
       gap(std::integral_constant<int, 3>{});
       dma(std::integral_constant<int, 1>{});
-      acc[t1] = mfma_pinned(a1.hi, bm, acc[t1]);
+      acc[t1] = mfma_pinned<ACC_AGPR>(a1.hi, bm, acc[t1]);
       __builtin_amdgcn_sched_barrier(0);
       gap(std::integral_constant<int, 4>{});
     }
-    acc[t0] = mfma_pinned(a0.hi, bh, acc[t0]);
+    acc[t0] = mfma_pinned<ACC_AGPR>(a0.hi, bh, acc[t0]);
     if constexpr (U == 2) {
       __builtin_amdgcn_sched_barrier(0);
       gap(std::integral_constant<int, 5>{});
       dma(std::integral_constant<int, U>{});
-      acc[t1] = mfma_pinned(a1.hi, bh, acc[t1]);
+      acc[t1] = mfma_pinned<ACC_AGPR>(a1.hi, bh, acc[t1]);
     } else {
       dma(std::integral_constant<int, U>{});
     }
diff --git a/dynibar_amd/csrc/dyn_nets.hip b/dynibar_amd/csrc/dyn_nets.hip
--- a/dynibar_amd/csrc/dyn_nets.hip
+++ b/dynibar_amd/csrc/dyn_nets.hip
@@ -71,6 +71,14 @@
   return [=](int t, int i, int s, int h) -> float { return (float)((double)fn(t, i, s, h) * scale); };
 }
 
+void pack_qkv_by_head(std::vector<float>& out, const float* Wq, const float* Wk, const float* Wv) {
+  for (int hd = 0; hd < 4; ++hd) {
+    pack_net_layer(out, 2, 64, [=](int t, int i, int s, int h) -> float { return (t == 0 ? Wq : Wk)[(size_t)(32 * hd + i) * 128 + chain_feature(s, h)]; });
+    if (hd % 2 == 0)
+      pack_net_layer(out, 2, 64, [=](int t, int i, int s, int h) -> float { return Wv[(size_t)(32 * (hd + t) + i) * 128 + chain_feature(s, h)]; });
+  }
+}
+
 }
 
 enum {
@@ -93,9 +101,6 @@
                           net_layer_chunks(4, SA_L4_STEPS) + 3 * net_layer_chunks(4, SA_L5_STEPS);
 #ifndef DYN_POINTS_DUO
 #define DYN_POINTS_DUO (DYN_SPLIT_TERMS == 3 ? 1 : 0)
-#endif
-#ifndef DYN_POINTS_PERSIST
-#define DYN_POINTS_PERSIST 0
 #endif
 #if DYN_POINTS_DUO
 #define PTS_CP 16
@@ -126,7 +131,8 @@
 constexpr size_t ST_OFF_CTB = ST_OFF_CTA + SA_CT;
 constexpr size_t ST_OFF_CTC = ST_OFF_CTB + SB_CT;
 constexpr size_t ST_OFF_REF = ST_OFF_CTC + SC_CT;
-constexpr size_t ST_BLOB_FLOATS = ST_OFF_REF + 35 * 66 + 36;
+constexpr size_t ST_OFF_B8 = (ST_OFF_REF + 35 * 66 + 36 + 63) / 64 * 64;
+constexpr size_t ST_BLOB_FLOATS = ST_OFF_B8 + (DYN_POINTS_DUO ? (size_t)SB_CHUNKS * PTS_CHUNK : 0);
 
 enum {
   DT_RAYDIR0_W, DT_RAYDIR0_B, DT_RAYDIR2_W, DT_RAYDIR2_B, DT_BASE0_W, DT_BASE0_B, DT_BASE2_W, DT_BASE2_B, DT_VIS0_W, DT_VIS0_B, DT_VIS2_W,
@@ -148,7 +154,8 @@
 constexpr size_t DY_OFF_CTB = DY_OFF_CTA + SA_CT;
 constexpr size_t DY_OFF_POSENC = DY_OFF_CTB + DB_CT;
 constexpr size_t DY_OFF_TIME = DY_OFF_POSENC + 256 * 128;
-constexpr size_t DY_BLOB_FLOATS = DY_OFF_TIME + 256 * 21 + 256 + 35 * 256 + 36;
+constexpr size_t DY_OFF_B8 = (DY_OFF_TIME + 256 * 21 + 256 + 35 * 256 + 36 + 63) / 64 * 64;
+constexpr size_t DY_BLOB_FLOATS = DY_OFF_B8 + (DYN_POINTS_DUO ? (size_t)DB_CHUNKS * PTS_CHUNK : 0);
 __host__ __device__ constexpr int da_c35(int q, int h) { return h == 0 ? q : (q < 17 ? 18 + q : -1); }
 
 __host__ __device__ constexpr int sa_c70(int q, int h) {
@@ -216,6 +223,7 @@
   pack_net_layer(o, 4, SA_L5_STEPS, scaled(chained(T[ST_VIS2_W], nullptr, 128, 128, 128), DYN_ELU_POST));
   pack_net_layer(o, 4, SA_L5_STEPS, scaled(chained(T[ST_VISB0_W], nullptr, 128, 128, 128), DYN_ELU_PRE));
   DYN_REQUIRE(o.size() == ST_OFF_B, "static pack: A stream size mismatch");
+  const auto pack_b = [&](bool by_head) {
 #if DYN_POINTS_DUO
   g_pack_chunk_pairs = PTS_CP;
 #endif
@@ -228,13 +236,19 @@
     }, DYN_ELU_PRE));
   }
   pack_net_layer(o, 4, 129, scaled_wb(chained(T[ST_GEO2_W], T[ST_GEO2_B], 128, 256, 256), 128, DYN_ELU_POST, 1.0));
-  pack_net_layer(o, 4, 64, chained(T[ST_WQ], nullptr, 128, 128, 128));
-  pack_net_layer(o, 4, 64, chained(T[ST_WK], nullptr, 128, 128, 128));
-  pack_net_layer(o, 4, 64, chained(T[ST_WV], nullptr, 128, 128, 128));
+  if (by_head) {
+    pack_qkv_by_head(o, T[ST_WQ], T[ST_WK], T[ST_WV]);
+  } else {
+    pack_net_layer(o, 4, 64, chained(T[ST_WQ], nullptr, 128, 128, 128));
+    pack_net_layer(o, 4, 64, chained(T[ST_WK], nullptr, 128, 128, 128));
+    pack_net_layer(o, 4, 64, chained(T[ST_WV], nullptr, 128, 128, 128));
+  }
   pack_net_layer(o, 4, 64, chained(T[ST_FC], nullptr, 128, 128, 128));
   pack_net_layer(o, 4, 65, scaled(chained(T[ST_OG0_W], T[ST_OG0_B], 128, 128, 128), DYN_ELU_PRE));
   pack_net_layer(o, 4, 65, scaled(chained(T[ST_RGB0_W], T[ST_RGB0_B], 128, 128, 261), DYN_ELU_PRE));
   g_pack_chunk_pairs = B6_CHUNK_PAIRS;
+  };
+  pack_b(false);
   DYN_REQUIRE(o.size() == ST_OFF_C, "static pack: B stream size mismatch");
   {
     const float* W = T[ST_RGB0_W];
@@ -275,7 +289,11 @@
   o.resize(ST_OFF_REF, 0.f);
   for (int i = 0; i < 35 * 66; ++i) o.push_back(T[ST_REFFEAT_W][i]);
   for (int i = 0; i < 35; ++i) o.push_back(T[ST_REFFEAT_B][i]);
-  o.resize(ST_BLOB_FLOATS, 0.f);
+  o.resize(ST_OFF_B8, 0.f);
+#if DYN_POINTS_DUO
+  pack_b(true);
+#endif
+  DYN_REQUIRE(o.size() == ST_BLOB_FLOATS, "static pack: B8 stream size mismatch");
   DYN_REQUIRE(!g_pack_range_error, "dyn_static_net_pack: a weight is outside the half-float range of the split engine (|w| >= 65504 or not finite)");
   for (size_t i = 0; i < ST_BLOB_FLOATS; ++i) blob[i] = o[i];
   return 0;
@@ -1218,23 +1236,6 @@
   return n_cu[slot];
 }
 
-static dim3 points_grid(dim3 full) {
-#if DYN_POINTS_DUO && DYN_POINTS_PERSIST
-  static int n_cu[DYN_MAX_DEVICES] = {0};
-  int dev = 0;
-  (void)hipGetDevice(&dev);
-  const int slot = (dev >= 0 && dev < DYN_MAX_DEVICES) ? dev : 0;
-  if (n_cu[slot] == 0) {
-    hipDeviceProp_t prop;
-    n_cu[slot] = (hipGetDeviceProperties(&prop, dev) == hipSuccess && prop.multiProcessorCount > 0) ? prop.multiProcessorCount : 256;
-  }
-  static const int no_persist = getenv("DYN_POINTS_NO_PERSIST") != nullptr;
-  return (no_persist || full.x <= (unsigned)n_cu[slot]) ? full : dim3((unsigned)n_cu[slot]);
-#else
-  return full;
-#endif
-}
-
 template <bool DYN, int PHASE>
 __global__ void __launch_bounds__(DYN_NET_THREADS, 1) k_net_points(StaticArgs p) {
   constexpr int PHASE_KID = 1;
@@ -1258,24 +1259,7 @@
 
   const int TPR = p.TPR;
   const float one_h0 = h == 0 ? 1.0f : 0.0f;
-  constexpr bool PERSIST = DYN_POINTS_PERSIST && DYN_POINTS_DUO && PHASE == 0;
-  const long n_wg = (p.n_tiles_b + 3) / 4;
-  auto gin_src = [&](long wgi, bool& valid_) DYN_INLINE_LAMBDA {
-    const long tile_ = wgi * 4 + wave;
-    const long ray_ = tile_ / TPR;
-    valid_ = (ray_ < p.R) && ((int)(tile_ - ray_ * TPR) * 32 + j < p.S);
-    return reinterpret_cast<const float4*>(p.ws + p.o.off_gin) + (tile_ < p.n_tiles_b ? tile_ : 0) * SB_GIN_RECS * 64 + lane;
-  };
-#if DYN_POINTS_DUO
-  ring.wrap = PERSIST ? 1 : 0;
-#endif
-  long wgi = blockIdx.x;
-  do {
-  const bool more = PERSIST && wgi + gridDim.x < n_wg;
-#if DYN_POINTS_DUO
-  ring.more = more;
-#endif
-  const long tile = wgi * 4 + wave;
+  const long tile = (long)blockIdx.x * 4 + wave;
   const long ray = tile / TPR;
   const int kt_self = (int)(tile - ray * TPR);
   const int smp = kt_self * 32 + j;
@@ -1301,8 +1285,8 @@
     f32x16 a9[8];
     {
       float gin[129];
-      bool gv;
-      const float4* src = gin_src(wgi, gv);
+      const bool gv = valid;
+      const float4* src = reinterpret_cast<const float4*>(p.ws + p.o.off_gin) + (tile < p.n_tiles_b ? tile : 0) * SB_GIN_RECS * 64 + lane;
 #pragma unroll
       for (int i = 0; i < 32; ++i) {
         const float4 v = gv ? nt_load4<4>(src + i * 64) : make_float4(0.f, 0.f, 0.f, 0.f);
@@ -1567,13 +1551,6 @@
       for (int r = 0; r < 16; ++r) g[t][r] = (o[t][r] - mu) * rstd * gam[t * 16 + r] + bet[t * 16 + r];
   }
   DYN_PHASE(4);
-  float pf[SB_GIN_RECS];
-  if (PERSIST) {
-    bool gv;
-    const float* nsrc = reinterpret_cast<const float*>(gin_src(more ? wgi + gridDim.x : wgi, gv));
-#pragma unroll
-    for (int i = 0; i < SB_GIN_RECS; ++i) pf[i] = (more && gv) ? nsrc[i * 256] : 0.f;
-  }
   if (!DYN) {
     f32x16 a[4];
     acc_zero(a);
@@ -1642,23 +1619,319 @@
     if (valid && h == 0) reinterpret_cast<float4*>(p.raw)[point] = make_float4(rgb[0], rgb[1], rgb[2], sigma);
   }
   DYN_PHASE(20);
+}
+
 #if DYN_POINTS_DUO
-  if (PERSIST) {
-    float sink = nvalid;
+#define PTS8_LAYER(NT, NSLOTS) mlp_layer_b6_duo<NT, NSLOTS, PTS_CP, 2, false>
+#define SB8_VL_LD 260
+#define SB8_KV_FLOATS (32 * SB8_VL_LD)
+static_assert(SB8_KV_FLOATS >= 8 * 2 * 2 * 64 * 4, "the K image fits the shared region");
+static_assert(pts_layer_chunks(8, 129) == 3 * pts_layer_chunks(8, 32) + pts_layer_chunks(8, 33) && 32 % (8 * (PTS_CP / 8)) == 0 && pts_layer_chunks(8, 81) == pts_layer_chunks(8, 64) + pts_layer_chunks(8, 17),
+              "the two-part layers split at a chunk boundary");
+static_assert(4 * pts_layer_chunks(2, 64) + 2 * pts_layer_chunks(2, 64) == 3 * pts_layer_chunks(4, 64), "the head-interleaved stream is as long as the plain one");
+
+template <bool DYN, int MAXT>
+__global__ void __launch_bounds__(DYN_VIEW_THREADS, 2) k_net_points_w8(StaticArgs p) {
+  constexpr int PHASE_KID = 1;
+  (void)PHASE_KID;
+  DYN_PHASE(0);
+  constexpr int CT = DYN ? DB_CT : SB_CT;
+  float* lds = reinterpret_cast<float*>(dyn_smem);
+  float* ctab = lds + PTS_RING_SLOTS * PTS_CHUNK;
+  float* KV = ctab + CT;
+  const int tid = threadIdx.x, lane = tid & 63, j = lane & 31, h = lane >> 5, wave = tid >> 6;
+  for (int i = tid; i < CT; i += DYN_VIEW_THREADS) ctab[i] = p.blob[(DYN ? DY_OFF_CTB : ST_OFF_CTB) + i];
+  PtsRing ring;
+  ring3_init(ring, p.blob + (DYN ? DY_OFF_B8 : ST_OFF_B8), DYN ? DB_CHUNKS : SB_CHUNKS, lds, DYN_VIEW_THREADS, PTS_CP);
+  DYN_PHASE_RING_KID(ring, 1);
+  lds_barrier();
+
+  const int TPR = p.TPR;
+  const float one_h0 = h == 0 ? 1.0f : 0.0f;
 #if defined(__AMDGCN__)
-    asm volatile("" : "+v"(sink));
+  const int wave_u = __builtin_amdgcn_readfirstlane(wave);
+#else
+  const int wave_u = wave;
 #endif
-#pragma unroll
-    for (int i = 0; i < SB_GIN_RECS; ++i) sink += pf[i];
+  const long tile = (long)blockIdx.x * (DYN_VIEW_THREADS / 64) + wave_u;
+  const int tpr_shift = TPR >> 1;
+  const long ray = tile >> tpr_shift;
+  const int kt_self = (int)(tile & (TPR - 1));
+  const bool valid = (ray < p.R) && (kt_self * 32 + j < p.S);
+  bool q_ok, no_view, few_views;
+  {
+    const float nvalid = valid ? p.ws[p.o.off_nvalid + ray * p.S + kt_self * 32 + j] : 0.f;
+    q_ok = nvalid > 1.0f;
+    no_view = nvalid == 0.f;
+    few_views = nvalid < 1.0f;
+  }
+
+  f32x16 g[4];
+  {
+    f32x16 a9[8];
+    acc_zero(a9);
+    const float4* src = reinterpret_cast<const float4*>(p.ws + p.o.off_gin) + (tile < p.n_tiles_b ? tile : 0) * SB_GIN_RECS * 64 + lane;
+    dyn_static_for<3>([&](auto PART) DYN_INLINE_LAMBDA {
+      constexpr int part = decltype(PART)::value;
+      float gin[32];
+#pragma unroll
+      for (int i = 0; i < 8; ++i) {
+        const float4 v = valid ? nt_load4<4>(src + (part * 8 + i) * 64) : make_float4(0.f, 0.f, 0.f, 0.f);
+        gin[i * 4] = v.x; gin[i * 4 + 1] = v.y; gin[i * 4 + 2] = v.z; gin[i * 4 + 3] = v.w;
+      }
+      PTS8_LAYER(8, 32)(ring, a9, [&](int s) { return gin[s]; });
+    });
+    {
+      float gin[33];
+#pragma unroll
+      for (int i = 0; i < 8; ++i) {
+        const float4 v = valid ? nt_load4<4>(src + (24 + i) * 64) : make_float4(0.f, 0.f, 0.f, 0.f);
+        gin[i * 4] = v.x; gin[i * 4 + 1] = v.y; gin[i * 4 + 2] = v.z; gin[i * 4 + 3] = v.w;
+      }
+      gin[32] = valid ? src[32 * 64].x : (h == 1 ? 1.0f : 0.f);
+      PTS8_LAYER(8, 33)(ring, a9, [&](int s) { return gin[s]; });
+    }
+    acc_zero(g);
+    PTS8_LAYER(4, 129)(ring, g, [&](int s) { return s < 128 ? elu_s(a9[s / 16][s % 16]) : one_h0; });
+    acc_elu(g);
+  }
+  if (DYN) {
+    const float4* pe = reinterpret_cast<const float4*>(p.blob + DY_OFF_POSENC + ((valid ? kt_self * 32 + j : 0) * 2 + h) * 64);
+#pragma unroll
+    for (int t = 0; t < 4; ++t)
+#pragma unroll
+      for (int q = 0; q < 4; ++q) {
+        const float4 v = pe[t * 4 + q];
+        g[t][q * 4] += v.x; g[t][q * 4 + 1] += v.y; g[t][q * 4 + 2] += v.z; g[t][q * 4 + 3] += v.w;
+      }
+  }
+  DYN_PHASE(1);
+  f32x16 att[4];
+  {
+    const float inv_temp = 1.0f / 5.656854249492381f;
+    const int wave0 = wave_u - kt_self;
+    auto split8 = [&](const float (&v)[8], u32x4v& hi, u32x4v& mid) DYN_INLINE_LAMBDA {
+#pragma unroll
+      for (int p2 = 0; p2 < 4; ++p2) {
+        unsigned h_, m_, l_;
+        split3_pair(v[2 * p2], v[2 * p2 + 1], h_, m_, l_);
+        hi[p2] = h_; mid[p2] = m_;
+      }
+    };
+    u32x4v* Kimg = reinterpret_cast<u32x4v*>(KV);
+    f32x16 vnext;
+    dyn_static_for<4>([&](auto HD) DYN_INLINE_LAMBDA {
+      constexpr int hd = decltype(HD)::value;
+      f32x16 qk[2], vh;
+      acc_zero(qk);
+      PTS8_LAYER(2, 64)(ring, qk, [&](int s) { return g[s / 16][s % 16]; });
+      lds_barrier();
+#pragma unroll
+      for (int m = 0; m < 2; ++m) {
+        float kv[8];
+#pragma unroll
+        for (int e = 0; e < 8; ++e) kv[e] = qk[1][8 * m + e];
+        u32x4v khi, kmid;
+        split8(kv, khi, kmid);
+        Kimg[((wave_u * 2 + m) * 2 + 0) * 64 + lane] = khi;
+        Kimg[((wave_u * 2 + m) * 2 + 1) * 64 + lane] = kmid;
+      }
+      u32x4v qhi[2], qmid[2];
+#pragma unroll
+      for (int m = 0; m < 2; ++m) {
+        float qv[8];
+#pragma unroll
+        for (int e = 0; e < 8; ++e) qv[e] = qk[0][8 * m + e] * inv_temp;
+        split8(qv, qhi[m], qmid[m]);
+      }
+      if constexpr (hd % 2 == 0) {
+        f32x16 vv2[2];
+        acc_zero(vv2);
+        PTS8_LAYER(2, 64)(ring, vv2, [&](int s) { return g[s / 16][s % 16]; });
+        vh = vv2[0];
+        vnext = vv2[1];
+      } else {
+        vh = vnext;
+      }
+      lds_barrier();
+      f32x16 sc[MAXT];
+      acc_zero(sc);
+#pragma unroll
+      for (int kt = 0; kt < MAXT; ++kt)
+        if (kt < TPR) {
+#pragma unroll
+          for (int m = 0; m < 2; ++m) {
+            const u32x4v ahi = Kimg[(((wave0 + kt) * 2 + m) * 2 + 0) * 64 + lane], amid = Kimg[(((wave0 + kt) * 2 + m) * 2 + 1) * 64 + lane];
+            sc[kt] = mfma_bf16(amid, qhi[m], sc[kt]);
+            sc[kt] = mfma_bf16(ahi, qmid[m], sc[kt]);
+            sc[kt] = mfma_bf16(ahi, qhi[m], sc[kt]);
+          }
+          __builtin_amdgcn_sched_barrier(0);
+        }
+      float mx = -3.0e38f;
+#pragma unroll
+      for (int kt = 0; kt < MAXT; ++kt)
+        if (kt < TPR) {
+#pragma unroll
+          for (int r = 0; r < 16; ++r) {
+            const bool key_ok = kt * 32 + dyn_fi(r, h) < p.S;
+            float v = q_ok ? sc[kt][r] : -1e9f;
+            v = key_ok ? v : -3.0e38f;
+            sc[kt][r] = v;
+            mx = fmaxf(mx, v);
+          }
+        }
+      mx = fmaxf(mx, __shfl_xor(mx, 32));
+      float sum = 0.f;
+#pragma unroll
+      for (int kt = 0; kt < MAXT; ++kt)
+        if (kt < TPR) {
+#pragma unroll
+          for (int r = 0; r < 16; ++r) {
+            const float e = sc[kt][r] > -1.0e38f ? __expf(sc[kt][r] - mx) : 0.f;
+            sc[kt][r] = e;
+            sum += e;
+          }
+        }
+      sum += __shfl_xor(sum, 32);
+      const float inv = 1.0f / sum;
+      lds_barrier();
+#pragma unroll
+      for (int r = 0; r < 16; ++r) KV[dyn_fi(r, h) * SB8_VL_LD + wave_u * 32 + j] = vh[r];
+      lds_barrier();
+      f32x16 oh;
+#pragma unroll
+      for (int r = 0; r < 16; ++r) oh[r] = 0.f;
+#pragma unroll
+      for (int kt = 0; kt < MAXT; ++kt)
+        if (kt < TPR) {
+#pragma unroll
+          for (int m = 0; m < 2; ++m) {
+            const float* vrow = KV + j * SB8_VL_LD + (wave0 + kt) * 32 + 16 * m + 4 * h;
+            const float4 v0 = *reinterpret_cast<const float4*>(vrow), v1 = *reinterpret_cast<const float4*>(vrow + 8);
+            const float vv[8] = {v0.x, v0.y, v0.z, v0.w, v1.x, v1.y, v1.z, v1.w};
+            float pv[8];
+#pragma unroll
+            for (int e = 0; e < 8; ++e) pv[e] = sc[kt][8 * m + e] * inv;
+            u32x4v ahi, amid, phi, pmid;
+            split8(vv, ahi, amid);
+            split8(pv, phi, pmid);
+            oh = mfma_bf16(amid, phi, oh);
+            oh = mfma_bf16(ahi, pmid, oh);
+            oh = mfma_bf16(ahi, phi, oh);
+          }
+          __builtin_amdgcn_sched_barrier(0);
+        }
+      att[hd] = oh;
+    });
+  }
+  int lane_t = lane;
 #if defined(__AMDGCN__)
-    asm volatile("" ::"v"(sink));
+  asm volatile("" : "+v"(lane_t));
 #endif
-    ring3_next_pass(ring);
-  }
+  const int j_t = lane_t & 31, h_t = lane_t >> 5;
+  const float one_h0_t = h_t == 0 ? 1.0f : 0.0f;
+  {
+    DYN_PHASE(3);
+    PTS8_LAYER(4, 64)(ring, g, [&](int s) { return att[s / 16][s % 16]; });
+    f32x16 (&o)[4] = g;
+    float s1 = 0.f;
+#pragma unroll
+    for (int t = 0; t < 4; ++t)
+#pragma unroll
+      for (int r = 0; r < 16; ++r) s1 += o[t][r];
+    s1 += __shfl_xor(s1, 32);
+    const float mu = s1 * (1.0f / 128.0f);
+    float s2 = 0.f;
+#pragma unroll
+    for (int t = 0; t < 4; ++t)
+#pragma unroll
+      for (int r = 0; r < 16; ++r) {
+        const float d = o[t][r] - mu;
+        s2 += d * d;
+      }
+    s2 += __shfl_xor(s2, 32);
+    const float rstd = 1.0f / sqrtf(s2 * (1.0f / 128.0f) + 1e-6f);
+    const float* gam = ctab + h_t * 64;
+    const float* bet = ctab + 128 + h_t * 64;
+#pragma unroll
+    for (int t = 0; t < 4; ++t)
+#pragma unroll
+      for (int r = 0; r < 16; ++r) g[t][r] = (o[t][r] - mu) * rstd * gam[t * 16 + r] + bet[t * 16 + r];
+  }
+  DYN_PHASE(4);
+  const long point = valid ? ray * p.S + kt_self * 32 + j_t : 0;
+  if (!DYN) {
+    f32x16 a[4];
+    acc_zero(a);
+    PTS8_LAYER(4, 65)(ring, a, [&](int s) { return s < 64 ? g[s / 16][s % 16] : one_h0_t; });
+    acc_elu_s(a);
+    float sigma = row_dot<4>(a, ctab + 256) + ctab[384];
+    if (few_views) sigma = -1e9f;
+    if (valid && h_t == 0) p.raw[point * 4 + 3] = sigma;
+    acc_zero(a);
+    PTS8_LAYER(4, 65)(ring, a, [&](int s) { return s < 64 ? g[s / 16][s % 16] : one_h0_t; });
+    if (valid) {
+      float4* dst = reinterpret_cast<float4*>(p.ws + p.o.off_hg) + tile * SB_HG_RECS * 64 + lane;
+#pragma unroll
+      for (int t = 0; t < 4; ++t)
+#pragma unroll
+        for (int q = 0; q < 4; ++q) dst[(t * 4 + q) * 64] = make_float4(a[t][q * 4], a[t][q * 4 + 1], a[t][q * 4 + 2], a[t][q * 4 + 3]);
+    }
+  } else {
+    f32x16 g2[4];
+    {
+      f32x16 a8[8];
+      acc_zero(a8);
+      PTS8_LAYER(8, 64)(ring, a8, [&](int s) { return g[s / 16][s % 16]; });
+      float pe[17];
+      float c3[3] = {0.f, 0.f, 0.f};
+      if (valid) { c3[0] = p.pts[point * 3]; c3[1] = p.pts[point * 3 + 1]; c3[2] = p.pts[point * 3 + 2]; }
+#pragma unroll
+      for (int c = 0; c < 3; ++c) octave_embed<5>(c3[c], h_t, pe + c * 5);
+      pe[15] = h_t == 0 ? c3[0] : c3[1];
+      pe[16] = h_t == 0 ? c3[2] : 1.0f;
+      PTS8_LAYER(8, 17)(ring, a8, [&](int s) { return pe[s]; });
+      acc_zero(g2);
+      PTS8_LAYER(4, 129)(ring, g2, [&](int s) { return s < 128 ? elu_s(a8[s / 16][s % 16]) : one_h0_t; });
+    }
+    f32x16 a[4];
+    acc_zero(a);
+    PTS8_LAYER(4, 65)(ring, a, [&](int s) {
+      if (s >= 64) return one_h0_t;
+      const float r = elu1(g2[s / 16][s % 16]);
+      g2[s / 16][s % 16] = r;
+      return r;
+    });
+    acc_elu_s(a);
+    float sigma = row_dot<4>(a, ctab + 256) + ctab[384] - p.shift;
+    if (few_views) sigma = -1e9f;
+    float pd[14];
+    {
+      float d3[3] = {0.f, 0.f, 1.f};
+      if (valid) unit3(p.ray_d[ray * 3], p.ray_d[ray * 3 + 1], p.ray_d[ray * 3 + 2], d3[0], d3[1], d3[2]);
+#pragma unroll
+      for (int c = 0; c < 3; ++c) octave_embed<4>(d3[c], h_t, pd + c * 4);
+      pd[12] = h_t == 0 ? d3[0] : d3[1];
+      pd[13] = h_t == 0 ? d3[2] : 1.0f;
+    }
+    acc_zero(a);
+    PTS8_LAYER(4, 78)(ring, a, [&](int s) { return s < 64 ? g2[s / 16][s % 16] : pd[s - 64]; });
+    f32x16 b2[2];
+    acc_zero(b2);
+    PTS8_LAYER(2, 65)(ring, b2, [&](int s) { return s < 64 ? elu_s(a[s / 16][s % 16]) : one_h0_t; });
+    acc_elu_s(b2);
+    float rgb[3];
+#pragma unroll
+    for (int c = 0; c < 3; ++c) {
+      rgb[c] = sigmoid1(row_dot<2>(b2, ctab + 400 + c * 64) + ctab[385 + c]);
+      if (no_view) rgb[c] = 0.f;
+    }
+    if (valid && h_t == 0) reinterpret_cast<float4*>(p.raw)[point] = make_float4(rgb[0], rgb[1], rgb[2], sigma);
+  }
+  DYN_PHASE(20);
+}
 #endif
-  wgi += gridDim.x;
-  } while (PERSIST && wgi < n_wg);
-}
 
 #define DYN_BLEND_THREADS 256
 template <int VSEG, int THREADS>
@@ -1914,7 +2187,14 @@
   else if (q->V <= 16) DYN_LAUNCH(DYN_K_STATIC_VIEWS, "k_static_views", k_static_views<16>, grid_a, blk_v, lds_a, stream, a);
   else DYN_LAUNCH(DYN_K_STATIC_VIEWS, "k_static_views", k_static_views<32>, grid_a, blk_v, lds_a, stream, a);
   if (a.TPR <= 4) {
-    DYN_LAUNCH(DYN_K_STATIC_POINTS, "k_static_points", (k_net_points<false, 0>), points_grid(grid_b), blk, lds_b, stream, a);
+#if DYN_POINTS_DUO
+    const dim3 grid_b8(dyn_cdiv(a.n_tiles_b, DYN_VIEW_THREADS / 64));
+    const size_t lds_b8 = (PTS_RING_SLOTS * PTS_CHUNK + SB_CT + SB8_KV_FLOATS) * sizeof(float);
+    if (a.TPR <= 2) DYN_LAUNCH(DYN_K_STATIC_POINTS, "k_static_points", (k_net_points_w8<false, 2>), grid_b8, blk_v, lds_b8, stream, a);
+    else DYN_LAUNCH(DYN_K_STATIC_POINTS, "k_static_points", (k_net_points_w8<false, 4>), grid_b8, blk_v, lds_b8, stream, a);
+#else
+    DYN_LAUNCH(DYN_K_STATIC_POINTS, "k_static_points", (k_net_points<false, 0>), grid_b, blk, lds_b, stream, a);
+#endif
   } else {
     DYN_LAUNCH(DYN_K_STATIC_POINTS_QKV, "k_static_points_qkv", (k_net_points<false, 1>), grid_b, blk, lds_b, stream, a);
     DYN_LAUNCH(DYN_K_STATIC_POINTS, "k_static_points", (k_net_points<false, 2>), grid_b, blk, lds_b, stream, a);
@@ -1975,6 +2255,7 @@
   pack_net_layer(o, 4, SA_L5_STEPS, scaled(chained(T[DT_VIS2_W], nullptr, 128, 128, 128), DYN_ELU_POST));
   pack_net_layer(o, 4, SA_L5_STEPS, scaled(chained(T[DT_VISB0_W], nullptr, 128, 128, 128), DYN_ELU_PRE));
   DYN_REQUIRE(o.size() == DY_OFF_B, "dynamic pack: A stream size mismatch");
+  const auto pack_b = [&](bool by_head) {
 #if DYN_POINTS_DUO
   g_pack_chunk_pairs = PTS_CP;
 #endif
@@ -1987,9 +2268,13 @@
     }, DYN_ELU_PRE));
   }
   pack_net_layer(o, 4, 129, scaled_wb(chained(T[DT_GEO2_W], T[DT_GEO2_B], 128, 256, 256), 128, DYN_ELU_POST, 1.0));
-  pack_net_layer(o, 4, 64, chained(T[DT_WQ], nullptr, 128, 128, 128));
-  pack_net_layer(o, 4, 64, chained(T[DT_WK], nullptr, 128, 128, 128));
-  pack_net_layer(o, 4, 64, chained(T[DT_WV], nullptr, 128, 128, 128));
+  if (by_head) {
+    pack_qkv_by_head(o, T[DT_WQ], T[DT_WK], T[DT_WV]);
+  } else {
+    pack_net_layer(o, 4, 64, chained(T[DT_WQ], nullptr, 128, 128, 128));
+    pack_net_layer(o, 4, 64, chained(T[DT_WK], nullptr, 128, 128, 128));
+    pack_net_layer(o, 4, 64, chained(T[DT_WV], nullptr, 128, 128, 128));
+  }
   pack_net_layer(o, 4, 64, chained(T[DT_FC], nullptr, 128, 128, 128));
   {
     const float *W = T[DT_REFPTS0_W], *b = T[DT_REFPTS0_B];
@@ -2015,6 +2300,8 @@
   }
   pack_net_layer(o, 2, 65, scaled_wb(chained(T[DT_RGB2_W], T[DT_RGB2_B], 64, 128, 128), 64, DYN_ELU_POST * DYN_ELU_PRE, DYN_ELU_PRE));
   g_pack_chunk_pairs = B6_CHUNK_PAIRS;
+  };
+  pack_b(false);
   DYN_REQUIRE(o.size() == DY_OFF_CTA, "dynamic pack: B stream size mismatch");
   pack_rowtab(o, T[DT_VIS2_W] + 128 * 128, 128, DYN_ELU_POST);
   pack_rowtab(o, T[DT_VISB2_W], 128, DYN_ELU_POST);
@@ -2045,7 +2332,11 @@
   for (int i = 0; i < 256; ++i) o.push_back(T[DT_RAYDIR0_B][i]);
   for (int i = 0; i < 35 * 256; ++i) o.push_back(T[DT_RAYDIR2_W][i]);
   for (int i = 0; i < 35; ++i) o.push_back(T[DT_RAYDIR2_B][i]);
-  o.resize(DY_BLOB_FLOATS, 0.f);
+  o.resize(DY_OFF_B8, 0.f);
+#if DYN_POINTS_DUO
+  pack_b(true);
+#endif
+  DYN_REQUIRE(o.size() == DY_BLOB_FLOATS, "dynamic pack: B8 stream size mismatch");
   DYN_REQUIRE(!g_pack_range_error, "dyn_dynamic_net_pack: a weight is outside the half-float range of the split engine (|w| >= 65504 or not finite)");
   for (size_t i = 0; i < DY_BLOB_FLOATS; ++i) blob[i] = o[i];
   return 0;
@@ -2156,7 +2447,14 @@
   else if (q->V <= 16) DYN_LAUNCH(DYN_K_DYNAMIC_VIEWS, "k_dynamic_views", k_dynamic_views<16>, grid_a, blk_v, lds_a, stream, a);
   else DYN_LAUNCH(DYN_K_DYNAMIC_VIEWS, "k_dynamic_views", k_dynamic_views<32>, grid_a, blk_v, lds_a, stream, a);
   if (a.TPR <= 4) {
-    DYN_LAUNCH(DYN_K_DYNAMIC_POINTS, "k_dynamic_points", (k_net_points<true, 0>), points_grid(grid_b), blk, lds_b, stream, a);
+#if DYN_POINTS_DUO
+    const dim3 grid_b8(dyn_cdiv(a.n_tiles_b, DYN_VIEW_THREADS / 64));
+    const size_t lds_b8 = (PTS_RING_SLOTS * PTS_CHUNK + DB_CT + SB8_KV_FLOATS) * sizeof(float);
+    if (a.TPR <= 2) DYN_LAUNCH(DYN_K_DYNAMIC_POINTS, "k_dynamic_points", (k_net_points_w8<true, 2>), grid_b8, blk_v, lds_b8, stream, a);
+    else DYN_LAUNCH(DYN_K_DYNAMIC_POINTS, "k_dynamic_points", (k_net_points_w8<true, 4>), grid_b8, blk_v, lds_b8, stream, a);
+#else
+    DYN_LAUNCH(DYN_K_DYNAMIC_POINTS, "k_dynamic_points", (k_net_points<true, 0>), grid_b, blk, lds_b, stream, a);
+#endif
   } else {
     DYN_LAUNCH(DYN_K_DYNAMIC_POINTS_QKV, "k_dynamic_points_qkv", (k_net_points<true, 1>), grid_b, blk, lds_b, stream, a);
     DYN_LAUNCH(DYN_K_DYNAMIC_POINTS, "k_dynamic_points", (k_net_points<true, 2>), grid_b, blk, lds_b, stream, a);
```
